# sanderslab/magellanmapper

Hardware: AMD Instinct MI355X
Metric: Mvoxels/s, 2048x2048x1024 uint16 stack, 5-sigma LoG blob detection (higher is better)
Workload: dtype f16x2 MFMA (f32 accumulate) + 16-bit fixed-point intermediates; f64 re-score of every candidate

## Files before the change

### include/mmx.h

```cpp
#ifndef MMX_H
#define MMX_H

#include <stddef.h>
#include <stdint.h>

#ifdef __cplusplus
extern "C" {
#endif

#define MMX_ABI_VERSION 19

typedef enum {
    MMX_OK = 0,
    MMX_ERR_ARG = 1,
    MMX_ERR_HIP = 2,
    MMX_ERR_NO_DEVICE = 3,
    MMX_ERR_WORKSPACE = 4,
    MMX_ERR_UNSUPPORTED = 5,
    MMX_DEFERRED = 6
} mmx_status;

typedef enum { MMX_U8 = 0, MMX_U16 = 1, MMX_F32 = 2, MMX_F64 = 3 } mmx_dtype;

#define MMX_MAX_RADIUS_FAST 24
#define MMX_MAX_RADIUS_GENERIC 255
#define MMX_MAX_BLOCKS 65535
#define MMX_COLOC_BALL 33

typedef struct {
    int64_t src_off;
    int32_t nz, ny, nx;
    int32_t slot;
    int32_t px;
    int32_t _pad;
} mmx_block;
#define MMX_ROW_ALIGN 32

typedef struct {
    const void* d_data;
    int32_t dtype;
    float value_range;
    int64_t stride_z, stride_y, stride_x;
} mmx_volume;

typedef struct {
    int32_t slot;
    int32_t s;
    int32_t z, y, x;
    uint32_t flags;
    float v;
    float nbr_max;
    double v64;
    uint64_t band;
} mmx_cand;

#define MMX_CAND_CONTESTED 1u
#define MMX_CAND_BAND 2u
#define MMX_CAND_PROBE 4u

int mmx_abi_version(void);
const char* mmx_strerror(int status);
const char* mmx_last_hip_error(void);
int mmx_device_count(void);

typedef enum {
    MMX_ZX_AUTO = -1,
    MMX_ZX_SEPARATE = 0,
    MMX_ZX_PACKED = 2,
    MMX_ZX_TILED = 6,
    MMX_ZX_TILED_Q16 = 7
} mmx_zx_mode;
#define MMX_ZX_PREPACKED 0x100
#define MMX_ZX_Y_VALU    0x200
#define MMX_MASK_ROWS 1
#define MMX_MASK_QUADS 2
int mmx_log_batch_f32(const mmx_volume* vol, const mmx_block* d_blocks, const mmx_block* h_blocks,
                      int n_blocks, int64_t slot_elems,
                      const double* h_w0, const double* h_w2, int radius, double norm,
                      float* d_log, float* d_work, uint64_t* d_nms_mask, float nms_lo, float nms_eps,
                      int* h_mask_written, int zx_mode, int* h_zx_path, void* stream);

#define MMX_LOG_ABS_TOL 1e-4

double mmx_tiled_q16_error_bound(const double* h_w0, const double* h_w2, int radius, double norm);

int mmx_zx_pack(const mmx_volume* vol, const mmx_block* d_blocks, const mmx_block* h_blocks, int n_blocks,
                int64_t slot_elems, float* d_work, void* stream);

size_t mmx_workspace_bytes(int n_blocks, int64_t slot_elems, int n_sigma, int with_masks);

int mmx_log_batch_f32_generic(const mmx_volume* vol, const mmx_block* d_blocks,
                              const mmx_block* h_blocks, int n_blocks, int64_t slot_elems,
                              const double* h_w0, const double* h_w2, int radius, double norm,
                              float* d_log, float* d_work, void* stream);

int mmx_peaks_batch(const float* d_log, const uint64_t* d_nms_mask, int mask_layout, int n_sigma, const mmx_block* d_blocks,
                    const mmx_block* h_blocks, int n_blocks, int64_t slot_elems,
                    float thr, float eps, mmx_cand* d_cands, uint32_t cap,
                    uint32_t* d_count, void* stream);

int mmx_rescore_f64(const mmx_volume* vol, const mmx_block* d_blocks, int n_blocks,
                    mmx_cand* d_pts, uint32_t cap, const uint32_t* d_count,
                    const double* d_w0, const double* d_w2, const int32_t* h_radius,
                    const double* h_norm, int n_sigma, int store_f32, void* stream);

int mmx_expand_probes(mmx_cand* d_cands, uint32_t cap, uint32_t* d_count, uint32_t* d_n_cands,
                      const mmx_block* d_blocks, int n_blocks, int n_sigma, void* stream);

typedef struct {
    const mmx_volume* vol32;
    const mmx_volume* vol_exact;
    const mmx_block* d_blocks;
    const mmx_block* h_blocks;
    int32_t n_blocks, n_sigma;
    int64_t slot_elems;
    const double* h_w0; const double* h_w2;
    const double* d_w0; const double* d_w2;
    const int32_t* h_radius;
    const double* h_norm;
    float* d_work;
    size_t work_bytes;
    float thr, eps;
    mmx_cand* d_cands;
    uint32_t cap, h_prefix;
    uint32_t* d_count;
    uint32_t* h_count;
    mmx_cand* h_cands;
    int32_t zx_mode, zx_flags, store_f32, exact, expand, _pad;
    void* stream; void* tail_stream; void* pack_stream;
    void* ev_work_free; void* ev_work_read; void* ev_done;
} mmx_detect_args;
typedef struct {
    int32_t zx_path;
    int32_t mask_layout;
    int32_t n_pass_rounds;
    int32_t _pad;
    double q16_bound;
} mmx_detect_info;
int mmx_detect_batch(const mmx_detect_args* args, mmx_detect_info* info);
const char* mmx_detect_last_error(void);
int mmx_log_scales_f32(const mmx_detect_args* args, mmx_detect_info* info);
int mmx_detect_batch_capture(const mmx_detect_args* args, mmx_detect_info* info, void** graph);
int mmx_graph_launch(void* graph, void* stream, void* ev_done, mmx_detect_info* info);
int mmx_graph_destroy(void* graph);
int mmx_event_synchronize(void* ev);
int mmx_stream_wait_event(void* stream, void* ev);
int mmx_timing_is_enabled(void);

int mmx_overlap_pairs(const double* d_blobs, const int32_t* d_offsets, int n_blocks,
                      double overlap, double band, double max_sigma, int32_t* d_pairs, double* d_frac,
                      uint32_t cap, uint32_t* d_count, void* stream);

int mmx_close_pairs(const int32_t* d_master, int n_master, const int32_t* d_check, int n_check,
                    const int32_t tol[3], int32_t* d_last, uint8_t* d_hit, void* stream);

typedef struct {
    int64_t src_off;
    int64_t dst_off;
    int64_t scratch_off;
    int32_t nz, ny, nx;
    int32_t qclass;
} mmx_subblock;

typedef struct {
    int32_t lo_prev, lo_next, hi_prev, hi_next;
    double lo_gamma, hi_gamma;
} mmx_quantile_class;

typedef struct {
    double clip_min, clip_max;
    double max_thresh;
    double unsharp_strength;
    double erosion_threshold;
    int32_t radius;
    int32_t rgb_guess;
    double tv_weight;
    double tv_factor;
} mmx_preproc_params;

#define MMX_PP_IDENTITY 1
#define MMX_PP_ERODED 2
#define MMX_PP_EXACT_MEAN 4
typedef struct {
    double vmin, vmax, mean;
    int32_t flags;
    int32_t _pad;
} mmx_subblock_info;

#define MMX_PP_RADIUS 32
#define MMX_PP_MAX_SIDE 32
#define MMX_PP_MAX_LDS 163840

int64_t mmx_preprocess_fast_lds(int nz, int ny, int nx);

int mmx_preprocess_batch(const mmx_volume* vol, const mmx_subblock* d_subs, const mmx_subblock* h_subs,
                         int n_subs, const mmx_quantile_class* d_qclasses, int n_qclasses,
                         const mmx_preproc_params* params, const double* d_weights,
                         int64_t dst_sy, int64_t dst_sz, float* d_out32, double* d_out64,
                         mmx_subblock_info* d_info, void* stream);

#define MMX_PP_AUTO 0
#define MMX_PP_SINGLE 1
#define MMX_PP_PIPELINED 2
#define MMX_PP_TILES_PER_WG 8
int64_t mmx_preprocess_work_bytes(const mmx_subblock* h_subs, int n_subs);
int mmx_preprocess_batch_mode(const mmx_volume* vol, const mmx_subblock* d_subs, const mmx_subblock* h_subs,
                              int n_subs, const mmx_quantile_class* d_qclasses, int n_qclasses,
                              const mmx_preproc_params* params, const double* d_weights,
                              int64_t dst_sy, int64_t dst_sz, float* d_out32, double* d_out64,
                              mmx_subblock_info* d_info, int mode, int tiles_per_wg,
                              void* d_work, int64_t work_bytes, void* stream);

int mmx_preprocess_batch_generic(const mmx_volume* vol, const mmx_subblock* d_subs,
                                 const mmx_subblock* h_subs, int n_subs,
                                 const mmx_quantile_class* d_qclasses, int n_qclasses,
                                 const mmx_preproc_params* params, const double* d_weights,
                                 int64_t dst_sy, int64_t dst_sz, float* d_out32, double* d_out64,
                                 mmx_subblock_info* d_info, double* d_scratch, int64_t scratch_doubles,
                                 void* stream);

int mmx_coloc_means(const mmx_volume* vol, const mmx_block* d_blocks, int n_blocks,
                    const int32_t* d_blobs, const int32_t* d_offsets, int n_blobs,
                    double* d_mean, int32_t* d_count, void* stream);
int mmx_coloc_voxels(const mmx_volume* vol, const mmx_block* d_blocks, int n_blocks,
                     const int32_t* d_blobs, const int32_t* d_offsets, int n_blobs,
                     double* d_mean, int32_t* d_count, double* d_voxels, void* stream);

int mmx_unmix_batch(const mmx_volume* vol, const mmx_volume* h_subs, const double* h_facs, int n_subs,
                    const mmx_block* d_blocks, const mmx_block* h_blocks, int n_blocks,
                    int64_t dst_slot, int64_t dst_sy, int64_t dst_sz,
                    float* d_out32, double* d_out64, void* stream);

typedef struct {
    int64_t src_off;
    int32_t in_nz, in_ny, in_nx;
    int32_t out_nz, out_ny, out_nx;
    int32_t slot;
    int32_t tz, ty, tx;
} mmx_resize_block;
int mmx_minmax_batch(const mmx_volume* vol, const mmx_block* d_blocks, const mmx_block* h_blocks,
                     int n_blocks, double* d_minmax, void* stream);
int mmx_resize_batch(const mmx_volume* vol, const mmx_resize_block* d_blocks,
                     const mmx_resize_block* h_blocks, int n_blocks,
                     const int32_t* d_index, const double* d_weight, const double* d_minmax,
                     int64_t dst_slot, int64_t dst_sy, int64_t dst_sz,
                     void* d_out, float* d_out32, void* stream);

int mmx_resize_batch_as(const mmx_volume* vol, const mmx_resize_block* d_blocks,
                        const mmx_resize_block* h_blocks, int n_blocks,
                        const int32_t* d_index, const double* d_weight, const double* d_minmax,
                        int64_t dst_slot, int64_t dst_sy, int64_t dst_sz,
                        int out_dtype, void* d_out, float* d_out32, void* stream);

int mmx_gauss_axis_batch(const mmx_volume* vol, const mmx_block* d_blocks, const mmx_block* h_blocks,
                         int n_blocks, int axis, const double* d_weights, const int32_t* d_radius,
                         int w_pitch, int nearest, int64_t dst_slot, int64_t dst_sy, int64_t dst_sz,
                         void* d_out, void* stream);

typedef struct { int32_t z0, z1; int64_t rank[4]; } mmx_rank_group;
size_t mmx_order_stats_workspace(int n_groups);
int mmx_order_stats(const mmx_volume* vol, int64_t nz, int64_t ny, int64_t nx,
                    const mmx_rank_group* d_groups, const mmx_rank_group* h_groups, int n_groups,
                    double* d_stats , int32_t* d_nan ,
                    void* d_work, size_t work_bytes, void* stream);

#define MMX_K_COUNT 13
int mmx_timing_enable(int on);
int mmx_timing_read(double* ms, int64_t* launches, int n);

int mmx_copy_rect_h2d(void* d_dst, size_t dpitch, const void* h_src, size_t spitch, size_t width, size_t height,
                      void* stream);
int mmx_host_stage_upload(const void* h_src, void* d_dst, const int64_t* regions, int32_t n_regions, int64_t nz,
                          int64_t ny, int64_t row_bytes, void* const* h_staging, int64_t staging_bytes, int32_t depth,
                          void* const* events, void* stream, int32_t device, int64_t* n_queued, const int32_t* cancel,
                          int32_t n_threads);
int mmx_event_query(void* ev);
int mmx_event_create(void** ev);
int mmx_event_destroy(void* ev);
int mmx_event_record(void* ev, void* stream);
int mmx_event_elapsed_ms(void* start, void* stop, float* ms);

int mmx_host_prune_axis(const int32_t* zyx, const int32_t* tag, double* abs_zyx,
                        const int64_t* cur, int64_t n_cur, int axis, int n_sections,
                        const double* bounds, double last_end, const int32_t tol[3],
                        const double* nxt_lo, const double* nxt_hi,
                        int64_t* out_cur, int64_t* out_n,
                        int64_t* n_slab, int64_t* n_after, int64_t* n_next);

typedef struct {
    const int32_t* src_cols;
    int64_t n_out, n_main;
    int32_t abs_dst[3];
} mmx_row_layout;
int mmx_host_take_rows(const double* table, int64_t ld, const int64_t* rows, int64_t n, const double* abs_zyx,
                       const mmx_row_layout* layout, double* out, double* out_rest);
int mmx_host_gather_parts_by_key(const double* table, int64_t ld, int32_t n_parts, const int64_t* const* ids,
                                 const int64_t* const* keys, const double* const* abs_rows, const int64_t* n_rows,
                                 int64_t n_keys, const mmx_row_layout* layout, double* out, int64_t out_rows,
                                 double* out_rest);

int mmx_host_prune_region(const int32_t* zyx, const int32_t* tag, double* abs_zyx, const int64_t* cur, int64_t n_cur,
                          int64_t own_lo, int64_t own_hi, const int32_t n_sections[3], const double* const bounds[3],
                          const double last_end[3], const int32_t tol[3], const double* const nxt_lo[3],
                          const double* const nxt_hi[3], int64_t* out_rows, int64_t* out_keys, int64_t* out_n,
                          int64_t* n_slab, int64_t* n_after, int64_t* n_next, int64_t stat_ld);
int mmx_host_prune_parts(const int32_t* zyx, const int32_t* tag, const double* abs_zyx, const double* chan,
                         int64_t chan_ld, const int64_t* parts, int n_parts, int own_part, const int32_t box_lo[3],
                         const int32_t box_hi[3], const double* channels, int n_channels,
                         const int32_t n_sections[3], const double* const bounds[3], const double last_end[3],
                         const int32_t tol[3], const double* const nxt_lo[3], const double* const nxt_hi[3],
                         int64_t n_keys, int64_t* out_ids, int64_t* out_keys, double* out_abs, int64_t* out_n,
                         int64_t* n_slab, int64_t* n_after, int64_t* n_next, int64_t stat_ld);
int mmx_host_rows_in_boxes(const int32_t* zyx, const int32_t* tag, const double* abs_zyx, const double* chan,
                           int64_t chan_ld, int64_t n, const int32_t* box_lo, const int32_t* box_hi, int n_boxes,
                           double* out, int64_t cap, int64_t* out_n);
int mmx_host_append_rows(const double* payload, int64_t n, const int32_t lo[3], const int32_t hi[3], int32_t* zyx,
                         int32_t* tag, double* abs_zyx, double* chan, int64_t chan_ld, int64_t at, int64_t cap,
                         int64_t* out_n);
int mmx_host_emit_parts(const double* table, int64_t ld, int32_t n_parts, const int64_t* const* ids,
                        const int64_t* const* keys, const double* const* abs_rows, const int64_t* n_rows,
                        const mmx_row_layout* layout, double* out, int64_t out_rows);
int mmx_host_merge_parts_by_key(const double* const* parts, const int64_t* n_rows, int32_t n_parts, int64_t ld,
                                int64_t n_keys, int64_t n_cols, double* out, int64_t out_rows);

int mmx_host_map_columns(const double* table, int64_t ld, int64_t n, const int32_t* src_cols,
                         int32_t n_map, double* out, int64_t out_ld, int32_t dst_col0);

int mmx_host_resolve_peaks(const mmx_cand* cands, uint32_t n_cands, uint32_t n_total, const mmx_block* blocks,
                           int n_blocks, int n_sigma, double thr, int32_t* out_nz_coords, double* out_nz_vals,
                           int32_t* out_coords, double* out_vals, int32_t* offsets, uint8_t* ties, double* stats);
int mmx_host_overlap_prune(const int32_t* coords, const int32_t* offsets, int n_blocks, const double* sigmas,
                           int n_sigma, double overlap, double band, uint8_t* alive, uint8_t* open_blocks,
                           int32_t* pairs, double* frac, int64_t cap, int64_t* n_pairs, int64_t* n_knife);
int mmx_host_emit_tables(const int32_t* coords, const uint8_t* alive, const int32_t* offsets, int n_blocks,
                         const double* sigmas, int n_sigma, double channel, const double* block_offsets,
                         const int32_t* block_tags, const int32_t* interior, double* store, int64_t ld,
                         int32_t* zyx, int32_t* tag, double* abs_zyx, int64_t row0, int64_t capacity,
                         int64_t* rows_per_block);
int mmx_host_emit_tables_multi(int32_t n_channels, const int32_t* const* coords, const uint8_t* const* alive,
                               const int32_t* const* offsets, int n_blocks, const double* const* sigmas,
                               const int32_t* n_sigma, const double* channel_ids, const double* block_offsets,
                               const int32_t* block_tags, const int32_t* interior, double* store, int64_t ld,
                               int32_t n_extra, int32_t* zyx, int32_t* tag, double* abs_zyx, int64_t row0,
                               int64_t capacity, int64_t* rows_per_block, uint8_t* any_before, int32_t* coloc_rows);
int mmx_host_coloc_flags(const double* means, const int32_t* mean_channels, int32_t n_mean_channels, int64_t n,
                         const int32_t* rows, const int64_t* row_offsets, int n_blocks, const int32_t* shapes,
                         int32_t n_channels, double* flags, int64_t ld);

typedef struct {
    const mmx_cand* cands; uint32_t n_cands, n_total;
    const mmx_block* blocks; int32_t n_blocks, n_sigma;
    double thr, eps;
    const double* sigmas; double overlap, overlap_band;
    double channel;
    const double* block_offsets; const int32_t* block_tags; const int32_t* interior;
    double* store; int64_t ld; int32_t* zyx; int32_t* tag; double* abs_zyx; int64_t capacity;
    int64_t* rows_per_block; uint8_t* any_before;
    const int32_t* n_sections; const double* const* bounds; const double* last_end; const int32_t* tol;
    const double* const* nxt_lo; const double* const* nxt_hi;
    int64_t* n_slab; int64_t* n_after; int64_t* n_next; int64_t stat_ld;
    const int32_t* src_cols; int32_t n_out, abs_dst0;
    double* out; int64_t out_capacity; int64_t* out_rows;
    double* stats;
} mmx_finish_stack_args;
int mmx_host_finish_stack(const mmx_finish_stack_args* a);

int mmx_cdist_f64(const double* d_a, int64_t n, const double* d_b, int64_t m, int dim, double* d_out, void* stream);
int mmx_host_lsap(const double* cost, int64_t nr, int64_t nc, int64_t* out_rows, int64_t* out_cols);

int mmx_calib_stream(int kind, const void* d_in, void* d_out, int64_t n_elems, void* stream);

#ifdef __cplusplus
}
#endif
#endif
```

### magellanmapper_amd/_native.py

```python
from __future__ import annotations

import ctypes
import os
from ctypes import (POINTER, Structure, c_char_p, c_double, c_float, c_int, c_int32, c_int64,
                    c_uint8, c_uint32, c_void_p)

import numpy as np

_HERE = os.path.dirname(os.path.abspath(__file__))
LIB_PATH = os.environ.get("MMX_LIB_PATH") or os.path.join(_HERE, "libmmx_hip.so")

MMX_ABI_VERSION = 19
MMX_U8, MMX_U16, MMX_F32, MMX_F64 = 0, 1, 2, 3
MMX_MAX_RADIUS_FAST = 24
MMX_MAX_RADIUS_GENERIC = 255
MMX_CAND_CONTESTED = 1
MMX_CAND_BAND = 2
MMX_CAND_PROBE = 4
MMX_ZX_AUTO, MMX_ZX_SEPARATE, MMX_ZX_PACKED, MMX_ZX_MFMA_F32, MMX_ZX_MFMA_F16, MMX_ZX_MFMA_F16_LDS = -1, 0, 2, 3, 4, 5
MMX_ZX_TILED, MMX_ZX_TILED_Q16, MMX_ZX_PREPACKED, MMX_ZX_Y_VALU = 6, 7, 0x100, 0x200
MMX_MASK_ROWS, MMX_MASK_QUADS = 1, 2
MMX_MAX_BLOCKS = 65535
MMX_COLOC_BALL = 33

BLOCK_DTYPE = np.dtype([("src_off", "<i8"), ("nz", "<i4"), ("ny", "<i4"), ("nx", "<i4"),
                        ("slot", "<i4"), ("px", "<i4"), ("_pad", "<i4")], align=True)
MMX_ROW_ALIGN = 32
CAND_DTYPE = np.dtype([("slot", "<i4"), ("s", "<i4"), ("z", "<i4"), ("y", "<i4"), ("x", "<i4"),
                       ("flags", "<u4"), ("v", "<f4"), ("nbr_max", "<f4"), ("v64", "<f8"),
                       ("band", "<u8")], align=True)
assert BLOCK_DTYPE.itemsize == 32 and CAND_DTYPE.itemsize == 48
SUBBLOCK_DTYPE = np.dtype([("src_off", "<i8"), ("dst_off", "<i8"), ("scratch_off", "<i8"),
                           ("nz", "<i4"), ("ny", "<i4"), ("nx", "<i4"), ("qclass", "<i4")], align=True)
QCLASS_DTYPE = np.dtype([("lo_prev", "<i4"), ("lo_next", "<i4"), ("hi_prev", "<i4"), ("hi_next", "<i4"),
                         ("lo_gamma", "<f8"), ("hi_gamma", "<f8")], align=True)
SUBINFO_DTYPE = np.dtype([("vmin", "<f8"), ("vmax", "<f8"), ("mean", "<f8"), ("flags", "<i4"),
                          ("_pad", "<i4")], align=True)
assert SUBBLOCK_DTYPE.itemsize == 40 and QCLASS_DTYPE.itemsize == 32 and SUBINFO_DTYPE.itemsize == 32
MMX_PP_IDENTITY, MMX_PP_ERODED, MMX_PP_EXACT_MEAN = 1, 2, 4
MMX_PP_AUTO, MMX_PP_SINGLE, MMX_PP_PIPELINED = 0, 1, 2
RESIZE_DTYPE = np.dtype([("src_off", "<i8"), ("in_nz", "<i4"), ("in_ny", "<i4"), ("in_nx", "<i4"),
                         ("out_nz", "<i4"), ("out_ny", "<i4"), ("out_nx", "<i4"), ("slot", "<i4"),
                         ("tz", "<i4"), ("ty", "<i4"), ("tx", "<i4")], align=True)
assert RESIZE_DTYPE.itemsize == 48
RANK_GROUP_DTYPE = np.dtype([("z0", "<i4"), ("z1", "<i4"), ("rank", "<i8", (4,))], align=True)
assert RANK_GROUP_DTYPE.itemsize == 40


class Volume(Structure):
    _fields_ = [("d_data", c_void_p), ("dtype", c_int32), ("value_range", c_float),
                ("stride_z", c_int64), ("stride_y", c_int64), ("stride_x", c_int64)]


class DetectArgs(Structure):
    _fields_ = [("vol32", POINTER(Volume)), ("vol_exact", POINTER(Volume)), ("d_blocks", c_void_p),
                ("h_blocks", c_void_p), ("n_blocks", c_int32), ("n_sigma", c_int32), ("slot_elems", c_int64),
                ("h_w0", c_void_p), ("h_w2", c_void_p), ("d_w0", c_void_p), ("d_w2", c_void_p),
                ("h_radius", c_void_p), ("h_norm", c_void_p), ("d_work", c_void_p), ("work_bytes", ctypes.c_size_t),
                ("thr", c_float), ("eps", c_float), ("d_cands", c_void_p), ("cap", c_uint32), ("h_prefix", c_uint32),
                ("d_count", c_void_p), ("h_count", c_void_p), ("h_cands", c_void_p),
                ("zx_mode", c_int32), ("zx_flags", c_int32), ("store_f32", c_int32), ("exact", c_int32),
                ("expand", c_int32), ("_pad", c_int32),
                ("stream", c_void_p), ("tail_stream", c_void_p), ("pack_stream", c_void_p),
                ("ev_work_free", c_void_p), ("ev_work_read", c_void_p), ("ev_done", c_void_p)]


class FinishStackArgs(Structure):
    _fields_ = [("cands", c_void_p), ("n_cands", c_uint32), ("n_total", c_uint32),
                ("blocks", c_void_p), ("n_blocks", c_int32), ("n_sigma", c_int32),
                ("thr", c_double), ("eps", c_double),
                ("sigmas", c_void_p), ("overlap", c_double), ("overlap_band", c_double),
                ("channel", c_double),
                ("block_offsets", c_void_p), ("block_tags", c_void_p), ("interior", c_void_p),
                ("store", c_void_p), ("ld", c_int64), ("zyx", c_void_p), ("tag", c_void_p), ("abs_zyx", c_void_p),
                ("capacity", c_int64), ("rows_per_block", c_void_p), ("any_before", c_void_p),
                ("n_sections", c_void_p), ("bounds", c_void_p), ("last_end", c_void_p), ("tol", c_void_p),
                ("nxt_lo", c_void_p), ("nxt_hi", c_void_p),
                ("n_slab", c_void_p), ("n_after", c_void_p), ("n_next", c_void_p), ("stat_ld", c_int64),
                ("src_cols", c_void_p), ("n_out", c_int32), ("abs_dst0", c_int32),
                ("out", c_void_p), ("out_capacity", c_int64), ("out_rows", c_void_p),
                ("stats", c_void_p)]


MMX_DEFERRED = 6


class RowLayout(Structure):
    _fields_ = [("src_cols", POINTER(c_int32)), ("n_out", c_int64), ("n_main", c_int64), ("abs_dst", c_int32 * 3)]


class DetectInfo(Structure):
    _fields_ = [("zx_path", c_int32), ("mask_layout", c_int32), ("n_pass_rounds", c_int32), ("_pad", c_int32),
                ("q16_bound", c_double)]


class PreprocParams(Structure):
    _fields_ = [("clip_min", c_double), ("clip_max", c_double), ("max_thresh", c_double),
                ("unsharp_strength", c_double), ("erosion_threshold", c_double),
                ("radius", c_int32), ("rgb_guess", c_int32), ("tv_weight", c_double), ("tv_factor", c_double)]


class MmxError(RuntimeError):
    """A C-ABI call returned a non-zero status."""


_lib = None

SYMBOLS = (
    "mmx_abi_version", "mmx_strerror", "mmx_last_hip_error", "mmx_device_count",
    "mmx_detect_batch", "mmx_log_scales_f32", "mmx_detect_batch_capture", "mmx_graph_launch", "mmx_graph_destroy", "mmx_detect_last_error",
    "mmx_event_synchronize", "mmx_stream_wait_event", "mmx_timing_is_enabled",
    "mmx_log_batch_f32", "mmx_log_batch_f32_generic", "mmx_zx_pack", "mmx_tiled_q16_error_bound", "mmx_workspace_bytes", "mmx_peaks_batch", "mmx_rescore_f64",
    "mmx_overlap_pairs", "mmx_close_pairs", "mmx_event_create", "mmx_event_destroy",
    "mmx_event_record", "mmx_event_elapsed_ms", "mmx_timing_enable", "mmx_timing_read",
    "mmx_calib_stream", "mmx_host_prune_axis",
    "mmx_preprocess_fast_lds", "mmx_preprocess_batch", "mmx_preprocess_batch_mode", "mmx_preprocess_work_bytes", "mmx_preprocess_batch_generic",
    "mmx_coloc_means", "mmx_coloc_voxels", "mmx_host_take_rows", "mmx_host_map_columns", "mmx_resize_batch_as", "mmx_gauss_axis_batch", "mmx_unmix_batch", "mmx_minmax_batch", "mmx_resize_batch",
    "mmx_cdist_f64", "mmx_host_lsap", "mmx_expand_probes", "mmx_host_resolve_peaks", "mmx_host_overlap_prune",
    "mmx_host_emit_tables", "mmx_host_prune_region", "mmx_host_prune_parts", "mmx_host_rows_in_boxes", "mmx_host_append_rows", "mmx_host_emit_parts", "mmx_host_merge_parts_by_key", "mmx_host_gather_parts_by_key", "mmx_host_emit_tables_multi", "mmx_host_coloc_flags", "mmx_host_finish_stack", "mmx_copy_rect_h2d", "mmx_host_stage_upload", "mmx_event_query",
    "mmx_order_stats_workspace", "mmx_order_stats",
)
KERNEL_KINDS = ("zpass", "ypass", "xpass", "generic", "peaks", "rescore", "overlap_pairs",
                "close_pairs", "zxpass", "y2pass", "preproc", "coloc", "zxpack")


def lib() -> ctypes.CDLL:
    global _lib
    if _lib is not None:
        return _lib
    if not os.path.exists(LIB_PATH):
        raise MmxError(
            f"{LIB_PATH} not found: the HIP extension has not been built "
            "(run __graft_entry__.build() or make -C magellanmapper_amd/csrc). "
            "There is no CPU fallback for this path.")
    try:
        import torch
    except ImportError:
        pass
    L = ctypes.CDLL(LIB_PATH)
    vp = c_void_p
    L.mmx_abi_version.restype = c_int
    L.mmx_strerror.restype = c_char_p
    L.mmx_strerror.argtypes = [c_int]
    L.mmx_last_hip_error.restype = c_char_p
    L.mmx_device_count.restype = c_int
    log_args = [POINTER(Volume), vp, vp, c_int, c_int64, POINTER(c_double), POINTER(c_double),
                c_int, c_double, vp, vp]
    L.mmx_log_batch_f32.argtypes = log_args + [vp, c_float, c_float, POINTER(c_int), c_int, POINTER(c_int), vp]
    L.mmx_log_batch_f32_generic.argtypes = log_args + [vp]
    L.mmx_workspace_bytes.argtypes = [c_int, c_int64, c_int, c_int]
    L.mmx_workspace_bytes.restype = ctypes.c_size_t
    L.mmx_zx_pack.argtypes = [POINTER(Volume), vp, vp, c_int, c_int64, vp, vp]
    L.mmx_tiled_q16_error_bound.argtypes = [POINTER(c_double), POINTER(c_double), c_int, c_double]
    L.mmx_tiled_q16_error_bound.restype = c_double
    L.mmx_peaks_batch.argtypes = [vp, vp, c_int, c_int, vp, vp, c_int, c_int64, c_float, c_float, vp,
                                  c_uint32, vp, vp]
    L.mmx_rescore_f64.argtypes = [POINTER(Volume), vp, c_int, vp, c_uint32, vp, vp, vp,
                                  POINTER(c_int32), POINTER(c_double), c_int, c_int, vp]
    L.mmx_overlap_pairs.argtypes = [vp, vp, c_int, c_double, c_double, c_double, vp, vp, c_uint32, vp, vp]
    L.mmx_close_pairs.argtypes = [vp, c_int, vp, c_int, POINTER(c_int32), vp, vp, vp]
    L.mmx_detect_batch.argtypes = [POINTER(DetectArgs), POINTER(DetectInfo)]
    L.mmx_log_scales_f32.argtypes = [POINTER(DetectArgs), POINTER(DetectInfo)]
    L.mmx_detect_batch_capture.argtypes = [POINTER(DetectArgs), POINTER(DetectInfo), POINTER(vp)]
    L.mmx_graph_launch.argtypes = [vp, vp, vp, POINTER(DetectInfo)]
    L.mmx_graph_destroy.argtypes = [vp]
    L.mmx_detect_last_error.restype = c_char_p
    L.mmx_event_synchronize.argtypes = [vp]
    L.mmx_stream_wait_event.argtypes = [vp, vp]
    L.mmx_event_create.argtypes = [POINTER(vp)]
    L.mmx_event_destroy.argtypes = [vp]
    L.mmx_event_record.argtypes = [vp, vp]
    L.mmx_event_elapsed_ms.argtypes = [vp, vp, POINTER(c_float)]
    L.mmx_timing_enable.argtypes = [c_int]
    L.mmx_timing_read.argtypes = [POINTER(c_double), POINTER(c_int64), c_int]
    L.mmx_calib_stream.argtypes = [c_int, vp, vp, c_int64, vp]
    L.mmx_host_prune_axis.argtypes = [vp, vp, vp, vp, c_int64, c_int, c_int, vp, c_double,
                                      POINTER(c_int32), vp, vp, vp, POINTER(c_int64), vp, vp, vp]
    L.mmx_preprocess_fast_lds.argtypes = [c_int, c_int, c_int]
    L.mmx_preprocess_fast_lds.restype = c_int64
    pre_args = [POINTER(Volume), vp, vp, c_int, vp, c_int, POINTER(PreprocParams), vp,
                c_int64, c_int64, vp, vp, vp]
    L.mmx_preprocess_batch.argtypes = pre_args + [vp]
    L.mmx_preprocess_batch_mode.argtypes = pre_args + [c_int, c_int, vp, c_int64, vp]
    L.mmx_preprocess_work_bytes.argtypes = [vp, c_int]
    L.mmx_preprocess_work_bytes.restype = c_int64
    L.mmx_preprocess_batch_generic.argtypes = pre_args + [vp, c_int64, vp]
    L.mmx_minmax_batch.argtypes = [POINTER(Volume), vp, vp, c_int, vp, vp]
    L.mmx_minmax_batch.restype = c_int
    L.mmx_resize_batch.argtypes = [POINTER(Volume), vp, vp, c_int, vp, vp, vp, c_int64, c_int64, c_int64,
                                   vp, vp, vp]
    L.mmx_resize_batch.restype = c_int
    L.mmx_resize_batch_as.argtypes = [POINTER(Volume), vp, vp, c_int, vp, vp, vp, c_int64, c_int64, c_int64,
                                      c_int, vp, vp, vp]
    L.mmx_resize_batch_as.restype = c_int
    L.mmx_gauss_axis_batch.argtypes = [POINTER(Volume), vp, vp, c_int, c_int, vp, vp, c_int, c_int,
                                       c_int64, c_int64, c_int64, vp, vp]
    L.mmx_gauss_axis_batch.restype = c_int
    L.mmx_unmix_batch.argtypes = [POINTER(Volume), POINTER(Volume), POINTER(c_double), c_int, vp, vp, c_int,
                                  c_int64, c_int64, c_int64, vp, vp, vp]
    L.mmx_unmix_batch.restype = c_int
    L.mmx_host_take_rows.argtypes = [vp, c_int64, vp, c_int64, vp, POINTER(RowLayout), vp, vp]
    L.mmx_host_map_columns.argtypes = [vp, c_int64, c_int64, POINTER(c_int32), c_int32, vp, c_int64, c_int32]
    L.mmx_cdist_f64.argtypes = [vp, c_int64, vp, c_int64, c_int, vp, vp]
    L.mmx_cdist_f64.restype = c_int
    L.mmx_host_lsap.argtypes = [vp, c_int64, c_int64, vp, vp]
    L.mmx_host_lsap.restype = c_int
    L.mmx_coloc_means.argtypes = [POINTER(Volume), vp, c_int, vp, vp, c_int, vp, vp, vp]
    L.mmx_coloc_means.restype = c_int
    L.mmx_coloc_voxels.argtypes = [POINTER(Volume), vp, c_int, vp, vp, c_int, vp, vp, vp, vp]
    L.mmx_coloc_voxels.restype = c_int
    L.mmx_expand_probes.argtypes = [vp, c_uint32, vp, vp, vp, c_int, c_int, vp]
    L.mmx_expand_probes.restype = c_int
    L.mmx_host_resolve_peaks.argtypes = [vp, c_uint32, c_uint32, vp, c_int, c_int, c_double, vp, vp, vp, vp, vp, vp, vp]
    L.mmx_host_overlap_prune.argtypes = [vp, vp, c_int, vp, c_int, c_double, c_double, vp, vp, vp, vp, c_int64,
                                         POINTER(c_int64), POINTER(c_int64)]
    L.mmx_host_prune_region.argtypes = [vp, vp, vp, vp, c_int64, c_int64, c_int64, POINTER(c_int32), POINTER(vp),
                                        POINTER(c_double), POINTER(c_int32), POINTER(vp), POINTER(vp), vp, vp,
                                        POINTER(c_int64), vp, vp, vp, c_int64]
    L.mmx_host_prune_parts.argtypes = [vp, vp, vp, vp, c_int64, vp, c_int, c_int, POINTER(c_int32), POINTER(c_int32),
                                       vp, c_int, POINTER(c_int32), POINTER(vp), POINTER(c_double), POINTER(c_int32),
                                       POINTER(vp), POINTER(vp), c_int64, vp, vp, vp, POINTER(c_int64), vp, vp, vp,
                                       c_int64]
    L.mmx_host_rows_in_boxes.argtypes = [vp, vp, vp, vp, c_int64, c_int64, vp, vp, c_int, vp, c_int64, POINTER(c_int64)]
    L.mmx_host_append_rows.argtypes = [vp, c_int64, POINTER(c_int32), POINTER(c_int32), vp, vp, vp, vp, c_int64,
                                       c_int64, c_int64, POINTER(c_int64)]
    L.mmx_host_gather_parts_by_key.argtypes = [vp, c_int64, c_int32, vp, vp, vp, vp, c_int64, POINTER(RowLayout), vp, c_int64, vp]
    L.mmx_host_emit_parts.argtypes = [vp, c_int64, c_int32, vp, vp, vp, vp, POINTER(RowLayout), vp, c_int64]
    L.mmx_host_merge_parts_by_key.argtypes = [vp, vp, c_int32, c_int64, c_int64, c_int64, vp, c_int64]
    L.mmx_host_emit_tables_multi.argtypes = [c_int32, vp, vp, vp, c_int, vp, vp, vp, vp, vp, vp, vp, c_int64, c_int32, vp, vp,
                                             vp, c_int64, c_int64, vp, vp, vp]
    L.mmx_host_coloc_flags.argtypes = [vp, vp, c_int32, c_int64, vp, vp, c_int, vp, c_int32, vp, c_int64]
    L.mmx_host_finish_stack.argtypes = [POINTER(FinishStackArgs)]
    L.mmx_host_stage_upload.argtypes = [vp, vp, vp, c_int32, c_int64, c_int64, c_int64, vp, c_int64, c_int32, vp, vp, c_int32,
                                        vp, vp, c_int32]
    L.mmx_event_query.argtypes = [vp]
    L.mmx_copy_rect_h2d.argtypes = [vp, ctypes.c_size_t, vp, ctypes.c_size_t, ctypes.c_size_t, ctypes.c_size_t, vp]
    L.mmx_host_emit_tables.argtypes = [vp, vp, vp, c_int, vp, c_int, c_double, vp, vp, vp, vp, c_int64, vp, vp, vp,
                                       c_int64, c_int64, vp]
    L.mmx_order_stats_workspace.argtypes = [c_int]
    L.mmx_order_stats_workspace.restype = ctypes.c_size_t
    L.mmx_order_stats.argtypes = [POINTER(Volume), c_int64, c_int64, c_int64, vp, vp, c_int, vp, vp, vp, ctypes.c_size_t, vp]
    L.mmx_order_stats.restype = c_int
    L.mmx_preprocess_batch.restype = c_int
    L.mmx_preprocess_batch_mode.restype = c_int
    L.mmx_preprocess_batch_generic.restype = c_int
    for name in SYMBOLS:
        fn = getattr(L, name)
        if name in ("mmx_preprocess_fast_lds", "mmx_workspace_bytes", "mmx_preprocess_work_bytes",
                    "mmx_order_stats_workspace"):
            continue
        if fn.restype is None or name.startswith(("mmx_log", "mmx_peaks", "mmx_rescore",
                                                  "mmx_overlap", "mmx_close", "mmx_event", "mmx_timing", "mmx_calib", "mmx_host")):
            fn.restype = c_int
    if L.mmx_abi_version() != MMX_ABI_VERSION:
        raise MmxError("libmmx_hip.so ABI version mismatch")
    _lib = L
    return L


def check(status: int, what: str) -> None:
    if status != 0:
        L = lib()
        msg = L.mmx_strerror(status).decode()
        hip = L.mmx_last_hip_error().decode()
        raise MmxError(f"{what}: {msg}" + (f" ({hip})" if hip else ""))


def as_double_ptr(a: np.ndarray):
    assert a.dtype == np.float64 and a.flags.c_contiguous
    return a.ctypes.data_as(POINTER(c_double))


def as_int32_ptr(a: np.ndarray):
    assert a.dtype == np.int32 and a.flags.c_contiguous
    return a.ctypes.data_as(POINTER(c_int32))


def timing_enable(on: bool = True, kinds=None) -> None:
    mask = 1 if on else 0
    if on and kinds is not None:
        mask = 0
        for k in kinds:
            mask |= 1 << (KERNEL_KINDS.index(k) + 1)
    check(lib().mmx_timing_enable(mask), "mmx_timing_enable")


def timing_read() -> dict:
    ms = (c_double * len(KERNEL_KINDS))()
    n = (c_int64 * len(KERNEL_KINDS))()
    check(lib().mmx_timing_read(ms, n, len(KERNEL_KINDS)), "mmx_timing_read")
    return {k: (ms[i], n[i]) for i, k in enumerate(KERNEL_KINDS)}


def keep_host_heap(mmap_threshold: int = 1 << 30, trim_threshold: int = (1 << 31) - 1) -> bool:
    try:
        libc = ctypes.CDLL("libc.so.6")
        ok1 = libc.mallopt(-3, int(mmap_threshold))
        ok2 = libc.mallopt(-1, int(trim_threshold))
        return bool(ok1 and ok2)
    except (OSError, AttributeError):
        return False
```

### magellanmapper_amd/csrc/mmx_api.hip

```cpp

#include <atomic>
#include <cstdio>
#include <cstdlib>
#include <cstring>

#include "mmx_common.h"

int mmx_launch_generic_pass(int pass, const mmx_volume* vol, const mmx_block* d_blocks, int n_blocks,
                            int max_vox, int64_t slot_elems, const float* w0, const float* w2, int radius,
                            const float* in1, const float* in2, float* out1, float* out2, hipStream_t s);
int mmx_launch_peaks(const float* d_log, int n_sigma, int64_t sigma_stride, const mmx_block* d_blocks,
                     int n_blocks, int max_vox, int64_t slot_elems, float thr, float eps,
                     mmx_cand* d_cands, uint32_t cap, uint32_t* d_count, hipStream_t stream);
int mmx_launch_peaks_sparse(const float* d_log, const unsigned long long* d_mask, int n_sigma,
                            int64_t sigma_stride, const mmx_block* d_blocks, int n_blocks, int max_vox,
                            int64_t slot_elems, float thr, float eps, mmx_cand* d_cands, uint32_t cap,
                            uint32_t* d_count, int quads, hipStream_t stream);

#include <mutex>
#include <vector>

namespace {
thread_local char g_hip_err[256] = "";

struct span { hipEvent_t a, b; int kind; };
std::mutex g_tm;
bool g_timing = false;
uint32_t g_kinds = ~0u;
std::vector<span> g_spans;
std::vector<hipEvent_t> g_pool;
hipEvent_t g_open[MMX_K_COUNT];

hipEvent_t take_event()
{
    if (!g_pool.empty()) { hipEvent_t e = g_pool.back(); g_pool.pop_back(); return e; }
    hipEvent_t e = nullptr;
    hipEventCreate(&e);
    return e;
}

int hip_fail(hipError_t e, const char* what)
{
    snprintf(g_hip_err, sizeof g_hip_err, "%s: %s", what, hipGetErrorString(e));
    return MMX_ERR_HIP;
}

constexpr int kColPrefetch = 4;
}

void mmx_time_begin(int kind, hipStream_t s)
{
    std::lock_guard<std::mutex> lk(g_tm);
    if (!g_timing || !((g_kinds >> kind) & 1u)) return;
    g_open[kind] = take_event();
    hipEventRecord(g_open[kind], s);
}

void mmx_time_end(int kind, hipStream_t s)
{
    std::lock_guard<std::mutex> lk(g_tm);
    if (!g_timing || !g_open[kind]) return;
    hipEvent_t b = take_event();
    hipEventRecord(b, s);
    g_spans.push_back({g_open[kind], b, kind});
    g_open[kind] = nullptr;
}

extern "C" {

int mmx_timing_enable(int on)
{
    std::lock_guard<std::mutex> lk(g_tm);
    for (auto& sp : g_spans) { g_pool.push_back(sp.a); g_pool.push_back(sp.b); }
    g_spans.clear();
    for (int k = 0; k < MMX_K_COUNT; ++k) g_open[k] = nullptr;
    g_timing = on != 0;
    g_kinds = on == 1 ? ~0u : ((uint32_t)on >> 1);
    return MMX_OK;
}

int mmx_timing_is_enabled(void)
{
    std::lock_guard<std::mutex> lk(g_tm);
    return g_timing ? 1 : 0;
}

int mmx_timing_read(double* ms, int64_t* launches, int n)
{
    if (!ms || !launches || n < MMX_K_COUNT) return MMX_ERR_ARG;
    std::lock_guard<std::mutex> lk(g_tm);
    for (int k = 0; k < n; ++k) { ms[k] = 0.0; launches[k] = 0; }
    for (auto& sp : g_spans) {
        hipError_t r = hipEventSynchronize(sp.b);
        if (r != hipSuccess) return hip_fail(r, "hipEventSynchronize");
        float t = 0.f;
        r = hipEventElapsedTime(&t, sp.a, sp.b);
        if (r != hipSuccess) return hip_fail(r, "hipEventElapsedTime");
        ms[sp.kind] += t;
        launches[sp.kind] += 1;
        g_pool.push_back(sp.a);
        g_pool.push_back(sp.b);
    }
    g_spans.clear();
    return MMX_OK;
}

int mmx_abi_version(void) { return MMX_ABI_VERSION; }
size_t mmx_workspace_bytes(int n_blocks, int64_t slot_elems, int n_sigma, int with_masks)
{
    if (n_blocks < 1 || slot_elems < 1 || n_sigma < 1) return 0;
    size_t bytes = (size_t)(4 + n_sigma) * (size_t)n_blocks * (size_t)slot_elems * sizeof(float);
    if (with_masks) {
        bytes = (bytes + 15) & ~(size_t)15;
        bytes += (size_t)n_sigma * (((size_t)n_blocks * (size_t)slot_elems) >> 5) * 16;
    }
    return bytes;
}

const char* mmx_strerror(int status)
{
    switch (status) {
        case MMX_OK: return "ok";
        case MMX_ERR_ARG: return "bad argument";
        case MMX_ERR_HIP: return "HIP runtime error";
        case MMX_ERR_NO_DEVICE: return "no gfx950 device";
        case MMX_ERR_WORKSPACE: return "workspace too small";
        case MMX_ERR_UNSUPPORTED: return "unsupported configuration";
        case MMX_DEFERRED: return "left to the caller";
        default: return "unknown status";
    }
}

const char* mmx_last_hip_error(void) { return g_hip_err; }


int mmx_device_count(void)
{
    int n = 0;
    hipError_t e = hipGetDeviceCount(&n);
    if (e != hipSuccess) { hip_fail(e, "hipGetDeviceCount"); return -1; }
    int ok = 0;
    for (int i = 0; i < n; ++i) {
        hipDeviceProp_t p;
        if (hipGetDeviceProperties(&p, i) == hipSuccess && strncmp(p.gcnArchName, "gfx950", 6) == 0) ++ok;
    }
    return ok;
}

static void q16_bounds(const double* w0, const double* w2, int radius, double norm, double* bp, double* bq, double* err)
{
    double s0 = w0[0], s2 = fabs(w2[0]);
    for (int k = 1; k <= radius; ++k) { s0 += 2.0 * w0[k]; s2 += 2.0 * fabs(w2[k]); }
    *bp = s0 * s0 * (1.0 + 1e-6);
    double pos = 0.0, neg = 0.0;
    for (int i = 0; i <= radius; ++i)
        for (int j = 0; j <= radius; ++j) {
            const double k = (w2[i] * w0[j] + w0[i] * w2[j]) * ((i ? 2.0 : 1.0) * (j ? 2.0 : 1.0));
            if (k > 0.0) pos += k; else neg -= k;
        }
    *bq = (pos > neg ? pos : neg) * (1.0 + 1e-4);
    const double drop = 255.0 / 65536.0 / 2048.0;
    const double biased = 4.0 * 0x1p-22;
    const double ydrop = 255.0 / 4096.0;
    *err = norm * (s2 * (*bp / 65535.0 * (0.5 + ydrop) + drop * s0 * s0 + biased * *bp) +
                   s0 * (*bq / 32767.0 * (0.5 + ydrop) + drop * 2.0 * s2 * s0 + biased * *bq)) + 1e-6;
}

double mmx_tiled_q16_error_bound(const double* h_w0, const double* h_w2, int radius, double norm)
{
    if (!h_w0 || !h_w2 || radius < 0 || radius > MMX_MAX_RADIUS_GENERIC) return -1.0;
    double bp, bq, err;
    q16_bounds(h_w0, h_w2, radius, norm, &bp, &bq, &err);
    return err;
}

}

void mmx_batch_geom_make(const mmx_volume* vol, const mmx_block* h_blocks, int n_blocks, int64_t slot_elems,
                         mmx_batch_geom* g)
{
    *g = mmx_batch_geom{};
    g->min_nz = g->min_ny = g->min_nx = 1 << 30;
    g->plan_status = MMX_ERR_UNSUPPORTED;
    g->rows_fit = g->quads_fit = true;
    if (n_blocks < 1 || n_blocks > MMX_MAX_BLOCKS) {
        g->status = n_blocks < 1 ? MMX_ERR_ARG : MMX_ERR_UNSUPPORTED;
        return;
    }
    for (int i = 0; i < n_blocks; ++i) {
        const mmx_block& b = h_blocks[i];
        if (b.nz < 1 || b.ny < 1 || b.nx < 1 || b.slot != i || b.px < b.nx || b.px % MMX_ROW_ALIGN) {
            if (g->status == MMX_OK) g->status = MMX_ERR_ARG;
            g->bad_block = true;
            return;
        }
        if ((int64_t)b.nz * b.ny * b.px > slot_elems && g->status == MMX_OK) g->status = MMX_ERR_WORKSPACE;
        if (b.nz < g->min_nz) g->min_nz = b.nz;
        if (b.ny < g->min_ny) g->min_ny = b.ny;
        if (b.nx < g->min_nx) g->min_nx = b.nx;
        if (b.ny > g->max_ny) g->max_ny = b.ny;
        if (b.nx > g->max_nx) g->max_nx = b.nx;
        if (b.px > g->max_px) g->max_px = b.px;
        if (b.ny * b.px > g->max_zcols) g->max_zcols = b.ny * b.px;
        if (b.nz * b.px > g->max_ycols) g->max_ycols = b.nz * b.px;
        if (b.nz * b.ny > g->max_rows) g->max_rows = b.nz * b.ny;
        if (b.nz * b.ny * b.px > g->max_vox) g->max_vox = b.nz * b.ny * b.px;
        if ((int64_t)b.ny * (((int64_t)b.nz * b.px + 63) >> 6) > (slot_elems >> 5) - 1) g->rows_fit = false;
        if ((int64_t)b.ny * ((b.nz + 3) >> 2) * ((b.nx + 15) >> 4) > (slot_elems >> 5) - 1) g->quads_fit = false;
        if (vol) {
            const int64_t lane = (int64_t)(b.ny - 1) * vol->stride_y + (int64_t)(b.nx - 1) * vol->stride_x;
            if (lane > g->max_lane_in) g->max_lane_in = lane;
        }
    }
    if (vol) g->plan_status = mmx_zx6_plan_make(h_blocks, n_blocks, slot_elems, vol->dtype, &g->plan);
}

namespace {

struct pass_weights {
    float z0[MMX_MAX_RADIUS_GENERIC + 1], z2[MMX_MAX_RADIUS_GENERIC + 1];
    float y0[MMX_MAX_RADIUS_GENERIC + 1], y2[MMX_MAX_RADIUS_GENERIC + 1];
    float x0[MMX_MAX_RADIUS_GENERIC + 1], x2[MMX_MAX_RADIUS_GENERIC + 1];
};
void make_weights(const mmx_volume* vol, const double* h_w0, const double* h_w2, int radius, double norm, pass_weights* w)
{
    double in_scale = 1.0;
    if (vol->dtype == MMX_U8) in_scale = 1.0 / 255.0;
    else if (vol->dtype == MMX_U16) in_scale = 1.0 / 65535.0;
    for (int k = 0; k <= radius; ++k) {
        w->z0[k] = (float)(h_w0[k] * in_scale);
        w->z2[k] = (float)(h_w2[k] * in_scale);
        w->y0[k] = (float)h_w0[k];
        w->y2[k] = (float)h_w2[k];
        w->x0[k] = (float)(-norm * h_w0[k]);
        w->x2[k] = (float)(-norm * h_w2[k]);
    }
}
mmx_taps_f32 taps(const float* a, const float* b, int radius)
{
    mmx_taps_f32 t;
    for (int k = 0; k <= MMX_MAX_RADIUS_FAST; ++k) {
        t.w0[k] = k <= radius ? a[k] : 0.f;
        t.w2[k] = k <= radius ? b[k] : 0.f;
    }
    return t;
}

int check_log_args(mmx_log_call* c, bool* y_valu, bool* prepacked)
{
    *y_valu = c->zx_mode >= 0 && (c->zx_mode & MMX_ZX_Y_VALU);
    if (*y_valu) c->zx_mode &= ~MMX_ZX_Y_VALU;
    *prepacked = c->zx_mode == (MMX_ZX_TILED | MMX_ZX_PREPACKED) || c->zx_mode == (MMX_ZX_TILED_Q16 | MMX_ZX_PREPACKED);
    if (*prepacked) c->zx_mode &= ~MMX_ZX_PREPACKED;
    if (c->zx_mode < MMX_ZX_AUTO || c->zx_mode > MMX_ZX_TILED_Q16 || c->zx_mode == 1 || (c->zx_mode >= 3 && c->zx_mode <= 5))
        return MMX_ERR_ARG;
    if (!c->vol || !c->vol->d_data || !c->d_blocks || !c->h_blocks || !c->h_w0 || !c->h_w2 || !c->d_log || !c->d_work)
        return MMX_ERR_ARG;
    if (c->n_blocks < 1 || c->radius < 0 || c->slot_elems < 1) return MMX_ERR_ARG;
    if (c->n_blocks > MMX_MAX_BLOCKS) return MMX_ERR_UNSUPPORTED;
    if (c->radius > MMX_MAX_RADIUS_GENERIC) return MMX_ERR_UNSUPPORTED;
    if (c->slot_elems >= (int64_t(1) << 29)) return MMX_ERR_UNSUPPORTED;
    if (c->slot_elems % MMX_ROW_ALIGN) return MMX_ERR_ARG;
    if (c->vol->dtype != MMX_U8 && c->vol->dtype != MMX_U16 && c->vol->dtype != MMX_F32)
        return MMX_ERR_UNSUPPORTED;
    return MMX_OK;
}

int fused_passes(const mmx_log_call& c, bool y_valu, bool prepacked, const mmx_batch_geom& g, const pass_weights& w)
{
    const mmx_volume* vol = c.vol;
    const int radius = c.radius, n_blocks = c.n_blocks;
    const int64_t slot_elems = c.slot_elems;
    hipStream_t s = c.stream;
    const bool fast_r = radius >= 1 && radius <= MMX_MAX_RADIUS_FAST;
    const bool lane_ok = g.max_lane_in * 8 < (int64_t(1) << 31);
    const bool fused = c.zx_mode != MMX_ZX_SEPARATE && fast_r && lane_ok && g.min_ny >= radius + kColPrefetch &&
                       g.min_nz >= radius + 1 && g.min_nx >= radius && g.max_px <= 512 && vol->stride_y < (1 << 30);
    if (!fused) return MMX_ERR_UNSUPPORTED;
    float* t0 = c.d_work;
    float* t1 = c.d_work + (int64_t)n_blocks * slot_elems;
    mmx_taps_f32 tzz = taps(w.z0, w.z2, radius), txx = taps(w.y0, w.y2, radius), tyy = taps(w.x0, w.x2, radius);
    int rc, path = MMX_ZX_PACKED;
    double q_bp = 0, q_bq = 0, q_err = 0, vscale = 0;
    q16_bounds(c.h_w0, c.h_w2, radius, c.norm, &q_bp, &q_bq, &q_err);
    const bool integer = vol->dtype == MMX_U8 || vol->dtype == MMX_U16;
    const bool ranged = vol->dtype == MMX_F32 && vol->value_range != 0.f && fabsf(vol->value_range) < 60000.f;
    const bool wants_entries = c.d_nms_mask && c.h_mask_written;
    const bool q16 = mmx_tiles_q16(c.zx_mode, vol, q_err, c.nms_eps, wants_entries, &vscale);
    const bool nonneg = vscale > 0.0;
    if (q16) { q_bp *= vscale; q_bq *= vscale; }
    bool tiled = (c.zx_mode == MMX_ZX_TILED || (c.zx_mode == MMX_ZX_TILED_Q16 && nonneg) ||
                  (c.zx_mode == MMX_ZX_AUTO && (integer || ranged))) && g.plan_status == MMX_OK;
    const mmx_zx6_plan& plan = g.plan;
    if (tiled && !prepacked) {
        mmx_timed_scope ts(MMX_K_ZXPACK, s);
        rc = mmx_launch_zx6_pack(vol, c.d_blocks, c.h_blocks, n_blocks, plan, c.d_work, s);
        if (rc == MMX_ERR_HIP) return hip_fail(hipGetLastError(), "voxel copy of the tiled path");
        tiled = rc == MMX_OK;
    }
    { mmx_timed_scope ts(MMX_K_ZX, s);
      rc = MMX_ERR_UNSUPPORTED;
      if (tiled) {
          path = q16 ? MMX_ZX_TILED_Q16 : MMX_ZX_TILED;
          rc = mmx_launch_zx6(vol, c.d_blocks, c.h_blocks, n_blocks, plan, txx, radius, c.d_work,
                              q16 ? (float)(1.0 / q_bp) : 0.f, q16 ? (float)(1.0 / q_bq) : 0.f, s);
          tiled = rc == MMX_OK;
      }
      if (rc == MMX_ERR_UNSUPPORTED) {
          path = MMX_ZX_PACKED;
          rc = mmx_launch_zx2(vol, c.d_blocks, n_blocks, g.max_ny, g.max_px, slot_elems, tzz, txx, radius, t0, t1, s);
      } }
    if (rc == MMX_OK && c.h_zx_path) *c.h_zx_path = path;
    if (rc == MMX_OK) {
        mmx_timed_scope ts(MMX_K_Y2, s);
        const bool want_mask = wants_entries && (tiled ? g.quads_fit : g.rows_fit);
        unsigned long long* d_mask = want_mask ? (unsigned long long*)c.d_nms_mask : nullptr;
        rc = MMX_ERR_UNSUPPORTED;
        if (tiled && q16 && !y_valu)
            rc = mmx_launch_ym(c.d_blocks, n_blocks, plan, slot_elems, tyy, radius, c.d_work,
                               (float)(q_bp / 65535.0), (float)(q_bq / 32767.0), c.d_log, d_mask, c.nms_lo, c.nms_eps, s);
        if (rc != MMX_ERR_UNSUPPORTED) ;
        else if (tiled)
            rc = mmx_launch_y6(c.d_blocks, n_blocks, plan, slot_elems, tyy, radius, c.d_work,
                               reinterpret_cast<const float*>(reinterpret_cast<const char*>(c.d_work) + plan.q_off),
                               q16 ? (float)(q_bp / 65535.0) : 0.f, q16 ? (float)(q_bq / 32767.0) : 0.f, c.d_log,
                               d_mask, c.nms_lo, c.nms_eps, s);
        else
            rc = mmx_launch_y2(c.d_blocks, n_blocks, g.max_ycols, slot_elems, tyy, radius, t0, t1, c.d_log,
                               d_mask, c.nms_lo, c.nms_eps, s);
        if (rc == MMX_OK && want_mask) *c.h_mask_written = tiled ? MMX_MASK_QUADS : MMX_MASK_ROWS;
    }
    return rc == MMX_ERR_HIP ? hip_fail(hipGetLastError(), "fused passes") : rc;
}

int separate_passes(const mmx_log_call& c, const mmx_batch_geom& g, const pass_weights& w)
{
    const mmx_volume* vol = c.vol;
    const int radius = c.radius, n_blocks = c.n_blocks;
    const int64_t slot_elems = c.slot_elems;
    hipStream_t s = c.stream;
    float* t0 = c.d_work;
    float* t1 = t0 + (int64_t)n_blocks * slot_elems;
    float* t2 = t1 + (int64_t)n_blocks * slot_elems;
    float* t3 = t2 + (int64_t)n_blocks * slot_elems;
    const bool fast_r = radius >= 1 && radius <= MMX_MAX_RADIUS_FAST;
    const bool lane_ok = g.max_lane_in * 8 < (int64_t(1) << 31);
    const bool fast_z = fast_r && lane_ok && g.min_nz >= radius + kColPrefetch && vol->stride_y < (1 << 30);
    const bool fast_y = fast_r && g.min_ny >= radius + kColPrefetch;
    const bool fast_x = fast_r && g.min_nx >= radius;
    int rc;
    { mmx_timed_scope ts(fast_z ? MMX_K_ZPASS : MMX_K_GENERIC, s);
    if (fast_z) rc = mmx_launch_zpass(vol, c.d_blocks, n_blocks, g.max_zcols, slot_elems, taps(w.z0, w.z2, radius), radius, t0, t1, s);
    else rc = mmx_launch_generic_pass(0, vol, c.d_blocks, n_blocks, g.max_vox, slot_elems, w.z0, w.z2, radius, nullptr, nullptr, t0, t1, s); }
    if (rc != MMX_OK) return rc == MMX_ERR_HIP ? hip_fail(hipGetLastError(), "z pass") : rc;
    { mmx_timed_scope ts(fast_y ? MMX_K_YPASS : MMX_K_GENERIC, s);
    if (fast_y) rc = mmx_launch_ypass(c.d_blocks, n_blocks, g.max_ycols, slot_elems, taps(w.y0, w.y2, radius), radius, t0, t1, t2, t3, s);
    else rc = mmx_launch_generic_pass(1, vol, c.d_blocks, n_blocks, g.max_vox, slot_elems, w.y0, w.y2, radius, t0, t1, t2, t3, s); }
    if (rc != MMX_OK) return rc == MMX_ERR_HIP ? hip_fail(hipGetLastError(), "y pass") : rc;
    { mmx_timed_scope ts(fast_x ? MMX_K_XPASS : MMX_K_GENERIC, s);
    if (fast_x) rc = mmx_launch_xpass(c.d_blocks, n_blocks, g.max_rows, g.max_nx, slot_elems, taps(w.x0, w.x2, radius), radius, t2, t3, c.d_log, s);
    else rc = mmx_launch_generic_pass(2, vol, c.d_blocks, n_blocks, g.max_vox, slot_elems, w.x0, w.x2, radius, t2, t3, c.d_log, nullptr, s); }
    if (rc != MMX_OK) return rc == MMX_ERR_HIP ? hip_fail(hipGetLastError(), "x pass") : rc;
    return MMX_OK;
}

}

int mmx_log_scale_f32(const mmx_log_call& call, const mmx_batch_geom& g)
{
    mmx_log_call c = call;
    if (c.h_mask_written) *c.h_mask_written = 0;
    if (c.h_zx_path) *c.h_zx_path = MMX_ZX_SEPARATE;
    bool y_valu, prepacked;
    int rc = check_log_args(&c, &y_valu, &prepacked);
    if (rc != MMX_OK) return rc;
    if (g.status != MMX_OK) return g.status;
    pass_weights w;
    make_weights(c.vol, c.h_w0, c.h_w2, c.radius, c.norm, &w);
    rc = fused_passes(c, y_valu, prepacked, g, w);
    if (rc != MMX_ERR_UNSUPPORTED) return rc;
    return separate_passes(c, g, w);
}

int mmx_zx_pack_geom(const mmx_volume* vol, const mmx_block* d_blocks, const mmx_block* h_blocks, int n_blocks,
                     int64_t slot_elems, const mmx_batch_geom& g, float* d_work, hipStream_t stream)
{
    if (!vol || !vol->d_data || !d_blocks || !h_blocks || !d_work || n_blocks < 1 || slot_elems < 1) return MMX_ERR_ARG;
    if (n_blocks > MMX_MAX_BLOCKS) return MMX_ERR_UNSUPPORTED;
    if (vol->dtype != MMX_U8 && vol->dtype != MMX_U16 && vol->dtype != MMX_F32) return MMX_ERR_UNSUPPORTED;
    if (g.bad_block) return MMX_ERR_ARG;
    if (g.plan_status != MMX_OK) return g.plan_status;
    mmx_timed_scope ts(MMX_K_ZXPACK, stream);
    const int rc = mmx_launch_zx6_pack(vol, d_blocks, h_blocks, n_blocks, g.plan, d_work, stream);
    return rc == MMX_ERR_HIP ? hip_fail(hipGetLastError(), "voxel copy of the tiled path") : rc;
}

extern "C" {

int mmx_log_batch_f32(const mmx_volume* vol, const mmx_block* d_blocks, const mmx_block* h_blocks,
                      int n_blocks, int64_t slot_elems,
                      const double* h_w0, const double* h_w2, int radius, double norm,
                      float* d_log, float* d_work, uint64_t* d_nms_mask, float nms_lo, float nms_eps,
                      int* h_mask_written, int zx_mode, int* h_zx_path, void* stream)
{
    mmx_batch_geom g{};
    if (vol && h_blocks) mmx_batch_geom_make(vol, h_blocks, n_blocks, slot_elems, &g);
    return mmx_log_scale_f32({vol, d_blocks, h_blocks, n_blocks, slot_elems, h_w0, h_w2, radius, norm, d_log, d_work,
                              d_nms_mask, nms_lo, nms_eps, h_mask_written, zx_mode, h_zx_path, (hipStream_t)stream}, g);
}

int mmx_log_batch_f32_generic(const mmx_volume* vol, const mmx_block* d_blocks, const mmx_block* h_blocks,
                              int n_blocks, int64_t slot_elems,
                              const double* h_w0, const double* h_w2, int radius, double norm,
                              float* d_log, float* d_work, void* stream)
{
    if (!vol || !vol->d_data || !d_blocks || !h_blocks || !h_w0 || !h_w2 || !d_log || !d_work)
        return MMX_ERR_ARG;
    if (n_blocks < 1 || radius < 0 || radius > MMX_MAX_RADIUS_GENERIC || slot_elems < 1) return MMX_ERR_ARG;
    if (n_blocks > MMX_MAX_BLOCKS) return MMX_ERR_UNSUPPORTED;
    mmx_batch_geom g;
    mmx_batch_geom_make(vol, h_blocks, n_blocks, slot_elems, &g);
    if (g.status != MMX_OK) return g.status;
    pass_weights w;
    make_weights(vol, h_w0, h_w2, radius, norm, &w);
    const int64_t n_slots = n_blocks;
    float* t0 = d_work;
    float* t1 = d_work + n_slots * slot_elems;
    float* t2 = t1 + n_slots * slot_elems;
    float* t3 = t2 + n_slots * slot_elems;
    hipStream_t s = (hipStream_t)stream;
    int rc = mmx_launch_generic_pass(0, vol, d_blocks, n_blocks, g.max_vox, slot_elems, w.z0, w.z2, radius, nullptr, nullptr, t0, t1, s);
    if (rc != MMX_OK) return rc;
    rc = mmx_launch_generic_pass(1, vol, d_blocks, n_blocks, g.max_vox, slot_elems, w.y0, w.y2, radius, t0, t1, t2, t3, s);
    if (rc != MMX_OK) return rc;
    return mmx_launch_generic_pass(2, vol, d_blocks, n_blocks, g.max_vox, slot_elems, w.x0, w.x2, radius, t2, t3, d_log, nullptr, s);
}

int mmx_zx_pack(const mmx_volume* vol, const mmx_block* d_blocks, const mmx_block* h_blocks, int n_blocks,
                int64_t slot_elems, float* d_work, void* stream)
{
    mmx_batch_geom g{};
    if (vol && h_blocks) mmx_batch_geom_make(vol, h_blocks, n_blocks, slot_elems, &g);
    return mmx_zx_pack_geom(vol, d_blocks, h_blocks, n_blocks, slot_elems, g, d_work, (hipStream_t)stream);
}

int mmx_peaks_batch(const float* d_log, const uint64_t* d_nms_mask, int mask_layout, int n_sigma, const mmx_block* d_blocks,
                    const mmx_block* h_blocks, int n_blocks, int64_t slot_elems,
                    float thr, float eps, mmx_cand* d_cands, uint32_t cap,
                    uint32_t* d_count, void* stream)
{
    if (!d_log || !d_blocks || !h_blocks || !d_cands || !d_count) return MMX_ERR_ARG;
    if (n_sigma < 1 || n_blocks < 1 || slot_elems < 1 || !(eps >= 0.f)) return MMX_ERR_ARG;
    if (n_blocks > MMX_MAX_BLOCKS) return MMX_ERR_UNSUPPORTED;
    if (slot_elems % MMX_ROW_ALIGN) return MMX_ERR_ARG;
    if (d_nms_mask && mask_layout != MMX_MASK_ROWS && mask_layout != MMX_MASK_QUADS) return MMX_ERR_ARG;
    mmx_batch_geom g;
    mmx_batch_geom_make(nullptr, h_blocks, n_blocks, slot_elems, &g);
    if (g.status != MMX_OK) return g.status;
    const int max_vox = g.max_vox;
    mmx_timed_scope ts(MMX_K_PEAKS, (hipStream_t)stream);
    int rc;
    if (d_nms_mask)
        rc = mmx_launch_peaks_sparse(d_log, (const unsigned long long*)d_nms_mask, n_sigma,
                                     (int64_t)n_blocks * slot_elems, d_blocks, n_blocks, max_vox, slot_elems,
                                     thr, eps, d_cands, cap, d_count, mask_layout == MMX_MASK_QUADS, (hipStream_t)stream);
    else
        rc = mmx_launch_peaks(d_log, n_sigma, (int64_t)n_blocks * slot_elems, d_blocks, n_blocks, max_vox,
                              slot_elems, thr, eps, d_cands, cap, d_count, (hipStream_t)stream);
    return rc == MMX_ERR_HIP ? hip_fail(hipGetLastError(), "peaks") : rc;
}

int mmx_copy_rect_h2d(void* d_dst, size_t dpitch, const void* h_src, size_t spitch, size_t width, size_t height,
                      void* stream)
{
    if (!d_dst || !h_src || width > dpitch || width > spitch) return MMX_ERR_ARG;
    if (!width || !height) return MMX_OK;
    hipError_t r = hipMemcpy2DAsync(d_dst, dpitch, h_src, spitch, width, height, hipMemcpyHostToDevice, (hipStream_t)stream);
    return r == hipSuccess ? MMX_OK : hip_fail(r, "hipMemcpy2DAsync");
}

int mmx_event_create(void** ev)
{
    if (!ev) return MMX_ERR_ARG;
    hipEvent_t e;
    hipError_t r = hipEventCreate(&e);
    if (r != hipSuccess) return hip_fail(r, "hipEventCreate");
    *ev = (void*)e;
    return MMX_OK;
}

int mmx_event_destroy(void* ev)
{
    hipError_t r = hipEventDestroy((hipEvent_t)ev);
    return r == hipSuccess ? MMX_OK : hip_fail(r, "hipEventDestroy");
}

int mmx_event_record(void* ev, void* stream)
{
    hipError_t r = hipEventRecord((hipEvent_t)ev, (hipStream_t)stream);
    return r == hipSuccess ? MMX_OK : hip_fail(r, "hipEventRecord");
}

int mmx_event_elapsed_ms(void* start, void* stop, float* ms)
{
    if (!ms) return MMX_ERR_ARG;
    hipError_t r = hipEventSynchronize((hipEvent_t)stop);
    if (r != hipSuccess) return hip_fail(r, "hipEventSynchronize");
    r = hipEventElapsedTime(ms, (hipEvent_t)start, (hipEvent_t)stop);
    return r == hipSuccess ? MMX_OK : hip_fail(r, "hipEventElapsedTime");
}

}
```

### magellanmapper_amd/csrc/mmx_common.h

```cpp
#pragma once

#include <hip/hip_runtime.h>
#include <stdint.h>

#include "../../include/mmx.h"

#define MMX_WG 256
#define MMX_MAX_GRID_X 2147483647

struct mmx_taps_f32 {
    float w0[MMX_MAX_RADIUS_FAST + 1];
    float w2[MMX_MAX_RADIUS_FAST + 1];
};

__host__ __device__ __forceinline__ int mmx_reflect(int i, int n)
{
    if (n == 1) return 0;
    const int period = 2 * n;
    i %= period;
    if (i < 0) i += period;
    return i < n ? i : period - 1 - i;
}

int mmx_launch_zpass(const mmx_volume* vol, const mmx_block* d_blocks, int n_blocks, int max_cols,
                     int64_t slot_elems, const mmx_taps_f32& taps, int radius,
                     float* d_gz, float* d_gzz, hipStream_t stream);
int mmx_launch_ypass(const mmx_block* d_blocks, int n_blocks, int max_cols, int64_t slot_elems,
                     const mmx_taps_f32& taps, int radius, const float* d_gz, const float* d_gzz,
                     float* d_a, float* d_bc, hipStream_t stream);
int mmx_launch_xpass(const mmx_block* d_blocks, int n_blocks, int max_rows, int max_nx,
                     int64_t slot_elems, const mmx_taps_f32& taps, int radius,
                     const float* d_a, const float* d_bc, float* d_log, hipStream_t stream);

int mmx_launch_zx2(const mmx_volume* vol, const mmx_block* d_blocks, int n_blocks, int max_ny, int max_px,
                   int64_t slot_elems, const mmx_taps_f32& tz, const mmx_taps_f32& tx, int radius,
                   float* d_p, float* d_q, hipStream_t s);
struct mmx_zx6_plan {
    int64_t tile_stride;
    int64_t pack_stride;
    int64_t q_off, tab_off, pack_off;
    int64_t tab_bytes;
    int max_tiles;
    int max_rowtiles;
};
int mmx_zx6_plan_make(const mmx_block* h_blocks, int n_blocks, int64_t slot_elems, int voxel_dtype, mmx_zx6_plan* plan);
int mmx_launch_zx6_pack(const mmx_volume* vol, const mmx_block* d_blocks, const mmx_block* h_blocks, int n_blocks,
                        const mmx_zx6_plan& plan, void* d_work, hipStream_t stream);
int mmx_launch_zx6(const mmx_volume* vol, const mmx_block* d_blocks, const mmx_block* h_blocks, int n_blocks,
                   const mmx_zx6_plan& plan, const mmx_taps_f32& tx, int radius, void* d_work, float qp, float qq,
                   hipStream_t stream);
int mmx_launch_y6(const mmx_block* d_blocks, int n_blocks, const mmx_zx6_plan& plan, int64_t slot_elems,
                  const mmx_taps_f32& taps, int radius, const float* d_p, const float* d_q, float cp, float cq,
                  float* d_log, unsigned long long* d_mask, float nms_lo, float nms_eps, hipStream_t stream);
int mmx_launch_ym(const mmx_block* d_blocks, int n_blocks, const mmx_zx6_plan& plan, int64_t slot_elems,
                  const mmx_taps_f32& taps, int radius, const float* d_p, float cp, float cq,
                  float* d_log, unsigned long long* d_mask, float nms_lo, float nms_eps, hipStream_t stream);
int mmx_launch_y2(const mmx_block* d_blocks, int n_blocks, int max_cols, int64_t slot_elems,
                  const mmx_taps_f32& taps, int radius, const float* d_p, const float* d_q,
                  float* d_log, unsigned long long* d_mask, float nms_lo, float nms_eps, hipStream_t stream);

struct mmx_batch_geom {
    int status;
    bool bad_block;
    int min_nz, min_ny, min_nx, max_ny, max_nx, max_px;
    int max_zcols, max_ycols, max_rows, max_vox;
    int64_t max_lane_in;
    bool rows_fit, quads_fit;
    mmx_zx6_plan plan;
    int plan_status;
};
void mmx_batch_geom_make(const mmx_volume* vol, const mmx_block* h_blocks, int n_blocks, int64_t slot_elems, mmx_batch_geom* g);

struct mmx_log_call {
    const mmx_volume* vol; const mmx_block* d_blocks; const mmx_block* h_blocks; int n_blocks; int64_t slot_elems;
    const double* h_w0; const double* h_w2; int radius; double norm;
    float* d_log; float* d_work; uint64_t* d_nms_mask; float nms_lo, nms_eps; int* h_mask_written;
    int zx_mode; int* h_zx_path; hipStream_t stream;
};
int mmx_log_scale_f32(const mmx_log_call& c, const mmx_batch_geom& g);
int mmx_zx_pack_geom(const mmx_volume* vol, const mmx_block* d_blocks, const mmx_block* h_blocks, int n_blocks,
                     int64_t slot_elems, const mmx_batch_geom& g, float* d_work, hipStream_t stream);

bool mmx_tiles_q16(int zx_mode, const mmx_volume* vol, double unit_bound, double band, bool entries_wanted, double* value_scale);

enum mmx_kernel_kind {
    MMX_K_ZPASS = 0, MMX_K_YPASS, MMX_K_XPASS, MMX_K_GENERIC, MMX_K_PEAKS, MMX_K_RESCORE,
    MMX_K_PAIRS, MMX_K_CLOSE, MMX_K_ZX, MMX_K_Y2, MMX_K_PREPROC, MMX_K_COLOC, MMX_K_ZXPACK, MMX_K_END
};
void mmx_time_begin(int kind, hipStream_t s);
void mmx_time_end(int kind, hipStream_t s);
static_assert(MMX_K_END == MMX_K_COUNT, "kernel kinds out of sync with mmx.h");
struct mmx_timed_scope {
    int kind; hipStream_t s;
    mmx_timed_scope(int k, hipStream_t st) : kind(k), s(st) { mmx_time_begin(k, st); }
    ~mmx_timed_scope() { mmx_time_end(kind, s); }
};
```

### magellanmapper_amd/csrc/mmx_detect.hip

```cpp

#include <algorithm>
#include <atomic>
#include <chrono>
#include <cstdlib>
#include <cmath>
#include <cstdio>
#include <cstring>
#include <mutex>
#include <thread>
#include <vector>

#include "mmx_common.h"

namespace {

thread_local char g_detect_err[256] = "";

std::mutex g_ev_mutex;
std::vector<hipEvent_t> g_ev_ring;
size_t g_ev_next = 0;
hipEvent_t ring_event()
{
    std::lock_guard<std::mutex> lk(g_ev_mutex);
    if (g_ev_ring.size() < 64) {
        hipEvent_t e = nullptr;
        if (hipEventCreateWithFlags(&e, hipEventDisableTiming) != hipSuccess) return nullptr;
        g_ev_ring.push_back(e);
        return e;
    }
    hipEvent_t e = g_ev_ring[g_ev_next];
    g_ev_next = (g_ev_next + 1) % g_ev_ring.size();
    return e;
}

int fail(hipError_t e, const char* what)
{
    snprintf(g_detect_err, sizeof g_detect_err, "%s: %s", what, hipGetErrorString(e));
    return MMX_ERR_HIP;
}

int after(hipStream_t a, hipStream_t b, const char* what)
{
    if (a == b) return MMX_OK;
    hipEvent_t e = ring_event();
    if (!e) return fail(hipErrorOutOfMemory, "hipEventCreate");
    hipError_t r = hipEventRecord(e, a);
    if (r != hipSuccess) return fail(r, what);
    r = hipStreamWaitEvent(b, e, 0);
    return r == hipSuccess ? MMX_OK : fail(r, what);
}

float* log_arrays(const mmx_detect_args* a) { return a->d_work + (size_t)4 * a->n_blocks * a->slot_elems; }
uint64_t* nms_entries(const mmx_detect_args* a)
{
    const float* end = log_arrays(a) + (size_t)a->n_sigma * a->n_blocks * a->slot_elems;
    return reinterpret_cast<uint64_t*>((reinterpret_cast<uintptr_t>(end) + 15) & ~(uintptr_t)15);
}

int passes(const mmx_detect_args* a, const mmx_batch_geom& g, bool with_mask, int mode, unsigned* layouts, int* zx_path,
           double* q16_bound, bool* pack_side)
{
    *layouts = 0;
    const mmx_volume* vol = a->vol32;
    const bool is_float = vol->dtype == MMX_F32;
    const bool float_ok = is_float && vol->value_range != 0.f;
    const int nb = a->n_blocks, ns = a->n_sigma;
    const int64_t slot = a->slot_elems;
    const size_t tab = MMX_MAX_RADIUS_GENERIC + 1;
    float* d_log = log_arrays(a);
    uint64_t* d_mask = nms_entries(a);
    const size_t mask_words = ((size_t)nb * slot) >> 5;
    int tiled_mode = MMX_ZX_TILED;
    if (mode == MMX_ZX_AUTO || mode == MMX_ZX_TILED_Q16) {
        double bound = 0.0;
        for (int s = 0; s < ns; ++s) {
            const double b = mmx_tiled_q16_error_bound(a->h_w0 + s * tab, a->h_w2 + s * tab, a->h_radius[s], a->h_norm[s]);
            if (b < 0) { bound = -1.0; break; }
            if (b > bound) bound = b;
        }
        double vscale;
        if (mmx_tiles_q16(mode, vol, bound, a->eps, true, &vscale)) { tiled_mode = MMX_ZX_TILED_Q16; *q16_bound = bound * vscale; }
    }
    bool packed = false;
    hipStream_t main = (hipStream_t)a->stream;
    if (((mode == MMX_ZX_AUTO || mode == MMX_ZX_TILED || mode == MMX_ZX_TILED_Q16) && !is_float) ||
        ((mode == MMX_ZX_AUTO || mode == MMX_ZX_TILED) && float_ok)) {
        hipStream_t ps = (*pack_side && a->pack_stream) ? (hipStream_t)a->pack_stream : main;
        int rc = mmx_zx_pack_geom(vol, a->d_blocks, a->h_blocks, nb, slot, g, a->d_work, ps);
        if (rc != MMX_OK && rc != MMX_ERR_UNSUPPORTED) return rc;
        if (ps != main) {
            const int st = after(ps, main, "voxel copy -> main stream");
            if (st != MMX_OK) return st;
            *pack_side = false;
        }
        packed = rc == MMX_OK;
    }
    for (int s = 0; s < ns; ++s) {
        int written = 0, path = 0;
        const int rc = mmx_log_scale_f32({vol, a->d_blocks, a->h_blocks, nb, slot, a->h_w0 + s * tab, a->h_w2 + s * tab,
                                          a->h_radius[s], a->h_norm[s], d_log + (size_t)s * nb * slot, a->d_work,
                                          with_mask ? d_mask + (size_t)s * mask_words * 2 : nullptr, a->thr - a->eps, a->eps,
                                          &written, packed ? (tiled_mode | MMX_ZX_PREPACKED | a->zx_flags) : mode, &path,
                                          main}, g);
        if (rc != MMX_OK) return rc;
        *zx_path = path;
        packed = packed && path == tiled_mode;
        *layouts |= 1u << (with_mask ? written : 0);
    }
    return MMX_OK;
}

}

bool mmx_tiles_q16(int zx_mode, const mmx_volume* vol, double unit_bound, double band, bool entries, double* value_scale)
{
    const bool ranged = vol->dtype == MMX_F32 && vol->value_range > 0.f && vol->value_range < 60000.f;
    *value_scale = vol->dtype == MMX_U8 || vol->dtype == MMX_U16 ? 1.0 : (ranged ? (double)vol->value_range : 0.0);
    if (!(*value_scale > 0.0)) return false;
    if (zx_mode == MMX_ZX_TILED_Q16) return true;
    const double bound = unit_bound * *value_scale;
    return zx_mode == MMX_ZX_AUTO && entries && bound >= 0.0 && 4.0 * bound <= band && bound <= MMX_LOG_ABS_TOL;
}

extern "C" {

const char* mmx_detect_last_error(void) { return g_detect_err; }

int mmx_log_scales_f32(const mmx_detect_args* a, mmx_detect_info* info)
{
    if (!a || !info) return MMX_ERR_ARG;
    memset(info, 0, sizeof *info);
    if (!a->vol32 || !a->d_blocks || !a->h_blocks || !a->h_w0 || !a->h_w2 || !a->h_radius || !a->h_norm || !a->d_work ||
        a->n_blocks < 1 || a->n_sigma < 1 || a->slot_elems < 1 || !(a->eps >= 0.f))
        return MMX_ERR_ARG;
    if (mmx_workspace_bytes(a->n_blocks, a->slot_elems, a->n_sigma, 1) > a->work_bytes) return MMX_ERR_WORKSPACE;
    hipStream_t main = (hipStream_t)a->stream;
    bool pack_side = a->pack_stream != nullptr && a->pack_stream != a->stream;
    if (a->ev_work_free) {
        hipError_t r = hipStreamWaitEvent(main, (hipEvent_t)a->ev_work_free, 0);
        if (r == hipSuccess && pack_side) r = hipStreamWaitEvent((hipStream_t)a->pack_stream, (hipEvent_t)a->ev_work_free, 0);
        if (r != hipSuccess) return fail(r, "wait for the workspace");
    }
    mmx_batch_geom g;
    mmx_batch_geom_make(a->vol32, a->h_blocks, a->n_blocks, a->slot_elems, &g);

    unsigned layouts = 0;
    int zx_path = 0;
    double q16_bound = 0.0;
    int rc = passes(a, g, true, a->zx_mode, &layouts, &zx_path, &q16_bound, &pack_side);
    if (rc != MMX_OK) return rc;
    if (layouts == ((1u << MMX_MASK_ROWS) | (1u << MMX_MASK_QUADS))) {
        rc = passes(a, g, true, MMX_ZX_PACKED, &layouts, &zx_path, &q16_bound, &pack_side);
        if (rc != MMX_OK) return rc;
        info->n_pass_rounds++;
    }
    if (layouts & (layouts - 1)) {
        rc = passes(a, g, false, a->zx_mode, &layouts, &zx_path, &q16_bound, &pack_side);
        if (rc != MMX_OK) return rc;
        info->n_pass_rounds++;
    }
    int mask_layout = 0;
    while (!(layouts & (1u << mask_layout))) ++mask_layout;
    info->zx_path = zx_path;
    info->mask_layout = mask_layout;
    info->q16_bound = zx_path == MMX_ZX_TILED_Q16 ? q16_bound : 0.0;
    info->n_pass_rounds++;
    return MMX_OK;
}

int mmx_detect_batch(const mmx_detect_args* a, mmx_detect_info* info)
{
    if (!a || !info) return MMX_ERR_ARG;
    memset(info, 0, sizeof *info);
    if (!a->d_cands || !a->d_count || a->cap < 1) return MMX_ERR_ARG;
    if (a->exact && (!a->vol_exact || !a->d_w0 || !a->d_w2)) return MMX_ERR_ARG;
    int rc = mmx_log_scales_f32(a, info);
    if (rc != MMX_OK) return rc;
    const int nb = a->n_blocks, ns = a->n_sigma;
    hipStream_t main = (hipStream_t)a->stream;
    hipStream_t tail = a->tail_stream ? (hipStream_t)a->tail_stream : main;
    hipError_t r;

    rc = after(main, tail, "LoG passes -> tail stream");
    if (rc != MMX_OK) return rc;
    r = hipMemsetAsync(a->d_count, 0, 2 * sizeof(uint32_t), tail);
    if (r != hipSuccess) return fail(r, "reset of the candidate counters");
    rc = mmx_peaks_batch(log_arrays(a), info->mask_layout ? nms_entries(a) : nullptr, info->mask_layout, ns, a->d_blocks, a->h_blocks,
                         nb, a->slot_elems, a->thr, a->eps, a->d_cands, a->cap, a->d_count, (void*)tail);
    if (rc != MMX_OK) return rc;
    if (a->ev_work_read) {
        r = hipEventRecord((hipEvent_t)a->ev_work_read, tail);
        if (r != hipSuccess) return fail(r, "record: workspace read");
    }
    if (a->expand) {
        rc = mmx_expand_probes(a->d_cands, a->cap, a->d_count, a->d_count + 1, a->d_blocks, nb, ns, (void*)tail);
        if (rc != MMX_OK) return rc;
    }
    if (a->exact) {
        rc = mmx_rescore_f64(a->vol_exact, a->d_blocks, nb, a->d_cands, a->cap, a->d_count, a->d_w0, a->d_w2,
                             a->h_radius, a->h_norm, ns, a->store_f32, (void*)tail);
        if (rc != MMX_OK) return rc;
    }
    if (a->h_count) {
        r = hipMemcpyAsync(a->h_count, a->d_count, 2 * sizeof(uint32_t), hipMemcpyDeviceToHost, tail);
        if (r != hipSuccess) return fail(r, "copy of the counters");
    }
    if (a->h_cands && a->h_prefix) {
        const size_t n = a->h_prefix < a->cap ? a->h_prefix : a->cap;
        r = hipMemcpyAsync(a->h_cands, a->d_cands, n * sizeof(mmx_cand), hipMemcpyDeviceToHost, tail);
        if (r != hipSuccess) return fail(r, "copy of the table's head");
    }
    if (a->ev_done) {
        r = hipEventRecord((hipEvent_t)a->ev_done, tail);
        if (r != hipSuccess) return fail(r, "record: batch done");
    }
    return MMX_OK;
}

int mmx_event_synchronize(void* ev)
{
    hipError_t r = hipEventSynchronize((hipEvent_t)ev);
    return r == hipSuccess ? MMX_OK : fail(r, "hipEventSynchronize");
}

int mmx_event_query(void* ev)
{
    hipError_t r = hipEventQuery((hipEvent_t)ev);
    if (r == hipSuccess) return 0;
    if (r == hipErrorNotReady) { (void)hipGetLastError(); return 1; }
    return fail(r, "hipEventQuery");
}

int mmx_stream_wait_event(void* stream, void* ev)
{
    hipError_t r = hipStreamWaitEvent((hipStream_t)stream, (hipEvent_t)ev, 0);
    return r == hipSuccess ? MMX_OK : fail(r, "hipStreamWaitEvent");
}

struct mmx_graph_s { hipGraph_t graph; hipGraphExec_t exec; mmx_detect_info info; };

int mmx_detect_batch_capture(const mmx_detect_args* a, mmx_detect_info* info, void** graph_out)
{
    if (!a || !info || !graph_out || !a->stream) return MMX_ERR_ARG;
    *graph_out = nullptr;
    hipStream_t main = (hipStream_t)a->stream;
    if (mmx_timing_is_enabled()) return MMX_ERR_UNSUPPORTED;
    hipError_t r = hipStreamBeginCapture(main, hipStreamCaptureModeThreadLocal);
    if (r != hipSuccess) return fail(r, "hipStreamBeginCapture");
    mmx_detect_args b = *a;
    b.ev_work_free = b.ev_work_read = b.ev_done = nullptr;
    b.pack_stream = nullptr;
    const int rc = mmx_detect_batch(&b, info);
    hipGraph_t g = nullptr;
    if (rc == MMX_OK && b.tail_stream && b.tail_stream != b.stream) {
        const int st = after((hipStream_t)b.tail_stream, main, "tail stream -> main stream");
        if (st != MMX_OK) { hipStreamEndCapture(main, &g); if (g) hipGraphDestroy(g); return st; }
    }
    r = hipStreamEndCapture(main, &g);
    if (rc != MMX_OK) { if (g) hipGraphDestroy(g); return rc; }
    if (r != hipSuccess || !g) return fail(r, "hipStreamEndCapture");
    hipGraphExec_t ex = nullptr;
    r = hipGraphInstantiate(&ex, g, nullptr, nullptr, 0);
    if (r != hipSuccess) { hipGraphDestroy(g); return fail(r, "hipGraphInstantiate"); }
    mmx_graph_s* out = new mmx_graph_s{g, ex, *info};
    *graph_out = out;
    return MMX_OK;
}

int mmx_graph_launch(void* graph, void* stream, void* ev_done, mmx_detect_info* info)
{
    if (!graph) return MMX_ERR_ARG;
    mmx_graph_s* g = static_cast<mmx_graph_s*>(graph);
    hipError_t r = hipGraphLaunch(g->exec, (hipStream_t)stream);
    if (r != hipSuccess) return fail(r, "hipGraphLaunch");
    if (ev_done) {
        r = hipEventRecord((hipEvent_t)ev_done, (hipStream_t)stream);
        if (r != hipSuccess) return fail(r, "record: graph done");
    }
    if (info) *info = g->info;
    return MMX_OK;
}

int mmx_graph_destroy(void* graph)
{
    if (!graph) return MMX_OK;
    mmx_graph_s* g = static_cast<mmx_graph_s*>(graph);
    hipGraphExecDestroy(g->exec);
    hipGraphDestroy(g->graph);
    delete g;
    return MMX_OK;
}

}


namespace {
struct spin_barrier {
    std::atomic<int> count{0};
    std::atomic<int> phase{0};
    int n = 1;
    void wait()
    {
        const int p = phase.load(std::memory_order_acquire);
        if (count.fetch_add(1, std::memory_order_acq_rel) + 1 == n) {
            count.store(0, std::memory_order_relaxed);
            phase.store(p + 1, std::memory_order_release);
        } else {
            int spins = 0;
            while (phase.load(std::memory_order_acquire) == p)
                if (++spins > 4000) std::this_thread::sleep_for(std::chrono::microseconds(40));
        }
    }
};
}

int mmx_host_stage_upload(const void* h_src, void* d_dst, const int64_t* regions, int32_t n_regions, int64_t nz,
                          int64_t ny, int64_t row_bytes, void* const* h_staging, int64_t staging_bytes, int32_t depth,
                          void* const* events, void* stream, int32_t device, int64_t* n_queued, const int32_t* cancel,
                          int32_t n_threads)
{
    if (!h_src || !d_dst || !regions || n_regions < 0 || nz < 0 || ny < 1 || row_bytes < 1 || !h_staging || depth < 1 ||
        !events || !n_queued || !cancel)
        return MMX_ERR_ARG;
    for (int k = 0; k < n_regions; ++k) {
        const int64_t* r = regions + 4 * (int64_t)k;
        if (r[0] < 0 || r[1] > nz || r[0] >= r[1] || r[2] < 0 || r[3] > ny || r[2] >= r[3] ||
            (r[1] - r[0]) * (r[3] - r[2]) * row_bytes > staging_bytes)
            return MMX_ERR_ARG;
    }
    if (hipSetDevice(device) != hipSuccess) return fail(hipGetLastError(), "hipSetDevice");
    const int T = std::max(1, std::min<int>(n_threads, 64));
    const int64_t plane = ny * row_bytes;
    std::atomic<int> status{MMX_OK};
    std::atomic<int> stop{0};
    spin_barrier go, filled;
    go.n = filled.n = T;
    const bool prof = getenv("MMX_STAGE_PROF") != nullptr;
    double t_wait = 0, t_fill = 0, t_queue = 0;
    auto now = [] { return std::chrono::duration<double, std::milli>(std::chrono::steady_clock::now().time_since_epoch()).count(); };
    const double t_begin = now();
    auto work = [&](int t) {
        for (int k = 0; k < n_regions; ++k) {
            const int64_t* r = regions + 4 * (int64_t)k;
            const int which = k % depth;
            double t0 = 0;
            if (t == 0) {
                if (prof) t0 = now();
                if (*(volatile const int32_t*)cancel) stop.store(1);
                else if (k >= depth && hipEventSynchronize((hipEvent_t)events[k - depth]) != hipSuccess) {
                    status.store(fail(hipGetLastError(), "hipEventSynchronize")); stop.store(1);
                }
                if (prof) { const double t1 = now(); t_wait += t1 - t0; t0 = t1; }
            }
            go.wait();
            if (stop.load()) return;
            const int64_t planes = r[1] - r[0], width = (r[3] - r[2]) * row_bytes;
            const int64_t a = planes * t / T, b = planes * (t + 1) / T;
            const char* src = (const char*)h_src + r[0] * plane + r[2] * row_bytes;
            char* dst = (char*)h_staging[which];
            for (int64_t z = a; z < b; ++z) std::memcpy(dst + z * width, src + z * plane, (size_t)width);
            filled.wait();
            if (t == 0) {
                if (prof) { const double t1 = now(); t_fill += t1 - t0; t0 = t1; }
                hipError_t e = hipMemcpy2DAsync((char*)d_dst + r[0] * plane + r[2] * row_bytes, (size_t)plane,
                                                h_staging[which], (size_t)width, (size_t)width, (size_t)planes,
                                                hipMemcpyHostToDevice, (hipStream_t)stream);
                if (e == hipSuccess) e = hipEventRecord((hipEvent_t)events[k], (hipStream_t)stream);
                if (e != hipSuccess) { status.store(fail(e, "staged upload")); stop.store(1); }
                else __atomic_store_n(n_queued, (int64_t)k + 1, __ATOMIC_RELEASE);
                if (prof) t_queue += now() - t0;
            }
        }
    };
    std::vector<std::thread> helpers;
    for (int t = 1; t < T; ++t) helpers.emplace_back(work, t);
    work(0);
    for (auto& h : helpers) h.join();
    if (prof)
        fprintf(stderr, "mmx_host_stage_upload: %d regions, %d threads, %.1f ms: waiting for staging buffers %.1f, filling %.1f, "
                "queueing copies %.1f\n", n_regions, T, now() - t_begin, t_wait, t_fill, t_queue);
    return status.load();
}
```

### magellanmapper_amd/csrc/mmx_fused.hip

```cpp

#include <type_traits>

#include "mmx_common.h"

namespace {

__device__ __forceinline__ int reflect_once(int i, int n)
{
    i = i < 0 ? -1 - i : i;
    return i >= n ? 2 * n - 1 - i : i;
}
__device__ __forceinline__ int reflect_clamped(int i, int n)
{
    i = reflect_once(i, n);
    return i < 0 ? 0 : (i >= n ? n - 1 : i);
}

using rsrc_t = __amdgpu_buffer_rsrc_t;
__device__ __forceinline__ rsrc_t make_rsrc(const void* p)
{
    return __builtin_amdgcn_make_buffer_rsrc(const_cast<void*>(p), 0, 0x7fffffff, 0x00020000);
}
template <typename T> struct vox;
template <> struct vox<uint8_t> {
    static __device__ __forceinline__ float load(rsrc_t r, unsigned o) { return __uint_as_float((unsigned)__builtin_amdgcn_raw_buffer_load_b8(r, o, 0, 0)); }
    static __device__ __forceinline__ float act(float raw) { return (float)__float_as_uint(raw); }
};
template <> struct vox<uint16_t> {
    static __device__ __forceinline__ float load(rsrc_t r, unsigned o) { return __uint_as_float((unsigned)__builtin_amdgcn_raw_buffer_load_b16(r, o, 0, 0)); }
    static __device__ __forceinline__ float act(float raw) { return (float)__float_as_uint(raw); }
};
template <> struct vox<float> {
    static __device__ __forceinline__ float load(rsrc_t r, unsigned o) { return __uint_as_float(__builtin_amdgcn_raw_buffer_load_b32(r, o, 0, 0)); }
    static __device__ __forceinline__ float act(float raw) { return raw; }
};

#ifndef Y2_PF
#define Y2_PF 4
#endif
constexpr int kPrefetch = Y2_PF;
typedef float v2f __attribute__((ext_vector_type(2)));
struct y2_taps {
    v2f w[MMX_MAX_RADIUS_FAST + 1];
};

template <int R, bool MASK>
__global__ void __launch_bounds__(MMX_WG)
y2_kernel(const mmx_block* __restrict__ blocks, int64_t slot_elems,
          const float* __restrict__ gp, const float* __restrict__ gq,
          float* __restrict__ out, y2_taps taps,
          unsigned long long* __restrict__ mask, float nms_lo, float nms_eps)
{
    using io = vox<float>;
    constexpr int N = 2 * R + 1;
    constexpr int M = N + kPrefetch;
    const mmx_block bd = blocks[blockIdx.y];
    const int ncol = bd.nz * bd.px;
    const int col = blockIdx.x * MMX_WG + threadIdx.x;
    if (col >= ncol) return;
    const int z = col / bd.px;
    const int x = col - z * bd.px;
    const int n = bd.ny;
    const int nx = bd.px;
    const unsigned voff = (unsigned)(z * bd.ny * nx + x) * 4u;
    const int64_t sbase = (int64_t)bd.slot * slot_elems;
    const float* i1 = gp + sbase;
    const float* i2 = gq + sbase;
    const float* w1 = out + sbase;

    const int lane = threadIdx.x & 63;
    const int nwords = (ncol + 63) >> 6;
    ulonglong2* mrow = MASK ? reinterpret_cast<ulonglong2*>(mask) + ((int64_t)bd.slot * slot_elems >> 5) + (col >> 6)
                            : nullptr;
    unsigned long long ab_prev = 0;
    const bool real = x < bd.nx;
    const bool has_l = lane > 0 && x > 0, has_r = lane < 63 && x + 1 < bd.nx && col + 1 < ncol;
    float prev1 = -INFINITY, prev2 = -INFINITY, nbx_prev = -INFINITY;
    int ydone = 0;

    v2f r[M];
#pragma unroll
    for (int j = -R; j < R + kPrefetch; ++j) {
        const int row = reflect_once(j, n) * nx;
        r[(j + M) % M] = (v2f){io::load(make_rsrc(i1 + row), voff), io::load(make_rsrc(i2 + row), voff)};
    }
    const rsrc_t rs1 = make_rsrc(i1), rs2 = make_rsrc(i2), rsw = make_rsrc(w1);
    const unsigned row_b = (unsigned)nx * 4u;
    unsigned qoff = (unsigned)(R + kPrefetch) * row_b;
    unsigned woff = 0;
    auto step = [&](int s, auto reflecting, int y) __attribute__((always_inline)) {
        float n1, n2;
        if constexpr (decltype(reflecting)::value) {
            const unsigned rnext = (unsigned)reflect_once(y + R + kPrefetch, n) * row_b;
            n1 = __uint_as_float(__builtin_amdgcn_raw_buffer_load_b32(rs1, voff, rnext, 0));
            n2 = __uint_as_float(__builtin_amdgcn_raw_buffer_load_b32(rs2, voff, rnext, 0));
        } else {
            n1 = __uint_as_float(__builtin_amdgcn_raw_buffer_load_b32(rs1, voff, qoff, 0));
            n2 = __uint_as_float(__builtin_amdgcn_raw_buffer_load_b32(rs2, voff, qoff, 0));
        }
        qoff += row_b;
        v2f a2 = r[s] * taps.w[0];
        v2f b2 = (r[(s - 1 + M) % M] + r[(s + 1) % M]) * taps.w[1];
#pragma unroll
        for (int k = 2; k <= R; k += 2) {
            const v2f sa = r[(s - k + M) % M] + r[(s + k) % M];
            a2 = __builtin_elementwise_fma(sa, taps.w[k], a2);
            if (k + 1 <= R) {
                const v2f sb = r[(s - k - 1 + M) % M] + r[(s + k + 1) % M];
                b2 = __builtin_elementwise_fma(sb, taps.w[k + 1], b2);
            }
        }
        a2 += b2;
        const float acc = a2.x + a2.y;
        const unsigned long long ab = MASK ? __ballot(real & (acc > nms_lo)) : ~0ull;
        if (ab) __builtin_amdgcn_raw_buffer_store_b32(__float_as_uint(acc), rsw, voff, woff, 0);
        woff += row_b;
        r[(s + R + kPrefetch) % M] = (v2f){n1, n2};
        if constexpr (MASK) {
            const float l = __uint_as_float((unsigned)__builtin_amdgcn_update_dpp(
                (int)__float_as_uint(acc), (int)__float_as_uint(acc), 0x138 , 0xf, 0xf, false));
            const float r = __uint_as_float((unsigned)__builtin_amdgcn_update_dpp(
                (int)__float_as_uint(acc), (int)__float_as_uint(acc), 0x130 , 0xf, 0xf, false));
            const float nbx = fmaxf(has_l ? l : -INFINITY, has_r ? r : -INFINITY);
            if (ydone > 0) {
                const bool cand = real & (prev1 > nms_lo) &
                                  !(fmaxf(fmaxf(prev2, acc), nbx_prev) > prev1 + nms_eps);
                const unsigned long long m = __ballot(cand);
                if (lane == 0) *mrow = make_ulonglong2(m, ab_prev);
                mrow += nwords;
            }
            prev2 = prev1; prev1 = acc; nbx_prev = nbx;
            ab_prev = ab;
            ++ydone;
        }
        __builtin_amdgcn_sched_barrier(0);
    };
    int y0 = 0;
#pragma unroll 1
    for (; y0 + M + R + kPrefetch <= n; y0 += M) {
#pragma unroll
        for (int s = 0; s < M; ++s) step(s, std::false_type{}, 0);
    }
#pragma unroll 1
    for (; y0 < n; y0 += M) {
#pragma unroll
        for (int s = 0; s < M; ++s) {
            if (y0 + s >= n) break;
            step(s, std::true_type{}, y0 + s);
        }
    }
    if constexpr (MASK) {
        const bool cand = real & (prev1 > nms_lo) & !(fmaxf(prev2, nbx_prev) > prev1 + nms_eps);
        const unsigned long long m = __ballot(cand);
        if (lane == 0) *mrow = make_ulonglong2(m, ab_prev);
    }
}

template <int R>
int launch_y2(const mmx_block* d_blocks, int n_blocks, int max_cols, int64_t slot_elems,
              const mmx_taps_f32& taps, const float* d_p, const float* d_q, float* d_log,
              unsigned long long* d_mask, float nms_lo, float nms_eps, hipStream_t s)
{
    dim3 grid((max_cols + MMX_WG - 1) / MMX_WG, n_blocks);
    y2_taps pk;
    for (int k = 0; k <= R; ++k) pk.w[k] = (v2f){taps.w2[k], taps.w0[k]};
    if (d_mask)
        hipLaunchKernelGGL((y2_kernel<R, true>), grid, dim3(MMX_WG), 0, s, d_blocks, slot_elems, d_p, d_q, d_log, pk,
                           d_mask, nms_lo, nms_eps);
    else
        hipLaunchKernelGGL((y2_kernel<R, false>), grid, dim3(MMX_WG), 0, s, d_blocks, slot_elems, d_p, d_q, d_log, pk,
                           d_mask, nms_lo, nms_eps);
    return hipGetLastError() == hipSuccess ? MMX_OK : MMX_ERR_HIP;
}

template <int R, bool MASK, bool Q16>
__global__ void __launch_bounds__(MMX_WG)
y6_kernel(const mmx_block* __restrict__ blocks, int64_t slot_elems, int64_t tile_stride,
          const float* __restrict__ gp, const float* __restrict__ gq,
          float* __restrict__ out, y2_taps taps,
          unsigned long long* __restrict__ mask, float nms_lo, float nms_eps)
{
    constexpr int N = 2 * R + 1;
    constexpr int M = N + kPrefetch;
    const mmx_block bd = blocks[blockIdx.y];
    const int ntx = (bd.nx + 15) >> 4, ntz = (bd.nz + 15) >> 4;
    const int tile = blockIdx.x;
    if (tile >= ntx * ntz) return;
    const int c = tile / ntz, U = tile - c * ntz;
    const int zq = __builtin_amdgcn_readfirstlane((int)(threadIdx.x >> 6));
    if (16 * U + 4 * zq >= bd.nz) return;
    const int lane = threadIdx.x & 63;
    const int xi = lane & 15;
    const int z = 16 * U + 4 * zq + (lane >> 4), x = 16 * c + xi;
    const int n = bd.ny;
    const bool real = z < bd.nz && x < bd.nx;
    const float* i1 = gp + (int64_t)bd.slot * tile_stride + (int64_t)tile * 256;
    const float* i2 = gq + (int64_t)bd.slot * tile_stride + (int64_t)tile * 256;
    const unsigned trow_b = (unsigned)(ntx * ntz) * 1024u;
    float* w1 = out + (int64_t)bd.slot * slot_elems;
    const unsigned voff = (unsigned)(zq * 64 + lane) * 4u;
    const unsigned ooff = (unsigned)((real ? z : 0) * bd.ny * bd.px + (real ? x : 0)) * 4u;
    const int nent = ((bd.nz + 3) >> 2) * ntx;
    ulonglong2* mrow = MASK ? reinterpret_cast<ulonglong2*>(mask) + ((int64_t)bd.slot * slot_elems >> 5) +
                              (4 * U + zq) * ntx + c
                            : nullptr;
    unsigned long long ab_prev = 0;
    const bool has_l = xi > 0, has_r = xi < 15 && x + 1 < bd.nx;
    float prev1 = -INFINITY, prev2 = -INFINITY, nbx_prev = -INFINITY;
    int ydone = 0;

    const rsrc_t rs1 = make_rsrc(i1), rs2 = make_rsrc(i2), rsw = make_rsrc(w1);
    auto unpack = [](unsigned d) __attribute__((always_inline)) {
        return (v2f){(float)(d & 0xffffu), (float)((int)d >> 16)};
    };
    v2f r[M];
#pragma unroll
    for (int j = -R; j < R + kPrefetch; ++j) {
        const unsigned row = (unsigned)reflect_once(j, n) * trow_b;
        if constexpr (Q16)
            r[(j + M) % M] = unpack(__builtin_amdgcn_raw_buffer_load_b32(rs1, voff, row, 0));
        else
            r[(j + M) % M] = (v2f){__uint_as_float(__builtin_amdgcn_raw_buffer_load_b32(rs1, voff, row, 0)),
                                   __uint_as_float(__builtin_amdgcn_raw_buffer_load_b32(rs2, voff, row, 0))};
    }
    const unsigned row_b = (unsigned)bd.px * 4u;
    unsigned qoff = (unsigned)(R + kPrefetch) * trow_b;
    unsigned woff = 0;
    auto step = [&](int s, auto reflecting, int y) __attribute__((always_inline)) {
        float n1, n2 = 0.f;
        if constexpr (decltype(reflecting)::value) {
            const unsigned rnext = (unsigned)reflect_once(y + R + kPrefetch, n) * trow_b;
            n1 = __uint_as_float(__builtin_amdgcn_raw_buffer_load_b32(rs1, voff, rnext, 0));
            if constexpr (!Q16) n2 = __uint_as_float(__builtin_amdgcn_raw_buffer_load_b32(rs2, voff, rnext, 0));
        } else {
            n1 = __uint_as_float(__builtin_amdgcn_raw_buffer_load_b32(rs1, voff, qoff, 0));
            if constexpr (!Q16) n2 = __uint_as_float(__builtin_amdgcn_raw_buffer_load_b32(rs2, voff, qoff, 0));
        }
        qoff += trow_b;
        v2f a2 = r[s] * taps.w[0];
        v2f b2 = (r[(s - 1 + M) % M] + r[(s + 1) % M]) * taps.w[1];
#pragma unroll
        for (int k = 2; k <= R; k += 2) {
            const v2f sa = r[(s - k + M) % M] + r[(s + k) % M];
            a2 = __builtin_elementwise_fma(sa, taps.w[k], a2);
            if (k + 1 <= R) {
                const v2f sb = r[(s - k - 1 + M) % M] + r[(s + k + 1) % M];
                b2 = __builtin_elementwise_fma(sb, taps.w[k + 1], b2);
            }
        }
        a2 += b2;
        const float acc = a2.x + a2.y;
        const unsigned long long ab = MASK ? __ballot(real & (acc > nms_lo)) : ~0ull;
        if (ab && real) __builtin_amdgcn_raw_buffer_store_b32(__float_as_uint(acc), rsw, ooff, woff, 0);
        woff += row_b;
        if constexpr (Q16) r[(s + R + kPrefetch) % M] = unpack(__float_as_uint(n1));
        else r[(s + R + kPrefetch) % M] = (v2f){n1, n2};
        if constexpr (MASK) {
            float nbx = -INFINITY;
            if (ab) {
                const float l = __uint_as_float((unsigned)__builtin_amdgcn_update_dpp(
                    (int)__float_as_uint(acc), (int)__float_as_uint(acc), 0x111 , 0xf, 0xf, false));
                const float rr = __uint_as_float((unsigned)__builtin_amdgcn_update_dpp(
                    (int)__float_as_uint(acc), (int)__float_as_uint(acc), 0x101 , 0xf, 0xf, false));
                nbx = fmaxf(has_l ? l : -INFINITY, has_r ? rr : -INFINITY);
            }
            if (ydone > 0) {
                unsigned long long m = 0;
                if (ab_prev) {
                    const bool cand = real & (prev1 > nms_lo) &
                                      !(fmaxf(fmaxf(prev2, acc), nbx_prev) > prev1 + nms_eps);
                    m = __ballot(cand);
                }
                if (lane == 0) *mrow = make_ulonglong2(m, ab_prev);
                mrow += nent;
            }
            prev2 = prev1; prev1 = acc; nbx_prev = nbx;
            ab_prev = ab;
            ++ydone;
        }
        __builtin_amdgcn_sched_barrier(0);
    };
    int y0 = 0;
#pragma unroll 1
    for (; y0 + M + R + kPrefetch <= n; y0 += M) {
#pragma unroll
        for (int s = 0; s < M; ++s) step(s, std::false_type{}, 0);
    }
#pragma unroll 1
    for (; y0 < n; y0 += M) {
#pragma unroll
        for (int s = 0; s < M; ++s) {
            if (y0 + s >= n) break;
            step(s, std::true_type{}, y0 + s);
        }
    }
    if constexpr (MASK) {
        const bool cand = real & (prev1 > nms_lo) & !(fmaxf(prev2, nbx_prev) > prev1 + nms_eps);
        const unsigned long long m = __ballot(cand);
        if (lane == 0) *mrow = make_ulonglong2(m, ab_prev);
    }
}

template <int R>
int launch_y6(const mmx_block* d_blocks, int n_blocks, const mmx_zx6_plan& plan, int64_t slot_elems,
              const mmx_taps_f32& taps, const float* d_p, const float* d_q, float cp, float cq, float* d_log,
              unsigned long long* d_mask, float nms_lo, float nms_eps, hipStream_t s)
{
    dim3 grid(plan.max_tiles, n_blocks);
    y2_taps pk;
    const bool q16 = cp > 0.f;
    for (int k = 0; k <= R; ++k) pk.w[k] = q16 ? (v2f){taps.w2[k] * cp, taps.w0[k] * cq} : (v2f){taps.w2[k], taps.w0[k]};
#define MMX_Y6_LAUNCH(MK, QQ) \
    hipLaunchKernelGGL((y6_kernel<R, MK, QQ>), grid, dim3(MMX_WG), 0, s, d_blocks, slot_elems, plan.tile_stride, d_p, d_q, \
                       d_log, pk, d_mask, nms_lo, nms_eps)
    if (d_mask) { if (q16) MMX_Y6_LAUNCH(true, true); else MMX_Y6_LAUNCH(true, false); }
    else        { if (q16) MMX_Y6_LAUNCH(false, true); else MMX_Y6_LAUNCH(false, false); }
#undef MMX_Y6_LAUNCH
    return hipGetLastError() == hipSuccess ? MMX_OK : MMX_ERR_HIP;
}

}

#define MMX_FOR_EACH_RADIUS(X) \
    X(1) X(2) X(3) X(4) X(5) X(6) X(7) X(8) X(9) X(10) X(11) X(12) X(13) X(14) X(15) X(16) \
    X(17) X(18) X(19) X(20) X(21) X(22) X(23) X(24)

int mmx_launch_y2(const mmx_block* d_blocks, int n_blocks, int max_cols, int64_t slot_elems,
                  const mmx_taps_f32& taps, int radius, const float* d_p, const float* d_q,
                  float* d_log, unsigned long long* d_mask, float nms_lo, float nms_eps, hipStream_t stream)
{
    switch (radius) {
#define X(R) case R: return launch_y2<R>(d_blocks, n_blocks, max_cols, slot_elems, taps, d_p, d_q, d_log, d_mask, nms_lo, nms_eps, stream);
        MMX_FOR_EACH_RADIUS(X)
#undef X
        default: return MMX_ERR_UNSUPPORTED;
    }
}

int mmx_launch_y6(const mmx_block* d_blocks, int n_blocks, const mmx_zx6_plan& plan, int64_t slot_elems,
                  const mmx_taps_f32& taps, int radius, const float* d_p, const float* d_q, float cp, float cq,
                  float* d_log, unsigned long long* d_mask, float nms_lo, float nms_eps, hipStream_t stream)
{
    switch (radius) {
#define X(R) case R: return launch_y6<R>(d_blocks, n_blocks, plan, slot_elems, taps, d_p, d_q, cp, cq, d_log, d_mask, nms_lo, nms_eps, stream);
        MMX_FOR_EACH_RADIUS(X)
#undef X
        default: return MMX_ERR_UNSUPPORTED;
    }
}
```

### magellanmapper_amd/csrc/mmx_peaks.hip

```cpp

#include "mmx_common.h"

namespace {

constexpr int kSigmaChunk = 8;

struct peak_ctx {
    const float* base;
    int64_t sigma_stride;
    int ns, nz, ny, nx, px, plane, slot;
    float thr, eps;
    mmx_cand* out;
    uint32_t cap;
    uint32_t* count;
};

__device__ __forceinline__ void check_voxel(const peak_ctx& c, int s, int idx, float v)
{
    const int z = idx / c.plane;
    const int rem = idx - z * c.plane;
    const int y = rem / c.px;
    const int x = rem - y * c.px;
    const int nz = c.nz, ny = c.ny, nx = c.nx, px = c.px, plane = c.plane;
    const float reject = v + c.eps;
    float m = -INFINITY;
    bool border = false;
    const float* ps = c.base + (int64_t)s * c.sigma_stride;
    if (x > 0) m = fmaxf(m, ps[idx - 1]); else border = true;
    if (x + 1 < nx) m = fmaxf(m, ps[idx + 1]); else border = true;
    if (y > 0) m = fmaxf(m, ps[idx - px]); else border = true;
    if (y + 1 < ny) m = fmaxf(m, ps[idx + px]); else border = true;
    if (z > 0) m = fmaxf(m, ps[idx - plane]); else border = true;
    if (z + 1 < nz) m = fmaxf(m, ps[idx + plane]); else border = true;
    if (m > reject) return;
    for (int ds = -1; ds <= 1; ++ds) {
        const int ss = s + ds;
        if (ss < 0 || ss >= c.ns) { border = true; continue; }
        const float* pss = c.base + (int64_t)ss * c.sigma_stride;
        for (int dz = -1; dz <= 1; ++dz) {
            const int zz = z + dz;
            if (zz < 0 || zz >= nz) continue;
            for (int dy = -1; dy <= 1; ++dy) {
                const int yy = y + dy;
                if (yy < 0 || yy >= ny) continue;
                const int row = zz * plane + yy * px;
#pragma unroll
                for (int dx = -1; dx <= 1; ++dx) {
                    const int xx = x + dx;
                    if (xx < 0 || xx >= nx) continue;
                    if ((ds | dz | dy | dx) == 0) continue;
                    m = fmaxf(m, pss[row + xx]);
                }
            }
            if (m > reject) return;
        }
    }
    if (border) m = fmaxf(m, 0.0f);
    if (!(v >= m - c.eps)) return;
    const bool contested = !(v > m + c.eps) || !(v > c.thr + c.eps);
    const uint32_t pos = atomicAdd(c.count, 1u);
    if (pos < c.cap) {
        mmx_cand r;
        r.slot = c.slot;
        r.s = s;
        r.z = z;
        r.y = y;
        r.x = x;
        r.flags = contested ? MMX_CAND_CONTESTED : 0u;
        r.v = v;
        r.nbr_max = m;
        r.v64 = __longlong_as_double(0x7ff8000000000000LL);
        r.band = 0;
        c.out[pos] = r;
    }
}

__global__ void __launch_bounds__(MMX_WG)
peaks_kernel(const float* __restrict__ log, int ns, int64_t sigma_stride,
             const mmx_block* __restrict__ blocks, int64_t slot_elems, float thr, float eps,
             mmx_cand* __restrict__ out, uint32_t cap, uint32_t* __restrict__ count)
{
    const mmx_block bd = blocks[blockIdx.y];
    peak_ctx c;
    c.base = log + (int64_t)bd.slot * slot_elems;
    c.sigma_stride = sigma_stride;
    c.ns = ns; c.nz = bd.nz; c.ny = bd.ny; c.nx = bd.nx; c.px = bd.px;
    c.plane = bd.ny * bd.px; c.slot = bd.slot;
    c.thr = thr; c.eps = eps; c.out = out; c.cap = cap; c.count = count;
    const int nquads = bd.nz * c.plane / 4;
    const float lo = thr - eps;
    const int qrow = bd.px / 4;

    for (int q = blockIdx.x * MMX_WG + threadIdx.x; q < nquads; q += gridDim.x * MMX_WG) {
        const int x0 = (q % qrow) * 4;
        if (x0 >= bd.nx) continue;
        const float4* p = reinterpret_cast<const float4*>(c.base) + q;
        const int64_t sstride4 = sigma_stride / 4;
        const int lane = threadIdx.x & 63;
        const bool has_left = x0 > 0 && lane > 0;
        const bool has_right = x0 + 4 < bd.nx && lane < 63 && q + 1 < nquads;
        const bool ok1 = x0 + 1 < bd.nx, ok2 = x0 + 2 < bd.nx, ok3 = x0 + 3 < bd.nx;
        for (int s0 = 0; s0 < ns; s0 += kSigmaChunk) {
            float e0[kSigmaChunk + 2], e1[kSigmaChunk + 2], e2[kSigmaChunk + 2], e3[kSigmaChunk + 2];
#pragma unroll
            for (int k = 0; k < kSigmaChunk + 2; ++k) {
                const int s = s0 + k - 1;
                float4 v = make_float4(-INFINITY, -INFINITY, -INFINITY, -INFINITY);
                if (s >= 0 && s < ns) v = p[(int64_t)s * sstride4];
                e0[k] = v.x;
                e1[k] = ok1 ? v.y : -INFINITY;
                e2[k] = ok2 ? v.z : -INFINITY;
                e3[k] = ok3 ? v.w : -INFINITY;
            }
            unsigned hits = 0;
#pragma unroll
            for (int k = 1; k <= kSigmaChunk; ++k) {
                if (s0 + k - 1 < ns) {
                    float lft = __shfl_up(e3[k], 1);
                    float rgt = __shfl_down(e0[k], 1);
                    lft = has_left ? lft : -INFINITY;
                    rgt = has_right ? rgt : -INFINITY;
                    const float n0 = fmaxf(fmaxf(lft, e1[k]), fmaxf(e0[k - 1], e0[k + 1]));
                    const float n1 = fmaxf(fmaxf(e0[k], e2[k]), fmaxf(e1[k - 1], e1[k + 1]));
                    const float n2 = fmaxf(fmaxf(e1[k], e3[k]), fmaxf(e2[k - 1], e2[k + 1]));
                    const float n3 = fmaxf(fmaxf(e2[k], rgt), fmaxf(e3[k - 1], e3[k + 1]));
                    const unsigned sh = 4 * (k - 1);
                    hits |= ((e0[k] > lo && !(n0 > e0[k] + eps)) ? 1u : 0u) << sh;
                    hits |= ((e1[k] > lo && !(n1 > e1[k] + eps)) ? 2u : 0u) << sh;
                    hits |= ((e2[k] > lo && !(n2 > e2[k] + eps)) ? 4u : 0u) << sh;
                    hits |= ((e3[k] > lo && !(n3 > e3[k] + eps)) ? 8u : 0u) << sh;
                }
            }
            while (hits) {
                const int b = __ffs(hits) - 1;
                hits &= hits - 1;
                const int j = b & 3;
                if (x0 + j >= bd.nx) continue;
                const int s = s0 + (b >> 2);
                const int idx = 4 * q + j;
                check_voxel(c, s, idx, c.base[(int64_t)s * sigma_stride + idx]);
            }
        }
    }
}

struct sparse_ctx {
    peak_ctx c;
    const ulonglong2* ent;
    int64_t ent_sigma_stride;
    int nwords;
    int quads, ntx;
};

__device__ __forceinline__ int64_t sparse_entry(const sparse_ctx& k, int z, int y, int x)
{
    return (int64_t)y * k.nwords + (k.quads ? (z >> 2) * k.ntx + (x >> 4) : (z * k.c.px + x) >> 6);
}

__device__ __forceinline__ float sparse_at(const sparse_ctx& k, int s, int z, int y, int x)
{
    const unsigned long long above = k.ent[(int64_t)s * k.ent_sigma_stride + sparse_entry(k, z, y, x)].y;
    if (!above) return -INFINITY;
    return k.c.base[(int64_t)s * k.c.sigma_stride + (int64_t)z * k.c.plane + y * k.c.px + x];
}

__device__ __forceinline__ void check_voxel_sparse(const sparse_ctx& k, int s, int z, int y, int x, float v)
{
    const peak_ctx& c = k.c;
    const int nz = c.nz, ny = c.ny, nx = c.nx;
    const float reject = v + c.eps;
    const float band_lo = v - c.eps;
    float m = -INFINITY;
    bool border = false;
    unsigned long long band = 0;
    unsigned band_hi = 0;
    for (int ds = -1; ds <= 1; ++ds) {
        const int ss = s + ds;
        if (ss < 0 || ss >= c.ns) { border = true; continue; }
        for (int dz = -1; dz <= 1; ++dz) {
            const int zz = z + dz;
            if (zz < 0 || zz >= nz) { border = true; continue; }
            for (int dy = -1; dy <= 1; ++dy) {
                const int yy = y + dy;
                if (yy < 0 || yy >= ny) { border = true; continue; }
                const ulonglong2* er = k.ent + (int64_t)ss * k.ent_sigma_stride;
                const float* row = c.base + (int64_t)ss * c.sigma_stride + (int64_t)zz * c.plane + yy * c.px;
#pragma unroll
                for (int dx = -1; dx <= 1; ++dx) {
                    const int xx = x + dx;
                    if (xx < 0 || xx >= nx) { border = true; continue; }
                    if ((ds | dz | dy | dx) == 0) continue;
                    if (er[sparse_entry(k, zz, yy, xx)].y) {
                        const float u = row[xx];
                        m = fmaxf(m, u);
                        if (u >= band_lo) {
                            int j = (((ds + 1) * 3 + (dz + 1)) * 3 + (dy + 1)) * 3 + (dx + 1);
                            j -= j > 40;
                            if (j < 64) band |= 1ull << j;
                            else band_hi |= 1u << (j - 64);
                        }
                    }
                }
            }
            if (m > reject) return;
        }
    }
    if (border) m = fmaxf(m, 0.0f);
    if (!(v >= m - c.eps)) return;
    const bool contested = !(v > m + c.eps) || !(v > c.thr + c.eps);
    const uint32_t pos = atomicAdd(c.count, 1u);
    if (pos < c.cap) {
        mmx_cand r;
        r.slot = c.slot;
        r.s = s;
        r.z = z;
        r.y = y;
        r.x = x;
        r.flags = (contested ? MMX_CAND_CONTESTED : 0u) | MMX_CAND_BAND | (band_hi << 16);
        r.v = v;
        r.nbr_max = m;
        r.v64 = __longlong_as_double(0x7ff8000000000000LL);
        r.band = band;
        c.out[pos] = r;
    }
}

__global__ void __launch_bounds__(MMX_WG)
peaks_sparse_kernel(const float* __restrict__ log, const ulonglong2* __restrict__ entries,
                    int ns, int64_t sigma_stride, const mmx_block* __restrict__ blocks, int64_t slot_elems,
                    float thr, float eps, mmx_cand* __restrict__ out, uint32_t cap,
                    uint32_t* __restrict__ count, int quads)
{
    const mmx_block bd = blocks[blockIdx.y];
    sparse_ctx k;
    peak_ctx& c = k.c;
    c.base = log + (int64_t)bd.slot * slot_elems;
    c.sigma_stride = sigma_stride;
    c.ns = ns; c.nz = bd.nz; c.ny = bd.ny; c.nx = bd.nx; c.px = bd.px;
    c.plane = bd.ny * bd.px; c.slot = bd.slot;
    c.thr = thr; c.eps = eps; c.out = out; c.cap = cap; c.count = count;
    const int ncol = bd.nz * bd.px;
    k.quads = quads;
    k.ntx = (bd.nx + 15) >> 4;
    k.nwords = quads ? ((bd.nz + 3) >> 2) * k.ntx : (ncol + 63) >> 6;
    k.ent = entries + ((int64_t)bd.slot * slot_elems >> 5);
    k.ent_sigma_stride = sigma_stride >> 5;
    const int64_t per_sigma = (int64_t)bd.ny * k.nwords;
    const int64_t total = per_sigma * ns;
    constexpr int kQ = 1024;
    __shared__ unsigned long long q[kQ];
    __shared__ int qn;
    auto test_bit = [&](int64_t i, int b) __attribute__((always_inline)) {
        const int s = (int)(i / per_sigma);
        const int64_t r = i - (int64_t)s * per_sigma;
        const int y = (int)(r / k.nwords);
        const int w = (int)(r - (int64_t)y * k.nwords);
        int z, x;
        if (k.quads) {
            const int zqi = w / k.ntx;
            z = 4 * zqi + (b >> 4);
            x = 16 * (w - zqi * k.ntx) + (b & 15);
        } else {
            const int col = (w << 6) + b;
            z = col / bd.px;
            x = col - z * bd.px;
        }
        if (x >= bd.nx || z >= bd.nz) return;
        const float v = c.base[(int64_t)s * sigma_stride + (int64_t)z * c.plane + y * bd.px + x];
        const float n0 = z > 0 ? sparse_at(k, s, z - 1, y, x) : -INFINITY;
        const float n1 = z + 1 < bd.nz ? sparse_at(k, s, z + 1, y, x) : -INFINITY;
        const float n2 = s > 0 ? sparse_at(k, s - 1, z, y, x) : -INFINITY;
        const float n3 = s + 1 < ns ? sparse_at(k, s + 1, z, y, x) : -INFINITY;
        if (fmaxf(fmaxf(n0, n1), fmaxf(n2, n3)) > v + eps) return;
        check_voxel_sparse(k, s, z, y, x, v);
    };
    if (threadIdx.x == 0) qn = 0;
    for (int j = threadIdx.x; j < kQ; j += MMX_WG) q[j] = ~0ull;
    __syncthreads();
    constexpr int kW = 8;
    const int64_t stride = (int64_t)gridDim.x * MMX_WG * kW;
    const int64_t rounds = (total + stride - 1) / stride;
    for (int64_t rd = 0; rd < rounds; ++rd) {
        const int64_t i0 = rd * stride + (int64_t)blockIdx.x * MMX_WG * kW + threadIdx.x;
        unsigned long long mw[kW];
#pragma unroll
        for (int u = 0; u < kW; ++u) {
            const int64_t i = i0 + (int64_t)u * MMX_WG;
            mw[u] = 0;
            if (i < total) {
                const int s = (int)(i / per_sigma);
                mw[u] = k.ent[(int64_t)s * k.ent_sigma_stride + (i - (int64_t)s * per_sigma)].x;
            }
        }
#pragma unroll
        for (int u = 0; u < kW; ++u) {
            unsigned long long m = mw[u];
            if (!m) continue;
            const int64_t i = i0 + (int64_t)u * MMX_WG;
            const int cnt = __popcll(m);
            const int at = atomicAdd(&qn, cnt);
            if (at + cnt <= kQ) {
                int j = at;
                while (m) {
                    const int b = __ffsll((long long)m) - 1;
                    m &= m - 1;
                    q[j++] = ((unsigned long long)i << 6) | (unsigned long long)b;
                }
            } else {
                while (m) {
                    const int b = __ffsll((long long)m) - 1;
                    m &= m - 1;
                    test_bit(i, b);
                }
            }
        }
        __syncthreads();
        const int nq = qn < kQ ? qn : kQ;
        for (int j = threadIdx.x; j < nq; j += MMX_WG) {
            const unsigned long long e = q[j];
            if (e != ~0ull) test_bit((int64_t)(e >> 6), (int)(e & 63));
        }
        __syncthreads();
        if (threadIdx.x == 0) qn = 0;
        for (int j = threadIdx.x; j < nq; j += MMX_WG) q[j] = ~0ull;
        __syncthreads();
    }
}

}

int mmx_launch_peaks_sparse(const float* d_log, const unsigned long long* d_mask, int n_sigma,
                            int64_t sigma_stride, const mmx_block* d_blocks, int n_blocks, int max_vox,
                            int64_t slot_elems, float thr, float eps, mmx_cand* d_cands, uint32_t cap,
                            uint32_t* d_count, int quads, hipStream_t stream)
{
    int64_t words = ((int64_t)max_vox / 64 + 1024) * n_sigma;
    int gx = (int)((words + MMX_WG * 8 - 1) / (MMX_WG * 8));
    if (gx > 8192) gx = 8192;
    if (gx < 1) gx = 1;
    dim3 grid(gx, n_blocks);
    hipLaunchKernelGGL(peaks_sparse_kernel, grid, dim3(MMX_WG), 0, stream, d_log,
                       reinterpret_cast<const ulonglong2*>(d_mask), n_sigma, sigma_stride,
                       d_blocks, slot_elems, thr, eps, d_cands, cap, d_count, quads);
    return hipGetLastError() == hipSuccess ? MMX_OK : MMX_ERR_HIP;
}

int mmx_launch_peaks(const float* d_log, int n_sigma, int64_t sigma_stride, const mmx_block* d_blocks,
                     int n_blocks, int max_vox, int64_t slot_elems, float thr, float eps,
                     mmx_cand* d_cands, uint32_t cap, uint32_t* d_count, hipStream_t stream)
{
    int gx = (max_vox / 4 + MMX_WG - 1) / MMX_WG;
    if (gx > 8192) gx = 8192;
    if (gx < 1) gx = 1;
    dim3 grid(gx, n_blocks);
    hipLaunchKernelGGL(peaks_kernel, grid, dim3(MMX_WG), 0, stream, d_log, n_sigma, sigma_stride,
                       d_blocks, slot_elems, thr, eps, d_cands, cap, d_count);
    return hipGetLastError() == hipSuccess ? MMX_OK : MMX_ERR_HIP;
}
```

### magellanmapper_amd/csrc/mmx_ymfma.hip

```cpp

#include <type_traits>

#include <cstdlib>

#include "mmx_common.h"

typedef _Float16 h2_y __attribute__((ext_vector_type(2)));
typedef _Float16 h8_y __attribute__((ext_vector_type(8)));
typedef float f2_y __attribute__((ext_vector_type(2)));
typedef float f4_y __attribute__((ext_vector_type(4)));
typedef unsigned u4_y __attribute__((ext_vector_type(4)));

struct ym_cfg {
    float w2[MMX_MAX_RADIUS_FAST + 1];
    float w0[MMX_MAX_RADIUS_FAST + 1];
    float unscale;
    float start;
    float lo, eps;
    int radius;
    int reverse;
};

namespace {

using rsrc_y = __amdgpu_buffer_rsrc_t;
__device__ __forceinline__ rsrc_y make_rsrc_y(const void* p)
{
    return __builtin_amdgcn_make_buffer_rsrc(const_cast<void*>(p), 0, 0x7fffffff, 0x00020000);
}
__device__ __forceinline__ unsigned pack_h2y(float a, float b)
{
    const f2_y v = {a, b};
    return __builtin_bit_cast(unsigned, __builtin_convertvector(v, h2_y));
}
__device__ __forceinline__ f4_y mfma_y(const u4_y& a, const u4_y& b, const f4_y& c)
{
    return __builtin_amdgcn_mfma_f32_16x16x32_f16(__builtin_bit_cast(h8_y, a), __builtin_bit_cast(h8_y, b), c, 0, 0, 0);
}

#ifndef YM5_OCC
#define YM5_OCC 2
#endif
#ifndef YM6_WAVES
#define YM6_WAVES 4
#define YM6_JH 4
#define YM6_NF 4
#endif
template <int NB, bool MASK>
__global__ void __launch_bounds__(NB <= 4 ? 256 : YM6_WAVES * 64, NB <= 4 ? 3 : (YM6_WAVES == 4 ? YM5_OCC : 1))
ym_kernel(const mmx_block* __restrict__ blocks, int64_t slot_elems, int64_t tile_stride,
          const unsigned* __restrict__ gt, float* __restrict__ out, ym_cfg cfg,
          unsigned long long* __restrict__ mask)
{
    constexpr int RB = 8 * (NB - 2);
    constexpr int NF = NB <= 4 ? 4 : YM6_NF;
    __shared__ u4_y frag[NB * NF * 64];
    constexpr int WAVES = NB <= 4 ? 4 : YM6_WAVES;
    constexpr int JH = NB <= 4 ? 4 : YM6_JH;
    __shared__ float tr[WAVES * 2 * 1024];

    const mmx_block bd = blocks[cfg.reverse ? gridDim.y - 1 - blockIdx.y : blockIdx.y];
    const int ntx = (bd.nx + 15) >> 4, ntz = (bd.nz + 15) >> 4;
    if ((int)blockIdx.x * (WAVES / 4) >= ntx * ntz) return;
    for (int e = threadIdx.x; e < NB * NF * 64; e += WAVES * 64) {
        const int ln = e & 63, f = e >> 6;
        const int piece = (f % NF) % (NF / 2), kern = (f % NF) / (NF / 2), t = f / NF;
        const int m = ln & 15, kq = ln >> 4;
        const int delta = RB - 16 * t;
        unsigned pk[4];
#pragma unroll
        for (int i = 0; i < 8; i += 2) {
            float v[2];
#pragma unroll
            for (int u = 0; u < 2; ++u) {
                int d = 8 * kq + i + u - m + delta;
                d = d < 0 ? -d : d;
                const float ws = d <= cfg.radius ? (kern ? cfg.w0[d] : cfg.w2[d]) : 0.f;
                const float h = (float)(_Float16)ws;
                v[u] = piece == 0 ? h : (piece == 1 ? (ws - h) * 256.f : h * 256.f);
            }
            pk[i >> 1] = pack_h2y(v[0], v[1]);
        }
        frag[e] = (u4_y){pk[0], pk[1], pk[2], pk[3]};
    }
    __syncthreads();

    const int wv = __builtin_amdgcn_readfirstlane((int)(threadIdx.x >> 6));
    const int tile = (int)blockIdx.x * (WAVES / 4) + (wv >> 2);
    if (tile >= ntx * ntz) return;
    const int c = tile / ntz, U = tile - c * ntz;
    const int zq = wv & 3;
    if (16 * U + 4 * zq >= bd.nz) return;
    const int lane = threadIdx.x & 63;
    const int n = bd.ny;
    const float nms_lo = cfg.lo, nms_eps = cfg.eps, us = cfg.unscale;
    const int kq = lane >> 4, n16 = lane & 15;
    const unsigned trow_b = (unsigned)(ntx * ntz) * 1024u;
    const rsrc_y rs = make_rsrc_y(gt + (int64_t)bd.slot * tile_stride + (int64_t)tile * 256);
    const unsigned voff = (unsigned)(zq * 256 + n16 * 16);
    const unsigned voff_s = voff + (unsigned)(8 * kq) * trow_b;
    const int xi = lane & 15;
    const int z = 16 * U + 4 * zq + (lane >> 4), x = 16 * c + xi;
    const bool real = z < bd.nz && x < bd.nx;
    float* w1 = out + (int64_t)bd.slot * slot_elems;
    const rsrc_y rsw = make_rsrc_y(w1);
    const unsigned ooff = (unsigned)((real ? z : 0) * bd.ny * bd.px + (real ? x : 0)) * 4u;
    const unsigned row_b = (unsigned)bd.px * 4u;
    const int nent = ((bd.nz + 3) >> 2) * ntx;
    ulonglong2* mrow = MASK ? reinterpret_cast<ulonglong2*>(mask) + ((int64_t)bd.slot * slot_elems >> 5) +
                              (4 * U + zq) * ntx + c
                            : nullptr;
    unsigned long long ab_prev = 0;
    const bool has_l = xi > 0, has_r = xi < 15 && x + 1 < bd.nx;
    float prev1 = -INFINITY, prev2 = -INFINITY, nbx_prev = -INFINITY;
    int ydone = 0;
    float* trw = tr + wv * 2048;

    auto row = [&](float acc, int y) __attribute__((always_inline)) {
        const unsigned long long ab = MASK ? __ballot(real & (acc > nms_lo)) : ~0ull;
#ifndef YM_NOSTORE
        if (ab && real) __builtin_amdgcn_raw_buffer_store_b32(__float_as_uint(acc * us), rsw, ooff, (unsigned)y * row_b, 0);
#endif
        if constexpr (MASK) {
            float nbx = -INFINITY;
            if (ab) {
                const float l = __uint_as_float((unsigned)__builtin_amdgcn_update_dpp(
                    (int)__float_as_uint(acc), (int)__float_as_uint(acc), 0x111 , 0xf, 0xf, false));
                const float rr = __uint_as_float((unsigned)__builtin_amdgcn_update_dpp(
                    (int)__float_as_uint(acc), (int)__float_as_uint(acc), 0x101 , 0xf, 0xf, false));
                nbx = fmaxf(has_l ? l : -INFINITY, has_r ? rr : -INFINITY);
            }
            if (ydone > 0) {
                unsigned long long m = 0;
                if (ab_prev) {
                    const bool cand = real & (prev1 > nms_lo) &
                                      !(fmaxf(fmaxf(prev2, acc), nbx_prev) > prev1 + nms_eps);
                    m = __ballot(cand);
                }
                if (lane == 0) *mrow = make_ulonglong2(m, ab_prev);
                mrow += nent;
            }
            prev2 = prev1; prev1 = acc; nbx_prev = nbx;
            ab_prev = ab;
            ++ydone;
        }
    };
    auto rows_of = [&](int T, int s, bool any) __attribute__((always_inline)) {
        if (T < 0 || 16 * T >= n) return;
        const int cnt = n - 16 * T < 16 ? n - 16 * T : 16;
        if (MASK && !any) {
            if (ydone > 0) {
                unsigned long long m = 0;
                if (ab_prev) {
                    const bool cand = real & (prev1 > nms_lo) & !(fmaxf(prev2, nbx_prev) > prev1 + nms_eps);
                    m = __ballot(cand);
                }
                if (lane == 0) *mrow = make_ulonglong2(m, ab_prev);
                mrow += nent;
            }
            if (lane < cnt - 1) mrow[(int64_t)lane * nent] = make_ulonglong2(0ull, 0ull);
            mrow += (int64_t)(cnt - 1) * nent;
            prev1 = prev2 = nbx_prev = -INFINITY;
            ab_prev = 0;
            ydone += cnt;
            return;
        }
        const float* src = trw + s * 1024 + lane;
        if (!MASK || cnt < 16) {
#pragma unroll 1
            for (int r = 0; r < cnt; ++r) row(src[r * 64], 16 * T + r);
            return;
        }
        float v[16];
#pragma unroll
        for (int r = 0; r < 16; ++r) v[r] = src[r * 64];
        unsigned long long ab[16];
        unsigned long long some = 0;
#pragma unroll
        for (int r = 0; r < 16; ++r) { ab[r] = __ballot(real & (v[r] > nms_lo)); some |= ab[r]; }
        unsigned e0 = 0, e1 = 0, e2 = 0, e3 = 0;
        auto put = [&](int ln, unsigned long long m, unsigned long long a) __attribute__((always_inline)) {
            const bool me = lane == ln;
            e0 = me ? (unsigned)m : e0;
            e1 = me ? (unsigned)(m >> 32) : e1;
            e2 = me ? (unsigned)a : e2;
            e3 = me ? (unsigned)(a >> 32) : e3;
        };
        if (ab_prev) {
            const bool cand = real & (prev1 > nms_lo) & !(fmaxf(fmaxf(prev2, v[0]), nbx_prev) > prev1 + nms_eps);
            put(0, __ballot(cand), ab_prev);
        }
        float nbx15 = -INFINITY;
        if (some) {
#pragma unroll
            for (int r = 0; r < 16; ++r) {
                if (ab[r]) {
#ifndef YM_NOSTORE
                    if (real) __builtin_amdgcn_raw_buffer_store_b32(__float_as_uint(v[r] * us), rsw, ooff, (unsigned)(16 * T + r) * row_b, 0);
#endif
                    const float l = __uint_as_float((unsigned)__builtin_amdgcn_update_dpp(
                        (int)__float_as_uint(v[r]), (int)__float_as_uint(v[r]), 0x111 , 0xf, 0xf, false));
                    const float rr = __uint_as_float((unsigned)__builtin_amdgcn_update_dpp(
                        (int)__float_as_uint(v[r]), (int)__float_as_uint(v[r]), 0x101 , 0xf, 0xf, false));
                    const float nbx = fmaxf(has_l ? l : -INFINITY, has_r ? rr : -INFINITY);
                    if (r < 15) {
                        const float below = r > 0 ? v[r > 0 ? r - 1 : 0] : prev1;
                        const bool cand = real & (v[r] > nms_lo) & !(fmaxf(fmaxf(below, v[r < 15 ? r + 1 : 15]), nbx) > v[r] + nms_eps);
                        put(r + 1, __ballot(cand), ab[r]);
                    } else {
                        nbx15 = nbx;
                    }
                }
            }
        }
        if (lane < 16 && (lane > 0 || ydone > 0)) {
            ulonglong2* dst = mrow + (int64_t)(ydone > 0 ? lane : lane - 1) * nent;
            *dst = make_ulonglong2((unsigned long long)e0 | ((unsigned long long)e1 << 32),
                                   (unsigned long long)e2 | ((unsigned long long)e3 << 32));
        }
        mrow += (int64_t)(ydone > 0 ? 16 : 15) * nent;
        prev2 = v[14]; prev1 = v[15]; nbx_prev = nbx15;
        ab_prev = ab[15];
        ydone += 16;
    };

#ifndef YM_PFD
#define YM_PFD 1
#endif
    constexpr int PFD = YM_PFD;
    u4_y rawA[8], rawB[PFD == 2 ? 8 : 1];
    auto load_block = [&](int b, u4_y (&raw)[8]) __attribute__((always_inline)) {
        const int r0 = -RB + 32 * b;
        if (r0 >= 0 && r0 + 32 <= n) {
#pragma unroll
            for (int i = 0; i < 8; ++i)
                raw[i] = __builtin_bit_cast(u4_y, __builtin_amdgcn_raw_buffer_load_b128(rs, voff_s, (unsigned)(r0 + i) * trow_b, 0));
        } else {
#pragma unroll
            for (int i = 0; i < 8; ++i) {
                int v = r0 + 8 * kq + i;
                v = v < 0 ? -1 - v : v;
                v = v >= n ? 2 * n - 1 - v : v;
                v = v < 0 ? 0 : (v > n - 1 ? n - 1 : v);
                raw[i] = __builtin_bit_cast(u4_y, __builtin_amdgcn_raw_buffer_load_b128(rs, voff + (unsigned)v * trow_b, 0, 0));
            }
        }
    };
    const int nT = (n + 15) >> 4;
    const int nKB = (nT + NB - 3) / 2 + 1;
    const f4_y start = {cfg.start, cfg.start, cfg.start, cfg.start};
    f4_y acc[NB][4];
#pragma unroll
    for (int t = 0; t < NB; ++t)
#pragma unroll
        for (int j = 0; j < 4; ++j) acc[t][j] = start;
    bool any0 = false, any1 = false;

    const _Float16 k256 = (_Float16)256.f;
    auto iter = [&](int b, u4_y (&raw)[8]) __attribute__((always_inline)) {
#ifndef YM_ROWS_LATE
#define YM_ROWS_LATE 1
#endif
        if (!YM_ROWS_LATE || b == nKB) {
#pragma unroll 1
            for (int h = 0; h < 2; ++h) rows_of(2 * (b - 1) - NB + 2 + h, h, h ? any1 : any0);
        }
        if (b == nKB) return false;
        if constexpr (JH < 4) { any0 = !MASK; any1 = !MASK; }
#pragma unroll
        for (int j0 = 0; j0 < 4; j0 += JH) {
            __builtin_amdgcn_sched_barrier(0);
            u4_y pc[JH][4];
#pragma unroll
            for (int j = 0; j < JH; ++j)
#pragma unroll
                for (int p = 0; p < 4; ++p) {
                    const unsigned d0 = raw[2 * p][j0 + j], d1 = raw[2 * p + 1][j0 + j];
                    pc[j][0][p] = __builtin_amdgcn_perm(d1, d0, 0x0c050c01u);
                    pc[j][1][p] = __builtin_amdgcn_perm(d1, d0, 0x0c040c00u);
                    pc[j][2][p] = __builtin_amdgcn_perm(d1, d0, 0x0c070c03u) ^ 0x00800080u;
                    pc[j][3][p] = __builtin_amdgcn_perm(d1, d0, 0x0c060c02u);
                }
            __builtin_amdgcn_sched_barrier(0);
            if (j0 + JH == 4 && b + PFD < nKB) load_block(b + PFD, raw);
            __builtin_amdgcn_sched_barrier(0);
            if (YM_ROWS_LATE && JH == 4) {
#pragma unroll 1
                for (int h = 0; h < 2; ++h) rows_of(2 * (b - 1) - NB + 2 + h, h, h ? any1 : any0);
                __builtin_amdgcn_sched_barrier(0);
            }
            auto tile_mfmas = [&](int t, bool fresh) __attribute__((always_inline)) {
                f4_y* a = &acc[t][j0];
                const u4_y* fr = frag + (t * NF) * 64 + lane;
                const u4_y ah = fr[0], al = fr[64], bh = fr[(NF / 2) * 64], bl = fr[(NF / 2 + 1) * 64];
                const u4_y a256 = NF == 6 ? fr[128] : __builtin_bit_cast(u4_y, __builtin_bit_cast(h8_y, ah) * k256);
                const u4_y b256 = NF == 6 ? fr[320] : __builtin_bit_cast(u4_y, __builtin_bit_cast(h8_y, bh) * k256);
#pragma unroll
                for (int j = 0; j < JH; ++j) a[j] = mfma_y(a256, pc[j][0], fresh ? start : a[j]);
#pragma unroll
                for (int j = 0; j < JH; ++j) a[j] = mfma_y(ah, pc[j][1], a[j]);
#pragma unroll
                for (int j = 0; j < JH; ++j) a[j] = mfma_y(al, pc[j][0], a[j]);
#pragma unroll
                for (int j = 0; j < JH; ++j) a[j] = mfma_y(b256, pc[j][2], a[j]);
#pragma unroll
                for (int j = 0; j < JH; ++j) a[j] = mfma_y(bh, pc[j][3], a[j]);
#pragma unroll
                for (int j = 0; j < JH; ++j) a[j] = mfma_y(bl, pc[j][2], a[j]);
            };
#pragma unroll
            for (int t = 0; t < 2; ++t) tile_mfmas(t, t >= NB - 2);
#pragma unroll
            for (int t = 0; t < 2; ++t) {
                const f4_y* a = &acc[t][j0];
                float mx = -INFINITY;
#pragma unroll
                for (int j = 0; j < JH; ++j)
#pragma unroll
                    for (int r = 0; r < 4; ++r) mx = fmaxf(mx, a[j][r]);
                const bool any = MASK ? __ballot(mx > nms_lo) != 0ull : true;
                if constexpr (JH == 4) {
                    if (t == 0) any0 = any; else any1 = any;
                    if (any) {
                        f4_y* dst = reinterpret_cast<f4_y*>(trw + t * 1024) + (4 * kq) * 16 + n16;
#pragma unroll
                        for (int r = 0; r < 4; ++r) dst[r * 16] = (f4_y){a[0][r], a[1][r], a[2][r], a[3][r]};
                    }
                } else {
                    if (t == 0) any0 |= any; else any1 |= any;
                    f2_y* dst = reinterpret_cast<f2_y*>(trw + t * 1024) + (4 * kq) * 32 + 2 * n16 + (j0 >> 1);
#pragma unroll
                    for (int r = 0; r < 4; ++r) dst[r * 32] = (f2_y){a[0][r], a[1][r]};
                }
            }
            __builtin_amdgcn_sched_barrier(0);
#pragma unroll
            for (int t = 2; t < NB; ++t) {
                tile_mfmas(t, t >= NB - 2);
                if constexpr (NB > 4) __builtin_amdgcn_sched_barrier(0);
            }
        }
#pragma unroll
        for (int t = 0; t + 2 < NB; ++t)
#pragma unroll
            for (int j = 0; j < 4; ++j) acc[t][j] = acc[t + 2][j];
        __builtin_amdgcn_wave_barrier();
        return true;
    };
    load_block(0, rawA);
    if constexpr (PFD == 2) {
        if (nKB > 1) load_block(1, reinterpret_cast<u4_y (&)[8]>(rawB));
#pragma unroll 1
        for (int b = 0;; b += 2) {
            if (!iter(b, rawA)) break;
            if (!iter(b + 1, reinterpret_cast<u4_y (&)[8]>(rawB))) break;
        }
    } else {
#pragma unroll 1
        for (int b = 0; iter(b, rawA); ++b) {}
    }
    if constexpr (MASK) {
        unsigned long long m = 0;
        if (ab_prev) {
            const bool cand = real & (prev1 > nms_lo) & !(fmaxf(prev2, nbx_prev) > prev1 + nms_eps);
            m = __ballot(cand);
        }
        if (lane == 0) *mrow = make_ulonglong2(m, ab_prev);
    }
}

template <int NB>
int launch_ym(const mmx_block* d_blocks, int n_blocks, const mmx_zx6_plan& plan, int64_t slot_elems,
              const ym_cfg& cfg, const float* d_p, float* d_log, unsigned long long* d_mask, hipStream_t s)
{
    constexpr int TPW = NB <= 4 ? 1 : YM6_WAVES / 4;
    dim3 grid((plan.max_tiles + TPW - 1) / TPW, n_blocks);
    if (d_mask)
        hipLaunchKernelGGL((ym_kernel<NB, true>), grid, dim3(256 * TPW), 0, s, d_blocks, slot_elems, plan.tile_stride,
                           reinterpret_cast<const unsigned*>(d_p), d_log, cfg, d_mask);
    else
        hipLaunchKernelGGL((ym_kernel<NB, false>), grid, dim3(256 * TPW), 0, s, d_blocks, slot_elems, plan.tile_stride,
                           reinterpret_cast<const unsigned*>(d_p), d_log, cfg, d_mask);
    return hipGetLastError() == hipSuccess ? MMX_OK : MMX_ERR_HIP;
}

}

int mmx_launch_ym(const mmx_block* d_blocks, int n_blocks, const mmx_zx6_plan& plan, int64_t slot_elems,
                  const mmx_taps_f32& taps, int radius, const float* d_p, float cp, float cq,
                  float* d_log, unsigned long long* d_mask, float nms_lo, float nms_eps, hipStream_t stream)
{
    if (radius < 1 || radius > 24 || radius > MMX_MAX_RADIUS_FAST || !(cp > 0.f) || !(cq > 0.f)) return MMX_ERR_UNSUPPORTED;
    ym_cfg cfg;
    float mx = 0.f;
    for (int k = 0; k <= radius; ++k) {
        cfg.w2[k] = taps.w2[k] * cp;
        cfg.w0[k] = taps.w0[k] * cq;
        mx = fmaxf(mx, fmaxf(fabsf(cfg.w2[k]), fabsf(cfg.w0[k])));
    }
    if (!(mx > 1e-30f) || !(mx < 1e30f)) return MMX_ERR_UNSUPPORTED;
    int e;
    frexpf(mx, &e);
    const float up = ldexpf(1.f, -e - 1);
    double q128 = 0.0;
    for (int k = 0; k <= MMX_MAX_RADIUS_FAST; ++k) {
        cfg.w2[k] = k <= radius ? cfg.w2[k] * up : 0.f;
        cfg.w0[k] = k <= radius ? cfg.w0[k] * up : 0.f;
        const float h = (float)(_Float16)cfg.w0[k];
        const float l = (float)(_Float16)((cfg.w0[k] - h) * 256.f);
        q128 += (k ? 2.0 : 1.0) * ((double)h * 256.0 + (double)l);
    }
    cfg.start = (float)(-128.0 * 0x1p-24 * q128);
    cfg.unscale = ldexpf(1.f, e + 1 + 24);
    cfg.lo = nms_lo / cfg.unscale;
    cfg.eps = nms_eps / cfg.unscale;
    cfg.radius = radius;
    cfg.reverse = 1;
    if (radius <= 8) return launch_ym<3>(d_blocks, n_blocks, plan, slot_elems, cfg, d_p, d_log, d_mask, stream);
    if (radius <= 16) return launch_ym<4>(d_blocks, n_blocks, plan, slot_elems, cfg, d_p, d_log, d_mask, stream);
    return launch_ym<5>(d_blocks, n_blocks, plan, slot_elems, cfg, d_p, d_log, d_mask, stream);
}
```

Before: 44200.

## Emit compacted list of nonzero NMS mask entries for sparse peak pass

The y-pass kernels now append the index of every nonzero NMS mask entry to a global candidate list, using a wave-aggregated atomic push. A new list-driven peaks kernel then visits only those entries instead of scanning every mask word. The sparse-scan kernel stays as a fallback that runs only when the list overflows. The cost is extra atomics and stores inside the y-pass, more workspace, and an extra launch.

```diff
diff --git a/include/mmx.h b/include/mmx.h
--- a/include/mmx.h
+++ b/include/mmx.h
@@ -8,7 +8,7 @@
 extern "C" {
 #endif
 
-#define MMX_ABI_VERSION 19
+#define MMX_ABI_VERSION 20
 
 typedef enum {
     MMX_OK = 0,
@@ -126,7 +126,8 @@
     uint32_t* d_count;
     uint32_t* h_count;
     mmx_cand* h_cands;
-    int32_t zx_mode, zx_flags, store_f32, exact, expand, _pad;
+    int32_t zx_mode, zx_flags, store_f32, exact, expand;
+    uint32_t list_cap;
     void* stream; void* tail_stream; void* pack_stream;
     void* ev_work_free; void* ev_work_read; void* ev_done;
 } mmx_detect_args;
diff --git a/magellanmapper_amd/_native.py b/magellanmapper_amd/_native.py
--- a/magellanmapper_amd/_native.py
+++ b/magellanmapper_amd/_native.py
@@ -10,7 +10,7 @@
 _HERE = os.path.dirname(os.path.abspath(__file__))
 LIB_PATH = os.environ.get("MMX_LIB_PATH") or os.path.join(_HERE, "libmmx_hip.so")
 
-MMX_ABI_VERSION = 19
+MMX_ABI_VERSION = 20
 MMX_U8, MMX_U16, MMX_F32, MMX_F64 = 0, 1, 2, 3
 MMX_MAX_RADIUS_FAST = 24
 MMX_MAX_RADIUS_GENERIC = 255
@@ -60,7 +60,7 @@
                 ("thr", c_float), ("eps", c_float), ("d_cands", c_void_p), ("cap", c_uint32), ("h_prefix", c_uint32),
                 ("d_count", c_void_p), ("h_count", c_void_p), ("h_cands", c_void_p),
                 ("zx_mode", c_int32), ("zx_flags", c_int32), ("store_f32", c_int32), ("exact", c_int32),
-                ("expand", c_int32), ("_pad", c_int32),
+                ("expand", c_int32), ("list_cap", c_uint32),
                 ("stream", c_void_p), ("tail_stream", c_void_p), ("pack_stream", c_void_p),
                 ("ev_work_free", c_void_p), ("ev_work_read", c_void_p), ("ev_done", c_void_p)]
 
diff --git a/magellanmapper_amd/csrc/mmx_api.hip b/magellanmapper_amd/csrc/mmx_api.hip
--- a/magellanmapper_amd/csrc/mmx_api.hip
+++ b/magellanmapper_amd/csrc/mmx_api.hip
@@ -15,7 +15,11 @@
 int mmx_launch_peaks_sparse(const float* d_log, const unsigned long long* d_mask, int n_sigma,
                             int64_t sigma_stride, const mmx_block* d_blocks, int n_blocks, int max_vox,
                             int64_t slot_elems, float thr, float eps, mmx_cand* d_cands, uint32_t cap,
-                            uint32_t* d_count, int quads, hipStream_t stream);
+                            uint32_t* d_count, int quads, const uint32_t* d_run_if, hipStream_t stream);
+int mmx_launch_peaks_list(const float* d_log, const unsigned long long* d_mask, int n_sigma,
+                          int64_t sigma_stride, const mmx_block* d_blocks, int n_blocks, int max_vox,
+                          int64_t slot_elems, float thr, float eps, mmx_cand* d_cands, uint32_t cap,
+                          uint32_t* d_count, int quads, const mmx_cand_list& list, hipStream_t stream);
 
 #include <mutex>
 #include <vector>
@@ -113,6 +117,7 @@
     if (with_masks) {
         bytes = (bytes + 15) & ~(size_t)15;
         bytes += (size_t)n_sigma * (((size_t)n_blocks * (size_t)slot_elems) >> 5) * 16;
+        bytes += MMX_LIST_HEAD_BYTES + (size_t)mmx_list_capacity(n_blocks, slot_elems, n_sigma) * sizeof(uint64_t);
     }
     return bytes;
 }
@@ -174,6 +179,13 @@
     return err;
 }
 
+}
+
+uint32_t mmx_list_capacity(int n_blocks, int64_t slot_elems, int n_sigma)
+{
+    const uint64_t entries = (uint64_t)n_sigma * (((uint64_t)n_blocks * (uint64_t)slot_elems) >> 5);
+    const uint64_t cap = entries / MMX_LIST_DIV;
+    return (uint32_t)(cap < 1024 ? 1024 : (cap > 0x7fffffffull ? 0x7fffffffull : cap));
 }
 
 void mmx_batch_geom_make(const mmx_volume* vol, const mmx_block* h_blocks, int n_blocks, int64_t slot_elems,
@@ -315,19 +327,20 @@
         mmx_timed_scope ts(MMX_K_Y2, s);
         const bool want_mask = wants_entries && (tiled ? g.quads_fit : g.rows_fit);
         unsigned long long* d_mask = want_mask ? (unsigned long long*)c.d_nms_mask : nullptr;
+        const mmx_cand_list list = want_mask ? c.list : mmx_cand_list{};
         rc = MMX_ERR_UNSUPPORTED;
         if (tiled && q16 && !y_valu)
             rc = mmx_launch_ym(c.d_blocks, n_blocks, plan, slot_elems, tyy, radius, c.d_work,
-                               (float)(q_bp / 65535.0), (float)(q_bq / 32767.0), c.d_log, d_mask, c.nms_lo, c.nms_eps, s);
+                               (float)(q_bp / 65535.0), (float)(q_bq / 32767.0), c.d_log, d_mask, c.nms_lo, c.nms_eps, list, s);
         if (rc != MMX_ERR_UNSUPPORTED) ;
         else if (tiled)
             rc = mmx_launch_y6(c.d_blocks, n_blocks, plan, slot_elems, tyy, radius, c.d_work,
                                reinterpret_cast<const float*>(reinterpret_cast<const char*>(c.d_work) + plan.q_off),
                                q16 ? (float)(q_bp / 65535.0) : 0.f, q16 ? (float)(q_bq / 32767.0) : 0.f, c.d_log,
-                               d_mask, c.nms_lo, c.nms_eps, s);
+                               d_mask, c.nms_lo, c.nms_eps, list, s);
         else
             rc = mmx_launch_y2(c.d_blocks, n_blocks, g.max_ycols, slot_elems, tyy, radius, t0, t1, c.d_log,
-                               d_mask, c.nms_lo, c.nms_eps, s);
+                               d_mask, c.nms_lo, c.nms_eps, list, s);
         if (rc == MMX_OK && want_mask) *c.h_mask_written = tiled ? MMX_MASK_QUADS : MMX_MASK_ROWS;
     }
     return rc == MMX_ERR_HIP ? hip_fail(hipGetLastError(), "fused passes") : rc;
@@ -449,6 +462,17 @@
                     float thr, float eps, mmx_cand* d_cands, uint32_t cap,
                     uint32_t* d_count, void* stream)
 {
+    return mmx_peaks_batch_list(d_log, d_nms_mask, mask_layout, n_sigma, d_blocks, h_blocks, n_blocks, slot_elems, thr, eps,
+                                d_cands, cap, d_count, mmx_cand_list{}, (hipStream_t)stream);
+}
+
+}
+
+int mmx_peaks_batch_list(const float* d_log, const uint64_t* d_nms_mask, int mask_layout, int n_sigma, const mmx_block* d_blocks,
+                         const mmx_block* h_blocks, int n_blocks, int64_t slot_elems,
+                         float thr, float eps, mmx_cand* d_cands, uint32_t cap,
+                         uint32_t* d_count, const mmx_cand_list& list, hipStream_t stream)
+{
     if (!d_log || !d_blocks || !h_blocks || !d_cands || !d_count) return MMX_ERR_ARG;
     if (n_sigma < 1 || n_blocks < 1 || slot_elems < 1 || !(eps >= 0.f)) return MMX_ERR_ARG;
     if (n_blocks > MMX_MAX_BLOCKS) return MMX_ERR_UNSUPPORTED;
@@ -460,15 +484,21 @@
     const int max_vox = g.max_vox;
     mmx_timed_scope ts(MMX_K_PEAKS, (hipStream_t)stream);
     int rc;
-    if (d_nms_mask)
+    if (d_nms_mask && list.head)
+        rc = mmx_launch_peaks_list(d_log, (const unsigned long long*)d_nms_mask, n_sigma,
+                                   (int64_t)n_blocks * slot_elems, d_blocks, n_blocks, max_vox, slot_elems,
+                                   thr, eps, d_cands, cap, d_count, mask_layout == MMX_MASK_QUADS, list, (hipStream_t)stream);
+    else if (d_nms_mask)
         rc = mmx_launch_peaks_sparse(d_log, (const unsigned long long*)d_nms_mask, n_sigma,
                                      (int64_t)n_blocks * slot_elems, d_blocks, n_blocks, max_vox, slot_elems,
-                                     thr, eps, d_cands, cap, d_count, mask_layout == MMX_MASK_QUADS, (hipStream_t)stream);
+                                     thr, eps, d_cands, cap, d_count, mask_layout == MMX_MASK_QUADS, nullptr, (hipStream_t)stream);
     else
         rc = mmx_launch_peaks(d_log, n_sigma, (int64_t)n_blocks * slot_elems, d_blocks, n_blocks, max_vox,
                               slot_elems, thr, eps, d_cands, cap, d_count, (hipStream_t)stream);
     return rc == MMX_ERR_HIP ? hip_fail(hipGetLastError(), "peaks") : rc;
 }
+
+extern "C" {
 
 int mmx_copy_rect_h2d(void* d_dst, size_t dpitch, const void* h_src, size_t spitch, size_t width, size_t height,
                       void* stream)
diff --git a/magellanmapper_amd/csrc/mmx_common.h b/magellanmapper_amd/csrc/mmx_common.h
--- a/magellanmapper_amd/csrc/mmx_common.h
+++ b/magellanmapper_amd/csrc/mmx_common.h
@@ -21,6 +21,42 @@
     if (i < 0) i += period;
     return i < n ? i : period - 1 - i;
 }
+
+#define MMX_LIST_HEAD_BYTES 16
+#define MMX_LIST_MAX_SIGMA 256
+#define MMX_LIST_DIV 16
+struct mmx_cand_list {
+    uint32_t* head;
+    uint32_t cap;
+    uint32_t sigma;
+};
+__host__ __device__ __forceinline__ unsigned long long* mmx_list_items(const mmx_cand_list& l)
+{
+    return reinterpret_cast<unsigned long long*>(l.head + MMX_LIST_HEAD_BYTES / sizeof(uint32_t));
+}
+uint32_t mmx_list_capacity(int n_blocks, int64_t slot_elems, int n_sigma);
+
+#ifdef __HIPCC__
+__device__ __forceinline__ void mmx_list_push(const mmx_cand_list& l, bool nz, unsigned long long item)
+{
+    const unsigned long long b = __ballot(nz);
+    if (!b) return;
+    const int lane = (int)__builtin_amdgcn_mbcnt_hi(~0u, __builtin_amdgcn_mbcnt_lo(~0u, 0u));
+    const int leader = __ffsll((long long)__ballot(true)) - 1;
+    uint32_t base = 0;
+    if (lane == leader) base = atomicAdd(l.head, (uint32_t)__popcll(b));
+    base = (uint32_t)__builtin_amdgcn_readfirstlane((int)base);
+    if (nz) {
+        const uint32_t pos = base + (uint32_t)__popcll(b & ((1ull << lane) - 1ull));
+        if (pos < l.cap) mmx_list_items(l)[pos] = item;
+        else l.head[1] = 1u;
+    }
+}
+__device__ __forceinline__ unsigned long long mmx_list_item(uint32_t sigma, int slot, int64_t entry)
+{
+    return ((unsigned long long)sigma << 40) | ((unsigned long long)(uint32_t)slot << 24) | (unsigned long long)entry;
+}
+#endif
 
 int mmx_launch_zpass(const mmx_volume* vol, const mmx_block* d_blocks, int n_blocks, int max_cols,
                      int64_t slot_elems, const mmx_taps_f32& taps, int radius,
@@ -51,13 +87,16 @@
                    hipStream_t stream);
 int mmx_launch_y6(const mmx_block* d_blocks, int n_blocks, const mmx_zx6_plan& plan, int64_t slot_elems,
                   const mmx_taps_f32& taps, int radius, const float* d_p, const float* d_q, float cp, float cq,
-                  float* d_log, unsigned long long* d_mask, float nms_lo, float nms_eps, hipStream_t stream);
+                  float* d_log, unsigned long long* d_mask, float nms_lo, float nms_eps, const mmx_cand_list& list,
+                  hipStream_t stream);
 int mmx_launch_ym(const mmx_block* d_blocks, int n_blocks, const mmx_zx6_plan& plan, int64_t slot_elems,
                   const mmx_taps_f32& taps, int radius, const float* d_p, float cp, float cq,
-                  float* d_log, unsigned long long* d_mask, float nms_lo, float nms_eps, hipStream_t stream);
+                  float* d_log, unsigned long long* d_mask, float nms_lo, float nms_eps, const mmx_cand_list& list,
+                  hipStream_t stream);
 int mmx_launch_y2(const mmx_block* d_blocks, int n_blocks, int max_cols, int64_t slot_elems,
                   const mmx_taps_f32& taps, int radius, const float* d_p, const float* d_q,
-                  float* d_log, unsigned long long* d_mask, float nms_lo, float nms_eps, hipStream_t stream);
+                  float* d_log, unsigned long long* d_mask, float nms_lo, float nms_eps, const mmx_cand_list& list,
+                  hipStream_t stream);
 
 struct mmx_batch_geom {
     int status;
@@ -76,8 +115,12 @@
     const double* h_w0; const double* h_w2; int radius; double norm;
     float* d_log; float* d_work; uint64_t* d_nms_mask; float nms_lo, nms_eps; int* h_mask_written;
     int zx_mode; int* h_zx_path; hipStream_t stream;
+    mmx_cand_list list;
 };
 int mmx_log_scale_f32(const mmx_log_call& c, const mmx_batch_geom& g);
+int mmx_peaks_batch_list(const float* d_log, const uint64_t* d_nms_mask, int mask_layout, int n_sigma, const mmx_block* d_blocks,
+                         const mmx_block* h_blocks, int n_blocks, int64_t slot_elems, float thr, float eps, mmx_cand* d_cands,
+                         uint32_t cap, uint32_t* d_count, const mmx_cand_list& list, hipStream_t stream);
 int mmx_zx_pack_geom(const mmx_volume* vol, const mmx_block* d_blocks, const mmx_block* h_blocks, int n_blocks,
                      int64_t slot_elems, const mmx_batch_geom& g, float* d_work, hipStream_t stream);
 
diff --git a/magellanmapper_amd/csrc/mmx_detect.hip b/magellanmapper_amd/csrc/mmx_detect.hip
--- a/magellanmapper_amd/csrc/mmx_detect.hip
+++ b/magellanmapper_amd/csrc/mmx_detect.hip
@@ -57,8 +57,19 @@
     return reinterpret_cast<uint64_t*>((reinterpret_cast<uintptr_t>(end) + 15) & ~(uintptr_t)15);
 }
 
+mmx_cand_list cand_list(const mmx_detect_args* a)
+{
+    mmx_cand_list l{};
+    if (a->n_sigma > MMX_LIST_MAX_SIGMA) return l;
+    uint64_t* at = nms_entries(a) + (size_t)a->n_sigma * (((size_t)a->n_blocks * a->slot_elems) >> 5) * 2;
+    l.head = reinterpret_cast<uint32_t*>(at);
+    l.cap = mmx_list_capacity(a->n_blocks, a->slot_elems, a->n_sigma);
+    if (a->list_cap && a->list_cap < l.cap) l.cap = a->list_cap;
+    return l;
+}
+
 int passes(const mmx_detect_args* a, const mmx_batch_geom& g, bool with_mask, int mode, unsigned* layouts, int* zx_path,
-           double* q16_bound, bool* pack_side)
+           double* q16_bound, bool* pack_side, const mmx_cand_list& list)
 {
     *layouts = 0;
     const mmx_volume* vol = a->vol32;
@@ -83,6 +94,10 @@
     }
     bool packed = false;
     hipStream_t main = (hipStream_t)a->stream;
+    if (with_mask && list.head) {
+        hipError_t r = hipMemsetAsync(list.head, 0, MMX_LIST_HEAD_BYTES, main);
+        if (r != hipSuccess) return fail(r, "reset of the candidate list");
+    }
     if (((mode == MMX_ZX_AUTO || mode == MMX_ZX_TILED || mode == MMX_ZX_TILED_Q16) && !is_float) ||
         ((mode == MMX_ZX_AUTO || mode == MMX_ZX_TILED) && float_ok)) {
         hipStream_t ps = (*pack_side && a->pack_stream) ? (hipStream_t)a->pack_stream : main;
@@ -97,11 +112,13 @@
     }
     for (int s = 0; s < ns; ++s) {
         int written = 0, path = 0;
+        mmx_cand_list ls = with_mask ? list : mmx_cand_list{};
+        ls.sigma = (uint32_t)s;
         const int rc = mmx_log_scale_f32({vol, a->d_blocks, a->h_blocks, nb, slot, a->h_w0 + s * tab, a->h_w2 + s * tab,
                                           a->h_radius[s], a->h_norm[s], d_log + (size_t)s * nb * slot, a->d_work,
                                           with_mask ? d_mask + (size_t)s * mask_words * 2 : nullptr, a->thr - a->eps, a->eps,
                                           &written, packed ? (tiled_mode | MMX_ZX_PREPACKED | a->zx_flags) : mode, &path,
-                                          main}, g);
+                                          main, ls}, g);
         if (rc != MMX_OK) return rc;
         *zx_path = path;
         packed = packed && path == tiled_mode;
@@ -126,7 +143,7 @@
 
 const char* mmx_detect_last_error(void) { return g_detect_err; }
 
-int mmx_log_scales_f32(const mmx_detect_args* a, mmx_detect_info* info)
+static int log_scales(const mmx_detect_args* a, mmx_detect_info* info, bool with_list)
 {
     if (!a || !info) return MMX_ERR_ARG;
     memset(info, 0, sizeof *info);
@@ -143,19 +160,20 @@
     }
     mmx_batch_geom g;
     mmx_batch_geom_make(a->vol32, a->h_blocks, a->n_blocks, a->slot_elems, &g);
+    const mmx_cand_list list = with_list ? cand_list(a) : mmx_cand_list{};
 
     unsigned layouts = 0;
     int zx_path = 0;
     double q16_bound = 0.0;
-    int rc = passes(a, g, true, a->zx_mode, &layouts, &zx_path, &q16_bound, &pack_side);
+    int rc = passes(a, g, true, a->zx_mode, &layouts, &zx_path, &q16_bound, &pack_side, list);
     if (rc != MMX_OK) return rc;
     if (layouts == ((1u << MMX_MASK_ROWS) | (1u << MMX_MASK_QUADS))) {
-        rc = passes(a, g, true, MMX_ZX_PACKED, &layouts, &zx_path, &q16_bound, &pack_side);
+        rc = passes(a, g, true, MMX_ZX_PACKED, &layouts, &zx_path, &q16_bound, &pack_side, list);
         if (rc != MMX_OK) return rc;
         info->n_pass_rounds++;
     }
     if (layouts & (layouts - 1)) {
-        rc = passes(a, g, false, a->zx_mode, &layouts, &zx_path, &q16_bound, &pack_side);
+        rc = passes(a, g, false, a->zx_mode, &layouts, &zx_path, &q16_bound, &pack_side, list);
         if (rc != MMX_OK) return rc;
         info->n_pass_rounds++;
     }
@@ -168,13 +186,15 @@
     return MMX_OK;
 }
 
+int mmx_log_scales_f32(const mmx_detect_args* a, mmx_detect_info* info) { return log_scales(a, info, false); }
+
 int mmx_detect_batch(const mmx_detect_args* a, mmx_detect_info* info)
 {
     if (!a || !info) return MMX_ERR_ARG;
     memset(info, 0, sizeof *info);
     if (!a->d_cands || !a->d_count || a->cap < 1) return MMX_ERR_ARG;
     if (a->exact && (!a->vol_exact || !a->d_w0 || !a->d_w2)) return MMX_ERR_ARG;
-    int rc = mmx_log_scales_f32(a, info);
+    int rc = log_scales(a, info, true);
     if (rc != MMX_OK) return rc;
     const int nb = a->n_blocks, ns = a->n_sigma;
     hipStream_t main = (hipStream_t)a->stream;
@@ -185,8 +205,9 @@
     if (rc != MMX_OK) return rc;
     r = hipMemsetAsync(a->d_count, 0, 2 * sizeof(uint32_t), tail);
     if (r != hipSuccess) return fail(r, "reset of the candidate counters");
-    rc = mmx_peaks_batch(log_arrays(a), info->mask_layout ? nms_entries(a) : nullptr, info->mask_layout, ns, a->d_blocks, a->h_blocks,
-                         nb, a->slot_elems, a->thr, a->eps, a->d_cands, a->cap, a->d_count, (void*)tail);
+    rc = mmx_peaks_batch_list(log_arrays(a), info->mask_layout ? nms_entries(a) : nullptr, info->mask_layout, ns, a->d_blocks,
+                              a->h_blocks, nb, a->slot_elems, a->thr, a->eps, a->d_cands, a->cap, a->d_count,
+                              info->mask_layout ? cand_list(a) : mmx_cand_list{}, tail);
     if (rc != MMX_OK) return rc;
     if (a->ev_work_read) {
         r = hipEventRecord((hipEvent_t)a->ev_work_read, tail);
diff --git a/magellanmapper_amd/csrc/mmx_fused.hip b/magellanmapper_amd/csrc/mmx_fused.hip
--- a/magellanmapper_amd/csrc/mmx_fused.hip
+++ b/magellanmapper_amd/csrc/mmx_fused.hip
@@ -43,13 +43,19 @@
 struct y2_taps {
     v2f w[MMX_MAX_RADIUS_FAST + 1];
 };
+__device__ __forceinline__ void put_entry(ulonglong2* at, const ulonglong2* base, unsigned long long m,
+                                          unsigned long long above, int slot, const mmx_cand_list& list)
+{
+    *at = make_ulonglong2(m, above);
+    if (list.head && m) mmx_list_push(list, true, mmx_list_item(list.sigma, slot, at - base));
+}
 
 template <int R, bool MASK>
 __global__ void __launch_bounds__(MMX_WG)
 y2_kernel(const mmx_block* __restrict__ blocks, int64_t slot_elems,
           const float* __restrict__ gp, const float* __restrict__ gq,
           float* __restrict__ out, y2_taps taps,
-          unsigned long long* __restrict__ mask, float nms_lo, float nms_eps)
+          unsigned long long* __restrict__ mask, float nms_lo, float nms_eps, mmx_cand_list list)
 {
     using io = vox<float>;
     constexpr int N = 2 * R + 1;
@@ -70,8 +76,8 @@
 
     const int lane = threadIdx.x & 63;
     const int nwords = (ncol + 63) >> 6;
-    ulonglong2* mrow = MASK ? reinterpret_cast<ulonglong2*>(mask) + ((int64_t)bd.slot * slot_elems >> 5) + (col >> 6)
-                            : nullptr;
+    ulonglong2* const mbase = MASK ? reinterpret_cast<ulonglong2*>(mask) + ((int64_t)bd.slot * slot_elems >> 5) : nullptr;
+    ulonglong2* mrow = MASK ? mbase + (col >> 6) : nullptr;
     unsigned long long ab_prev = 0;
     const bool real = x < bd.nx;
     const bool has_l = lane > 0 && x > 0, has_r = lane < 63 && x + 1 < bd.nx && col + 1 < ncol;
@@ -126,7 +132,7 @@
                 const bool cand = real & (prev1 > nms_lo) &
                                   !(fmaxf(fmaxf(prev2, acc), nbx_prev) > prev1 + nms_eps);
                 const unsigned long long m = __ballot(cand);
-                if (lane == 0) *mrow = make_ulonglong2(m, ab_prev);
+                if (lane == 0) put_entry(mrow, mbase, m, ab_prev, bd.slot, list);
                 mrow += nwords;
             }
             prev2 = prev1; prev1 = acc; nbx_prev = nbx;
@@ -152,24 +158,24 @@
     if constexpr (MASK) {
         const bool cand = real & (prev1 > nms_lo) & !(fmaxf(prev2, nbx_prev) > prev1 + nms_eps);
         const unsigned long long m = __ballot(cand);
-        if (lane == 0) *mrow = make_ulonglong2(m, ab_prev);
+        if (lane == 0) put_entry(mrow, mbase, m, ab_prev, bd.slot, list);
     }
 }
 
 template <int R>
 int launch_y2(const mmx_block* d_blocks, int n_blocks, int max_cols, int64_t slot_elems,
               const mmx_taps_f32& taps, const float* d_p, const float* d_q, float* d_log,
-              unsigned long long* d_mask, float nms_lo, float nms_eps, hipStream_t s)
+              unsigned long long* d_mask, float nms_lo, float nms_eps, const mmx_cand_list& list, hipStream_t s)
 {
     dim3 grid((max_cols + MMX_WG - 1) / MMX_WG, n_blocks);
     y2_taps pk;
     for (int k = 0; k <= R; ++k) pk.w[k] = (v2f){taps.w2[k], taps.w0[k]};
     if (d_mask)
         hipLaunchKernelGGL((y2_kernel<R, true>), grid, dim3(MMX_WG), 0, s, d_blocks, slot_elems, d_p, d_q, d_log, pk,
-                           d_mask, nms_lo, nms_eps);
+                           d_mask, nms_lo, nms_eps, list);
     else
         hipLaunchKernelGGL((y2_kernel<R, false>), grid, dim3(MMX_WG), 0, s, d_blocks, slot_elems, d_p, d_q, d_log, pk,
-                           d_mask, nms_lo, nms_eps);
+                           d_mask, nms_lo, nms_eps, list);
     return hipGetLastError() == hipSuccess ? MMX_OK : MMX_ERR_HIP;
 }
 
@@ -178,7 +184,7 @@
 y6_kernel(const mmx_block* __restrict__ blocks, int64_t slot_elems, int64_t tile_stride,
           const float* __restrict__ gp, const float* __restrict__ gq,
           float* __restrict__ out, y2_taps taps,
-          unsigned long long* __restrict__ mask, float nms_lo, float nms_eps)
+          unsigned long long* __restrict__ mask, float nms_lo, float nms_eps, mmx_cand_list list)
 {
     constexpr int N = 2 * R + 1;
     constexpr int M = N + kPrefetch;
@@ -201,9 +207,8 @@
     const unsigned voff = (unsigned)(zq * 64 + lane) * 4u;
     const unsigned ooff = (unsigned)((real ? z : 0) * bd.ny * bd.px + (real ? x : 0)) * 4u;
     const int nent = ((bd.nz + 3) >> 2) * ntx;
-    ulonglong2* mrow = MASK ? reinterpret_cast<ulonglong2*>(mask) + ((int64_t)bd.slot * slot_elems >> 5) +
-                              (4 * U + zq) * ntx + c
-                            : nullptr;
+    ulonglong2* const mbase = MASK ? reinterpret_cast<ulonglong2*>(mask) + ((int64_t)bd.slot * slot_elems >> 5) : nullptr;
+    ulonglong2* mrow = MASK ? mbase + (4 * U + zq) * ntx + c : nullptr;
     unsigned long long ab_prev = 0;
     const bool has_l = xi > 0, has_r = xi < 15 && x + 1 < bd.nx;
     float prev1 = -INFINITY, prev2 = -INFINITY, nbx_prev = -INFINITY;
@@ -271,7 +276,7 @@
                                       !(fmaxf(fmaxf(prev2, acc), nbx_prev) > prev1 + nms_eps);
                     m = __ballot(cand);
                 }
-                if (lane == 0) *mrow = make_ulonglong2(m, ab_prev);
+                if (lane == 0) put_entry(mrow, mbase, m, ab_prev, bd.slot, list);
                 mrow += nent;
             }
             prev2 = prev1; prev1 = acc; nbx_prev = nbx;
@@ -297,14 +302,14 @@
     if constexpr (MASK) {
         const bool cand = real & (prev1 > nms_lo) & !(fmaxf(prev2, nbx_prev) > prev1 + nms_eps);
         const unsigned long long m = __ballot(cand);
-        if (lane == 0) *mrow = make_ulonglong2(m, ab_prev);
+        if (lane == 0) put_entry(mrow, mbase, m, ab_prev, bd.slot, list);
     }
 }
 
 template <int R>
 int launch_y6(const mmx_block* d_blocks, int n_blocks, const mmx_zx6_plan& plan, int64_t slot_elems,
               const mmx_taps_f32& taps, const float* d_p, const float* d_q, float cp, float cq, float* d_log,
-              unsigned long long* d_mask, float nms_lo, float nms_eps, hipStream_t s)
+              unsigned long long* d_mask, float nms_lo, float nms_eps, const mmx_cand_list& list, hipStream_t s)
 {
     dim3 grid(plan.max_tiles, n_blocks);
     y2_taps pk;
@@ -312,7 +317,7 @@
     for (int k = 0; k <= R; ++k) pk.w[k] = q16 ? (v2f){taps.w2[k] * cp, taps.w0[k] * cq} : (v2f){taps.w2[k], taps.w0[k]};
 #define MMX_Y6_LAUNCH(MK, QQ) \
     hipLaunchKernelGGL((y6_kernel<R, MK, QQ>), grid, dim3(MMX_WG), 0, s, d_blocks, slot_elems, plan.tile_stride, d_p, d_q, \
-                       d_log, pk, d_mask, nms_lo, nms_eps)
+                       d_log, pk, d_mask, nms_lo, nms_eps, list)
     if (d_mask) { if (q16) MMX_Y6_LAUNCH(true, true); else MMX_Y6_LAUNCH(true, false); }
     else        { if (q16) MMX_Y6_LAUNCH(false, true); else MMX_Y6_LAUNCH(false, false); }
 #undef MMX_Y6_LAUNCH
@@ -327,10 +332,11 @@
 
 int mmx_launch_y2(const mmx_block* d_blocks, int n_blocks, int max_cols, int64_t slot_elems,
                   const mmx_taps_f32& taps, int radius, const float* d_p, const float* d_q,
-                  float* d_log, unsigned long long* d_mask, float nms_lo, float nms_eps, hipStream_t stream)
+                  float* d_log, unsigned long long* d_mask, float nms_lo, float nms_eps, const mmx_cand_list& list,
+                  hipStream_t stream)
 {
     switch (radius) {
-#define X(R) case R: return launch_y2<R>(d_blocks, n_blocks, max_cols, slot_elems, taps, d_p, d_q, d_log, d_mask, nms_lo, nms_eps, stream);
+#define X(R) case R: return launch_y2<R>(d_blocks, n_blocks, max_cols, slot_elems, taps, d_p, d_q, d_log, d_mask, nms_lo, nms_eps, list, stream);
         MMX_FOR_EACH_RADIUS(X)
 #undef X
         default: return MMX_ERR_UNSUPPORTED;
@@ -339,10 +345,11 @@
 
 int mmx_launch_y6(const mmx_block* d_blocks, int n_blocks, const mmx_zx6_plan& plan, int64_t slot_elems,
                   const mmx_taps_f32& taps, int radius, const float* d_p, const float* d_q, float cp, float cq,
-                  float* d_log, unsigned long long* d_mask, float nms_lo, float nms_eps, hipStream_t stream)
+                  float* d_log, unsigned long long* d_mask, float nms_lo, float nms_eps, const mmx_cand_list& list,
+                  hipStream_t stream)
 {
     switch (radius) {
-#define X(R) case R: return launch_y6<R>(d_blocks, n_blocks, plan, slot_elems, taps, d_p, d_q, cp, cq, d_log, d_mask, nms_lo, nms_eps, stream);
+#define X(R) case R: return launch_y6<R>(d_blocks, n_blocks, plan, slot_elems, taps, d_p, d_q, cp, cq, d_log, d_mask, nms_lo, nms_eps, list, stream);
         MMX_FOR_EACH_RADIUS(X)
 #undef X
         default: return MMX_ERR_UNSUPPORTED;
diff --git a/magellanmapper_amd/csrc/mmx_peaks.hip b/magellanmapper_amd/csrc/mmx_peaks.hip
--- a/magellanmapper_amd/csrc/mmx_peaks.hip
+++ b/magellanmapper_amd/csrc/mmx_peaks.hip
@@ -1,5 +1,10 @@
 
 #include "mmx_common.h"
+
+int mmx_launch_peaks_sparse(const float* d_log, const unsigned long long* d_mask, int n_sigma,
+                            int64_t sigma_stride, const mmx_block* d_blocks, int n_blocks, int max_vox,
+                            int64_t slot_elems, float thr, float eps, mmx_cand* d_cands, uint32_t cap,
+                            uint32_t* d_count, int quads, const uint32_t* d_run_if, hipStream_t stream);
 
 namespace {
 
@@ -225,14 +230,10 @@
     }
 }
 
-__global__ void __launch_bounds__(MMX_WG)
-peaks_sparse_kernel(const float* __restrict__ log, const ulonglong2* __restrict__ entries,
-                    int ns, int64_t sigma_stride, const mmx_block* __restrict__ blocks, int64_t slot_elems,
-                    float thr, float eps, mmx_cand* __restrict__ out, uint32_t cap,
-                    uint32_t* __restrict__ count, int quads)
-{
-    const mmx_block bd = blocks[blockIdx.y];
-    sparse_ctx k;
+__device__ __forceinline__ void sparse_ctx_make(sparse_ctx& k, const mmx_block& bd, const float* log,
+                                                const ulonglong2* entries, int ns, int64_t sigma_stride, int64_t slot_elems,
+                                                float thr, float eps, mmx_cand* out, uint32_t cap, uint32_t* count, int quads)
+{
     peak_ctx& c = k.c;
     c.base = log + (int64_t)bd.slot * slot_elems;
     c.sigma_stride = sigma_stride;
@@ -245,6 +246,43 @@
     k.nwords = quads ? ((bd.nz + 3) >> 2) * k.ntx : (ncol + 63) >> 6;
     k.ent = entries + ((int64_t)bd.slot * slot_elems >> 5);
     k.ent_sigma_stride = sigma_stride >> 5;
+}
+
+__device__ __forceinline__ void test_set_bit(const sparse_ctx& k, int s, int64_t r, int b)
+{
+    const peak_ctx& c = k.c;
+    const int y = (int)(r / k.nwords);
+    const int w = (int)(r - (int64_t)y * k.nwords);
+    int z, x;
+    if (k.quads) {
+        const int zqi = w / k.ntx;
+        z = 4 * zqi + (b >> 4);
+        x = 16 * (w - zqi * k.ntx) + (b & 15);
+    } else {
+        const int col = (w << 6) + b;
+        z = col / c.px;
+        x = col - z * c.px;
+    }
+    if (x >= c.nx || z >= c.nz) return;
+    const float v = c.base[(int64_t)s * c.sigma_stride + (int64_t)z * c.plane + y * c.px + x];
+    const float n0 = z > 0 ? sparse_at(k, s, z - 1, y, x) : -INFINITY;
+    const float n1 = z + 1 < c.nz ? sparse_at(k, s, z + 1, y, x) : -INFINITY;
+    const float n2 = s > 0 ? sparse_at(k, s - 1, z, y, x) : -INFINITY;
+    const float n3 = s + 1 < c.ns ? sparse_at(k, s + 1, z, y, x) : -INFINITY;
+    if (fmaxf(fmaxf(n0, n1), fmaxf(n2, n3)) > v + c.eps) return;
+    check_voxel_sparse(k, s, z, y, x, v);
+}
+
+__global__ void __launch_bounds__(MMX_WG)
+peaks_sparse_kernel(const float* __restrict__ log, const ulonglong2* __restrict__ entries,
+                    int ns, int64_t sigma_stride, const mmx_block* __restrict__ blocks, int64_t slot_elems,
+                    float thr, float eps, mmx_cand* __restrict__ out, uint32_t cap,
+                    uint32_t* __restrict__ count, int quads, const uint32_t* __restrict__ run_if)
+{
+    if (run_if && !*run_if) return;
+    const mmx_block bd = blocks[blockIdx.y];
+    sparse_ctx k;
+    sparse_ctx_make(k, bd, log, entries, ns, sigma_stride, slot_elems, thr, eps, out, cap, count, quads);
     const int64_t per_sigma = (int64_t)bd.ny * k.nwords;
     const int64_t total = per_sigma * ns;
     constexpr int kQ = 1024;
@@ -252,27 +290,7 @@
     __shared__ int qn;
     auto test_bit = [&](int64_t i, int b) __attribute__((always_inline)) {
         const int s = (int)(i / per_sigma);
-        const int64_t r = i - (int64_t)s * per_sigma;
-        const int y = (int)(r / k.nwords);
-        const int w = (int)(r - (int64_t)y * k.nwords);
-        int z, x;
-        if (k.quads) {
-            const int zqi = w / k.ntx;
-            z = 4 * zqi + (b >> 4);
-            x = 16 * (w - zqi * k.ntx) + (b & 15);
-        } else {
-            const int col = (w << 6) + b;
-            z = col / bd.px;
-            x = col - z * bd.px;
-        }
-        if (x >= bd.nx || z >= bd.nz) return;
-        const float v = c.base[(int64_t)s * sigma_stride + (int64_t)z * c.plane + y * bd.px + x];
-        const float n0 = z > 0 ? sparse_at(k, s, z - 1, y, x) : -INFINITY;
-        const float n1 = z + 1 < bd.nz ? sparse_at(k, s, z + 1, y, x) : -INFINITY;
-        const float n2 = s > 0 ? sparse_at(k, s - 1, z, y, x) : -INFINITY;
-        const float n3 = s + 1 < ns ? sparse_at(k, s + 1, z, y, x) : -INFINITY;
-        if (fmaxf(fmaxf(n0, n1), fmaxf(n2, n3)) > v + eps) return;
-        check_voxel_sparse(k, s, z, y, x, v);
+        test_set_bit(k, s, i - (int64_t)s * per_sigma, b);
     };
     if (threadIdx.x == 0) qn = 0;
     for (int j = threadIdx.x; j < kQ; j += MMX_WG) q[j] = ~0ull;
@@ -327,12 +345,109 @@
     }
 }
 
+__global__ void __launch_bounds__(MMX_WG)
+peaks_list_kernel(const float* __restrict__ log, const ulonglong2* __restrict__ entries,
+                  int ns, int64_t sigma_stride, const mmx_block* __restrict__ blocks, int n_blocks, int64_t slot_elems,
+                  float thr, float eps, mmx_cand* __restrict__ out, uint32_t cap,
+                  uint32_t* __restrict__ count, int quads, const unsigned long long* __restrict__ items,
+                  uint32_t* __restrict__ head, uint32_t list_cap)
+{
+    if (blockIdx.x == 0 && threadIdx.x == 0) head[2] = list_cap;
+    if (head[1]) return;
+    const uint32_t n = head[0] < list_cap ? head[0] : list_cap;
+    constexpr int kQ = 1024;
+    __shared__ unsigned long long q[kQ];
+    __shared__ int qn;
+    auto ctx_of = [&](unsigned long long item, sparse_ctx& k, int& s, int64_t& r) __attribute__((always_inline)) {
+        s = (int)(item >> 40);
+        const int slot = (int)(item >> 24) & 0xffff;
+        r = (int64_t)(item & 0xffffffull);
+        if (s >= ns || slot >= n_blocks) return false;
+        sparse_ctx_make(k, blocks[slot], log, entries, ns, sigma_stride, slot_elems, thr, eps, out, cap, count, quads);
+        return r < (int64_t)k.c.ny * k.nwords;
+    };
+    auto test_bit = [&](unsigned long long item, int b) __attribute__((always_inline)) {
+        sparse_ctx k;
+        int s;
+        int64_t r;
+        if (ctx_of(item, k, s, r)) test_set_bit(k, s, r, b);
+    };
+    if (threadIdx.x == 0) qn = 0;
+    for (int j = threadIdx.x; j < kQ; j += MMX_WG) q[j] = ~0ull;
+    __syncthreads();
+    constexpr int kW = 2;
+    const uint32_t stride = gridDim.x * MMX_WG * kW;
+    for (uint32_t i0 = blockIdx.x * MMX_WG * kW; i0 < n; i0 += stride) {
+        unsigned long long it[kW], mw[kW];
+#pragma unroll
+        for (int u = 0; u < kW; ++u) {
+            const uint32_t i = i0 + (uint32_t)u * MMX_WG + threadIdx.x;
+            it[u] = 0;
+            mw[u] = 0;
+            if (i < n) {
+                it[u] = items[i];
+                sparse_ctx k;
+                int s;
+                int64_t r;
+                if (ctx_of(it[u], k, s, r)) mw[u] = k.ent[(int64_t)s * k.ent_sigma_stride + r].x;
+            }
+        }
+#pragma unroll
+        for (int u = 0; u < kW; ++u) {
+            unsigned long long m = mw[u];
+            if (!m) continue;
+            const int cnt = __popcll(m);
+            const int at = atomicAdd(&qn, cnt);
+            if (at + cnt <= kQ) {
+                int j = at;
+                while (m) {
+                    const int b = __ffsll((long long)m) - 1;
+                    m &= m - 1;
+                    q[j++] = (it[u] << 6) | (unsigned long long)b;
+                }
+            } else {
+                while (m) {
+                    const int b = __ffsll((long long)m) - 1;
+                    m &= m - 1;
+                    test_bit(it[u], b);
+                }
+            }
+        }
+        __syncthreads();
+        const int nq = qn < kQ ? qn : kQ;
+        for (int j = threadIdx.x; j < nq; j += MMX_WG) {
+            const unsigned long long e = q[j];
+            if (e != ~0ull) test_bit(e >> 6, (int)(e & 63));
+        }
+        __syncthreads();
+        if (threadIdx.x == 0) qn = 0;
+        for (int j = threadIdx.x; j < nq; j += MMX_WG) q[j] = ~0ull;
+        __syncthreads();
+    }
+}
+
+}
+
+int mmx_launch_peaks_list(const float* d_log, const unsigned long long* d_mask, int n_sigma,
+                          int64_t sigma_stride, const mmx_block* d_blocks, int n_blocks, int max_vox,
+                          int64_t slot_elems, float thr, float eps, mmx_cand* d_cands, uint32_t cap,
+                          uint32_t* d_count, int quads, const mmx_cand_list& list, hipStream_t stream)
+{
+    int gx = (int)(((int64_t)list.cap + MMX_WG * 2 - 1) / (MMX_WG * 2));
+    if (gx > 1024) gx = 1024;
+    if (gx < 1) gx = 1;
+    hipLaunchKernelGGL(peaks_list_kernel, dim3(gx), dim3(MMX_WG), 0, stream, d_log,
+                       reinterpret_cast<const ulonglong2*>(d_mask), n_sigma, sigma_stride, d_blocks, n_blocks,
+                       slot_elems, thr, eps, d_cands, cap, d_count, quads, mmx_list_items(list), list.head, list.cap);
+    if (hipGetLastError() != hipSuccess) return MMX_ERR_HIP;
+    return mmx_launch_peaks_sparse(d_log, d_mask, n_sigma, sigma_stride, d_blocks, n_blocks, max_vox, slot_elems, thr,
+                                   eps, d_cands, cap, d_count, quads, list.head + 1, stream);
 }
 
 int mmx_launch_peaks_sparse(const float* d_log, const unsigned long long* d_mask, int n_sigma,
                             int64_t sigma_stride, const mmx_block* d_blocks, int n_blocks, int max_vox,
                             int64_t slot_elems, float thr, float eps, mmx_cand* d_cands, uint32_t cap,
-                            uint32_t* d_count, int quads, hipStream_t stream)
+                            uint32_t* d_count, int quads, const uint32_t* d_run_if, hipStream_t stream)
 {
     int64_t words = ((int64_t)max_vox / 64 + 1024) * n_sigma;
     int gx = (int)((words + MMX_WG * 8 - 1) / (MMX_WG * 8));
@@ -341,7 +456,7 @@
     dim3 grid(gx, n_blocks);
     hipLaunchKernelGGL(peaks_sparse_kernel, grid, dim3(MMX_WG), 0, stream, d_log,
                        reinterpret_cast<const ulonglong2*>(d_mask), n_sigma, sigma_stride,
-                       d_blocks, slot_elems, thr, eps, d_cands, cap, d_count, quads);
+                       d_blocks, slot_elems, thr, eps, d_cands, cap, d_count, quads, d_run_if);
     return hipGetLastError() == hipSuccess ? MMX_OK : MMX_ERR_HIP;
 }
 
diff --git a/magellanmapper_amd/csrc/mmx_ymfma.hip b/magellanmapper_amd/csrc/mmx_ymfma.hip
--- a/magellanmapper_amd/csrc/mmx_ymfma.hip
+++ b/magellanmapper_amd/csrc/mmx_ymfma.hip
@@ -50,7 +50,7 @@
 __global__ void __launch_bounds__(NB <= 4 ? 256 : YM6_WAVES * 64, NB <= 4 ? 3 : (YM6_WAVES == 4 ? YM5_OCC : 1))
 ym_kernel(const mmx_block* __restrict__ blocks, int64_t slot_elems, int64_t tile_stride,
           const unsigned* __restrict__ gt, float* __restrict__ out, ym_cfg cfg,
-          unsigned long long* __restrict__ mask)
+          unsigned long long* __restrict__ mask, mmx_cand_list list_arg)
 {
     constexpr int RB = 8 * (NB - 2);
     constexpr int NF = NB <= 4 ? 4 : YM6_NF;
@@ -58,6 +58,7 @@
     constexpr int WAVES = NB <= 4 ? 4 : YM6_WAVES;
     constexpr int JH = NB <= 4 ? 4 : YM6_JH;
     __shared__ float tr[WAVES * 2 * 1024];
+    __shared__ mmx_cand_list list_lds;
 
     const mmx_block bd = blocks[cfg.reverse ? gridDim.y - 1 - blockIdx.y : blockIdx.y];
     const int ntx = (bd.nx + 15) >> 4, ntz = (bd.nz + 15) >> 4;
@@ -83,7 +84,9 @@
         }
         frag[e] = (u4_y){pk[0], pk[1], pk[2], pk[3]};
     }
+    if (MASK && threadIdx.x == 0) list_lds = list_arg;
     __syncthreads();
+    const bool with_list = MASK && list_arg.head != nullptr;
 
     const int wv = __builtin_amdgcn_readfirstlane((int)(threadIdx.x >> 6));
     const int tile = (int)blockIdx.x * (WAVES / 4) + (wv >> 2);
@@ -110,6 +113,13 @@
     ulonglong2* mrow = MASK ? reinterpret_cast<ulonglong2*>(mask) + ((int64_t)bd.slot * slot_elems >> 5) +
                               (4 * U + zq) * ntx + c
                             : nullptr;
+    int erow = (4 * U + zq) * ntx + c;
+    auto put_row = [&](unsigned long long m, unsigned long long a) __attribute__((always_inline)) {
+        if (lane == 0) {
+            *mrow = make_ulonglong2(m, a);
+            if (with_list && m) { const mmx_cand_list list = list_lds; mmx_list_push(list, true, mmx_list_item(list.sigma, bd.slot, erow)); }
+        }
+    };
     unsigned long long ab_prev = 0;
     const bool has_l = xi > 0, has_r = xi < 15 && x + 1 < bd.nx;
     float prev1 = -INFINITY, prev2 = -INFINITY, nbx_prev = -INFINITY;
@@ -137,8 +147,9 @@
                                       !(fmaxf(fmaxf(prev2, acc), nbx_prev) > prev1 + nms_eps);
                     m = __ballot(cand);
                 }
-                if (lane == 0) *mrow = make_ulonglong2(m, ab_prev);
+                put_row(m, ab_prev);
                 mrow += nent;
+                erow += nent;
             }
             prev2 = prev1; prev1 = acc; nbx_prev = nbx;
             ab_prev = ab;
@@ -155,11 +166,13 @@
                     const bool cand = real & (prev1 > nms_lo) & !(fmaxf(prev2, nbx_prev) > prev1 + nms_eps);
                     m = __ballot(cand);
                 }
-                if (lane == 0) *mrow = make_ulonglong2(m, ab_prev);
+                put_row(m, ab_prev);
                 mrow += nent;
+                erow += nent;
             }
             if (lane < cnt - 1) mrow[(int64_t)lane * nent] = make_ulonglong2(0ull, 0ull);
             mrow += (int64_t)(cnt - 1) * nent;
+            erow += (cnt - 1) * nent;
             prev1 = prev2 = nbx_prev = -INFINITY;
             ab_prev = 0;
             ydone += cnt;
@@ -218,7 +231,13 @@
             *dst = make_ulonglong2((unsigned long long)e0 | ((unsigned long long)e1 << 32),
                                    (unsigned long long)e2 | ((unsigned long long)e3 << 32));
         }
+        if (with_list && (some | ab_prev)) {
+            const mmx_cand_list list = list_lds;
+            mmx_list_push(list, (e0 | e1) != 0u,
+                          mmx_list_item(list.sigma, bd.slot, erow + (ydone > 0 ? lane : lane - 1) * nent));
+        }
         mrow += (int64_t)(ydone > 0 ? 16 : 15) * nent;
+        erow += (ydone > 0 ? 16 : 15) * nent;
         prev2 = v[14]; prev1 = v[15]; nbx_prev = nbx15;
         ab_prev = ab[15];
         ydone += 16;
@@ -365,22 +384,23 @@
             const bool cand = real & (prev1 > nms_lo) & !(fmaxf(prev2, nbx_prev) > prev1 + nms_eps);
             m = __ballot(cand);
         }
-        if (lane == 0) *mrow = make_ulonglong2(m, ab_prev);
+        put_row(m, ab_prev);
     }
 }
 
 template <int NB>
 int launch_ym(const mmx_block* d_blocks, int n_blocks, const mmx_zx6_plan& plan, int64_t slot_elems,
-              const ym_cfg& cfg, const float* d_p, float* d_log, unsigned long long* d_mask, hipStream_t s)
+              const ym_cfg& cfg, const float* d_p, float* d_log, unsigned long long* d_mask, const mmx_cand_list& list,
+              hipStream_t s)
 {
     constexpr int TPW = NB <= 4 ? 1 : YM6_WAVES / 4;
     dim3 grid((plan.max_tiles + TPW - 1) / TPW, n_blocks);
     if (d_mask)
         hipLaunchKernelGGL((ym_kernel<NB, true>), grid, dim3(256 * TPW), 0, s, d_blocks, slot_elems, plan.tile_stride,
-                           reinterpret_cast<const unsigned*>(d_p), d_log, cfg, d_mask);
+                           reinterpret_cast<const unsigned*>(d_p), d_log, cfg, d_mask, list);
     else
         hipLaunchKernelGGL((ym_kernel<NB, false>), grid, dim3(256 * TPW), 0, s, d_blocks, slot_elems, plan.tile_stride,
-                           reinterpret_cast<const unsigned*>(d_p), d_log, cfg, d_mask);
+                           reinterpret_cast<const unsigned*>(d_p), d_log, cfg, d_mask, list);
     return hipGetLastError() == hipSuccess ? MMX_OK : MMX_ERR_HIP;
 }
 
@@ -388,7 +408,8 @@
 
 int mmx_launch_ym(const mmx_block* d_blocks, int n_blocks, const mmx_zx6_plan& plan, int64_t slot_elems,
                   const mmx_taps_f32& taps, int radius, const float* d_p, float cp, float cq,
-                  float* d_log, unsigned long long* d_mask, float nms_lo, float nms_eps, hipStream_t stream)
+                  float* d_log, unsigned long long* d_mask, float nms_lo, float nms_eps, const mmx_cand_list& list,
+                  hipStream_t stream)
 {
     if (radius < 1 || radius > 24 || radius > MMX_MAX_RADIUS_FAST || !(cp > 0.f) || !(cq > 0.f)) return MMX_ERR_UNSUPPORTED;
     ym_cfg cfg;
@@ -416,7 +437,7 @@
     cfg.eps = nms_eps / cfg.unscale;
     cfg.radius = radius;
     cfg.reverse = 1;
-    if (radius <= 8) return launch_ym<3>(d_blocks, n_blocks, plan, slot_elems, cfg, d_p, d_log, d_mask, stream);
-    if (radius <= 16) return launch_ym<4>(d_blocks, n_blocks, plan, slot_elems, cfg, d_p, d_log, d_mask, stream);
-    return launch_ym<5>(d_blocks, n_blocks, plan, slot_elems, cfg, d_p, d_log, d_mask, stream);
-}
+    if (radius <= 8) return launch_ym<3>(d_blocks, n_blocks, plan, slot_elems, cfg, d_p, d_log, d_mask, list, stream);
+    if (radius <= 16) return launch_ym<4>(d_blocks, n_blocks, plan, slot_elems, cfg, d_p, d_log, d_mask, list, stream);
+    return launch_ym<5>(d_blocks, n_blocks, plan, slot_elems, cfg, d_p, d_log, d_mask, list, stream);
+}
```

New measurement: 31450. -28.8%, worse.
